# architsharma97/earl_benchmark

Hardware: AMD Instinct MI355X
Metric: env steps/sec (aggregate) at N parallel envs (higher is better)
Workload: dtype f64

## Files before the change

### earl_benchmark_amd/_abi.py

```python
import ctypes as C
import os

EARL_OK = 0
REWARD_SPARSE, REWARD_DENSE = 0, 1
REWARD_TYPES = {'sparse': REWARD_SPARSE, 'dense': REWARD_DENSE}
TABLETOP3_EVAL_CHUNK = 8


class TabletopCfg(C.Structure):
  _fields_ = [('n', C.c_int32), ('env_offset', C.c_int32), ('reward_type', C.c_int32), ('wide_init', C.c_int32),
              ('reset_at_goal', C.c_int32), ('horizon', C.c_int32), ('goal_change_frequency', C.c_int32),
              ('auto_reset', C.c_int32), ('n_goals', C.c_int32), ('n_sample_goals', C.c_int32),
              ('seed', C.c_uint64), ('counter', C.c_uint64)]


class TabletopState(C.Structure):
  _fields_ = [('qpos', C.c_void_p), ('attached', C.c_void_p), ('goal_idx', C.c_void_p), ('goal_table', C.c_void_p),
              ('steps_since_reset', C.c_void_p), ('num_interventions', C.c_void_p),
              ('steps_since_goal_change', C.c_void_p), ('lifelong_return', C.c_void_p), ('counter_base', C.c_void_p)]


class TabletopOut(C.Structure):
  _fields_ = [('obs', C.c_void_p), ('reward', C.c_void_p), ('done', C.c_void_p), ('success', C.c_void_p), ('reward_f64', C.c_void_p)]


ACT_NONE, ACT_RELU, ACT_TANH = 0, 1, 2
ACTIVATIONS = {'none': ACT_NONE, 'relu': ACT_RELU, 'tanh': ACT_TANH}


class MlpPolicy(C.Structure):
  _fields_ = [('n_layers', C.c_int32), ('dims', C.c_int32 * 4), ('hidden_act', C.c_int32), ('out_act', C.c_int32), ('precision', C.c_int32),
              ('params', C.c_void_p)]


HEAD_MEAN, HEAD_SAMPLE = 0, 1
LOGSTD_CLAMP, LOGSTD_TANH = 0, 1
LOGSTD_MAPS = {'clamp': LOGSTD_CLAMP, 'tanh': LOGSTD_TANH}


class GaussianHead(C.Structure):
  _fields_ = [('mode', C.c_int32), ('log_std_map', C.c_int32), ('log_std_min', C.c_float), ('log_std_max', C.c_float), ('eps_out', C.c_void_p)]


class PolicyPopulation(C.Structure):
  _fields_ = [('n_policies', C.c_int32), ('envs_per_policy', C.c_int32), ('param_stride', C.c_int64)]


class EpisodeSummary(C.Structure):
  _fields_ = [('ret', C.c_void_p), ('success_last', C.c_void_p), ('first_success', C.c_void_p)]


class PlanParams(C.Structure):
  _fields_ = [('K', C.c_int32), ('H', C.c_int32), ('iterations', C.c_int32), ('iteration0', C.c_int32), ('sigma', C.c_float * 3), ('noise_counter', C.c_uint32),
              ('inv_temperature', C.c_double)]


class MpcOut(C.Structure):
  _fields_ = [('act', C.c_void_p), ('plan', C.c_void_p), ('ret0', C.c_void_p), ('best_ret', C.c_void_p)]


MPC_MAX_K, MPC_MAX_H = 1024, 256


class PlanValue(C.Structure):
  _fields_ = [('discount', C.c_double), ('value', C.POINTER(MlpPolicy))]


PLAN_VALUE_MAX_H1 = 16


class PlanPrior(C.Structure):
  _fields_ = [('policy', C.POINTER(MlpPolicy)), ('branches', C.c_int32), ('sigma', C.c_float * 3), ('act', C.c_void_p)]


PLAN_PRIOR_MAX_H1 = 16


class CemParams(C.Structure):
  _fields_ = [('K', C.c_int32), ('H', C.c_int32), ('iterations', C.c_int32), ('iteration0', C.c_int32), ('elites', C.c_int32), ('sigma', C.c_float * 3),
              ('noise_counter', C.c_uint32), ('alpha', C.c_float), ('std_min', C.c_float), ('std_max', C.c_float)]


CEM_MAX_K = 1024


class AgentPair(C.Structure):
  _fields_ = [('switch_every', C.c_int32 * 2), ('switch_on_success', C.c_int32), ('pad_', C.c_int32), ('param_stride', C.c_int64), ('backward_goal', C.c_void_p),
              ('phase', C.c_void_p), ('steps_in_phase', C.c_void_p), ('agent_out', C.c_void_p), ('forward_success', C.c_void_p), ('backward_success', C.c_void_p)]


class BackwardGoals(C.Structure):
  _fields_ = [('table', C.c_void_p), ('n_rows', C.c_int32), ('pad_', C.c_int32), ('row', C.c_void_p), ('row_out', C.c_void_p)]


PRECISION_BF16 = 16
PAIR_MAX_H2 = 128


class MotorParams(C.Structure):
  _fields_ = [('kp', C.c_double), ('kd', C.c_double), ('voltage', C.c_double), ('viscous_damping', C.c_double),
              ('torque_control', C.c_int32)]


class KitchenParams(C.Structure):
  _fields_ = [('pos_bound', C.c_double * 2 * 23), ('vel_bound', C.c_double * 2 * 23), ('pos_noise_amp', C.c_double * 23),
              ('act_mid', C.c_double * 9), ('act_amp', C.c_double * 9), ('mocap_range', C.c_double * 3),
              ('mocap_clip_lower', C.c_double * 3), ('mocap_clip_upper', C.c_double * 3), ('step_duration', C.c_double),
              ('robot_noise_ratio', C.c_double)]


class SawyerCfg(C.Structure):
  _fields_ = [('n', C.c_int32), ('env_offset', C.c_int32), ('reward_type', C.c_int32), ('horizon', C.c_int32),
              ('frame_skip', C.c_int32), ('att_hand', C.c_int32), ('att_right', C.c_int32), ('att_left', C.c_int32),
              ('att_obj', C.c_int32), ('obj_dof', C.c_int32), ('obj_kind', C.c_int32), ('n_goal_rows', C.c_int32), ('goal_change_frequency', C.c_int32), ('n_wide', C.c_int32),
              ('att_grasp', C.c_int32), ('att_lpad', C.c_int32), ('att_rpad', C.c_int32), ('pad2_', C.c_int32),
              ('action_scale', C.c_double),
              ('mocap_low', C.c_double * 3), ('mocap_high', C.c_double * 3), ('mocap_quat', C.c_double * 4),
              ('success_radius', C.c_double), ('hand_init_pos', C.c_double * 3), ('obj_init_pos', C.c_double * 3),
              ('obj_init_angle', C.c_double), ('angle_noise', C.c_double * 2),
              ('obj_low', C.c_double * 3), ('obj_high', C.c_double * 3), ('obj_reject_xy', C.c_double * 2), ('obj_reject_radius', C.c_double),
              ('goal_table', C.c_void_p), ('wide_table', C.c_void_p), ('wide_shift', C.c_double * 3), ('wide_noise', C.c_double),
              ('init_tcp', C.c_double * 3), ('box_corners', C.c_double * 3 * 4),
              ('seed', C.c_uint64), ('counter', C.c_uint64), ('step_counter', C.c_uint64)]


class SawyerState(C.Structure):
  _fields_ = [('qpos', C.c_void_p), ('qvel', C.c_void_p), ('mocap_pos', C.c_void_p), ('goal', C.c_void_p),
              ('steps_since_reset', C.c_void_p), ('steps_since_goal_change', C.c_void_p), ('obj_init', C.c_void_p),
              ('last_obs', C.c_void_p), ('fail_count', C.c_void_p), ('sched', C.c_void_p)]


class SawyerOut(C.Structure):
  _fields_ = [('obs', C.c_void_p), ('reward', C.c_void_p), ('done', C.c_void_p), ('success', C.c_void_p), ('status', C.c_void_p), ('info', C.c_void_p)]


class SawyerBranchWs(C.Structure):
  _fields_ = [('base', C.c_void_p), ('bytes', C.c_int64)]


class SawyerPlanParams(C.Structure):
  _fields_ = [('K', C.c_int32), ('H', C.c_int32), ('iterations', C.c_int32), ('iteration0', C.c_int32), ('sigma', C.c_float * 4), ('noise_counter', C.c_uint32),
              ('inv_temperature', C.c_double)]


class SawyerCemParams(C.Structure):
  _fields_ = [('K', C.c_int32), ('H', C.c_int32), ('iterations', C.c_int32), ('iteration0', C.c_int32), ('elites', C.c_int32), ('sigma', C.c_float * 4),
              ('noise_counter', C.c_uint32), ('alpha', C.c_float), ('std_min', C.c_float), ('std_max', C.c_float)]


class SawyerPlanPrior(C.Structure):
  _fields_ = [('policy', C.POINTER(MlpPolicy)), ('branches', C.c_int32), ('sigma', C.c_float * 4), ('obs0', C.c_void_p), ('act', C.c_void_p)]


SAWYER_PLAN_MAX_K = 8192
SAWYER_CEM_MAX_E = 1024
SAWYER_INFO = 8
SAWYER_INFO_KEYS = ('success', 'near_object', 'grasp_success', 'grasp_reward', 'in_place_reward', 'obj_to_target', 'unscaled_reward')
STEP_DIVERGED = 1


class KitchenCfg(C.Structure):
  _fields_ = [('n', C.c_int32), ('env_offset', C.c_int32), ('horizon', C.c_int32), ('frame_skip', C.c_int32), ('sensor_noise', C.c_int32),
              ('n_att', C.c_int32), ('site_att', C.c_int32 * 8), ('seed', C.c_uint64), ('counter', C.c_uint64), ('mocap_quat_dev', C.c_void_p)]


class KitchenState(C.Structure):
  _fields_ = [(k, C.c_void_p) for k in ('qpos', 'qvel', 'mocap_pos', 'goal', 'last_qp_robot', 'att_xpos', 'steps_since_reset', 'fail_count', 'last_obs',
                                        'action64', 'ctrl9', 'noise', 'qpos_bak', 'qvel_bak', 'sites', 'bad', 'mocap_bak', 'att_bak')]


class KitchenOut(C.Structure):
  _fields_ = [(k, C.c_void_p) for k in ('obs', 'reward', 'done', 'success', 'status')]


class MinitaurCfg(C.Structure):
  _fields_ = [('n', C.c_int32), ('env_offset', C.c_int32), ('horizon', C.c_int32), ('num_substeps', C.c_int32), ('settle_steps', C.c_int32),
              ('randomize', C.c_int32), ('n_goals', C.c_int32), ('goal_change_frequency', C.c_int32), ('overheat_steps', C.c_int32),
              ('motor_dof', C.c_int32 * 8), ('pad_', C.c_int32), ('motor_dir', C.c_double * 8), ('motor_kp', C.c_double), ('motor_kd', C.c_double),
              ('motor_velocity_limit', C.c_double), ('overheat_torque', C.c_double), ('distance_weight', C.c_double), ('energy_weight', C.c_double),
              ('success_radius', C.c_double), ('goal_table', C.c_void_p), ('reset_qpos', C.c_void_p),
              ('base_mass_err', C.c_double * 2), ('leg_mass_err', C.c_double * 2), ('leg_mass', C.c_double), ('motor_mass', C.c_double),
              ('foot_friction', C.c_double * 2), ('seed', C.c_uint64), ('counter', C.c_uint64), ('step_counter', C.c_uint64)]


class MinitaurState(C.Structure):
  _fields_ = [(k, C.c_void_p) for k in ('qpos', 'qvel', 'goal', 'motor_param', 'observed_torque', 'overheat', 'motor_enabled', 'steps_since_reset',
                                        'steps_since_goal_change', 'fail_count', 'last_obs')]


class MinitaurOut(C.Structure):
  _fields_ = [(k, C.c_void_p) for k in ('obs', 'reward', 'done', 'success', 'status')]


_P = C.POINTER
SIGNATURES = {
    'earl_tabletop_step': [_P(TabletopCfg), _P(TabletopState), C.c_void_p, C.c_void_p, _P(TabletopOut), C.c_void_p],
    'earl_tabletop_rollout': [_P(TabletopCfg), _P(TabletopState), C.c_int32, C.c_void_p, _P(TabletopOut), C.c_void_p],
    'earl_tabletop_reset_rollout': [_P(TabletopCfg), _P(TabletopState), C.c_int32, C.c_void_p, _P(TabletopOut), C.c_void_p],
    'earl_tabletop_eval_episodes': [_P(TabletopCfg), _P(TabletopState), C.c_int32, C.c_int32, C.c_void_p, C.c_int64, _P(TabletopOut), C.c_void_p],
    'earl_tabletop_policy_rollout': [_P(TabletopCfg), _P(TabletopState), _P(MlpPolicy), C.c_int32, C.c_int32, C.c_int32, _P(TabletopOut), C.c_void_p, C.c_void_p],
    'earl_tabletop_policy_rollout_gaussian': [_P(TabletopCfg), _P(TabletopState), _P(MlpPolicy), _P(GaussianHead), C.c_int32, C.c_int32, C.c_int32, _P(TabletopOut),
                                              C.c_void_p, C.c_void_p],
    'earl_tabletop_population_rollout': [_P(TabletopCfg), _P(TabletopState), _P(MlpPolicy), _P(PolicyPopulation), _P(GaussianHead), C.c_int32, C.c_int32, C.c_int32,
                                         _P(TabletopOut), C.c_void_p, _P(EpisodeSummary), C.c_void_p],
    'earl_tabletop_pair_rollout': [_P(TabletopCfg), _P(TabletopState), _P(MlpPolicy), _P(AgentPair), _P(GaussianHead), C.c_int32, C.c_int32, C.c_int32, _P(TabletopOut),
                                   C.c_void_p, C.c_void_p],
    'earl_tabletop_reset': [_P(TabletopCfg), _P(TabletopState), C.c_void_p, C.c_void_p, C.c_void_p, C.c_void_p],
    'earl_tabletop_observe': [_P(TabletopCfg), _P(TabletopState), _P(TabletopOut), C.c_void_p],
    'earl_tabletop_reward': [C.c_int32, C.c_void_p, C.c_int32, C.c_int32, C.c_void_p, C.c_void_p, C.c_void_p],
    'earl_tabletop_valid_init': [C.c_int32, C.c_void_p, C.c_void_p, C.c_void_p],
    'earl_tabletop3_step': [_P(TabletopCfg), _P(TabletopState), C.c_void_p, _P(TabletopOut), C.c_void_p],
    'earl_tabletop3_rollout': [_P(TabletopCfg), _P(TabletopState), C.c_int32, C.c_void_p, _P(TabletopOut), C.c_void_p],
    'earl_tabletop3_reset': [_P(TabletopCfg), _P(TabletopState), C.c_void_p, C.c_void_p, C.c_void_p],
    'earl_tabletop3_reward': [C.c_int32, C.c_void_p, C.c_int32, C.c_void_p, C.c_void_p, C.c_void_p],
    'earl_tabletop3_eval_episodes': [_P(TabletopCfg), _P(TabletopState), C.c_int32, C.c_int32, C.c_void_p, C.c_int64, _P(TabletopOut), C.c_void_p],
    'earl_tabletop3_policy_rollout': [_P(TabletopCfg), _P(TabletopState), _P(MlpPolicy), _P(PolicyPopulation), _P(GaussianHead), C.c_int32, C.c_int32, C.c_int32,
                                      _P(TabletopOut), C.c_void_p, _P(EpisodeSummary), C.c_void_p],
    'earl_tabletop3_pair_rollout': [_P(TabletopCfg), _P(TabletopState), _P(MlpPolicy), _P(AgentPair), _P(GaussianHead), C.c_int32, C.c_int32, C.c_int32, _P(TabletopOut),
                                    C.c_void_p, C.c_void_p],
    'earl_tabletop_branch_rollout': [_P(TabletopCfg), _P(TabletopState), C.c_int32, C.c_int32, C.c_void_p, C.c_int64, _P(EpisodeSummary), C.c_void_p, C.c_void_p],
    'earl_tabletop3_branch_rollout': [_P(TabletopCfg), _P(TabletopState), C.c_int32, C.c_int32, C.c_void_p, C.c_int64, _P(EpisodeSummary), C.c_void_p, C.c_void_p],
    'earl_tabletop_plan_mppi': [_P(TabletopCfg), _P(TabletopState), _P(PlanParams)] + [C.c_void_p] * 7,
    'earl_tabletop3_plan_mppi': [_P(TabletopCfg), _P(TabletopState), _P(PlanParams)] + [C.c_void_p] * 7,
    'earl_tabletop_plan_candidates': [_P(TabletopCfg), _P(PlanParams), C.c_int32, C.c_void_p, C.c_void_p, C.c_void_p],
    'earl_tabletop_mpc_rollout': [_P(TabletopCfg), _P(TabletopState), _P(PlanParams), C.c_int32, _P(TabletopOut), _P(MpcOut), C.c_void_p],
    'earl_tabletop3_mpc_rollout': [_P(TabletopCfg), _P(TabletopState), _P(PlanParams), C.c_int32, _P(TabletopOut), _P(MpcOut), C.c_void_p],
    'earl_tabletop_plan_mppi_value': [_P(TabletopCfg), _P(TabletopState), _P(PlanParams), _P(PlanValue)] + [C.c_void_p] * 7,
    'earl_tabletop3_plan_mppi_value': [_P(TabletopCfg), _P(TabletopState), _P(PlanParams), _P(PlanValue)] + [C.c_void_p] * 7,
    'earl_tabletop_mpc_rollout_value': [_P(TabletopCfg), _P(TabletopState), _P(PlanParams), _P(PlanValue), C.c_int32, _P(TabletopOut), _P(MpcOut), C.c_void_p],
    'earl_tabletop3_mpc_rollout_value': [_P(TabletopCfg), _P(TabletopState), _P(PlanParams), _P(PlanValue), C.c_int32, _P(TabletopOut), _P(MpcOut), C.c_void_p],
    'earl_tabletop_plan_mppi_prior': [_P(TabletopCfg), _P(TabletopState), _P(PlanParams), _P(PlanValue), _P(PlanPrior)] + [C.c_void_p] * 7,
    'earl_tabletop3_plan_mppi_prior': [_P(TabletopCfg), _P(TabletopState), _P(PlanParams), _P(PlanValue), _P(PlanPrior)] + [C.c_void_p] * 7,
    'earl_tabletop_plan_cem': [_P(TabletopCfg), _P(TabletopState), _P(CemParams), _P(PlanValue)] + [C.c_void_p] * 9,
    'earl_tabletop3_plan_cem': [_P(TabletopCfg), _P(TabletopState), _P(CemParams), _P(PlanValue)] + [C.c_void_p] * 9,
    'earl_tabletop_cem_candidates': [_P(TabletopCfg), _P(CemParams), C.c_int32, C.c_void_p, C.c_void_p, C.c_void_p, C.c_void_p],
    'earl_tabletop_mpc_rollout_cem': [_P(TabletopCfg), _P(TabletopState), _P(CemParams), _P(PlanValue), C.c_int32, _P(TabletopOut), _P(MpcOut), C.c_void_p],
    'earl_tabletop3_mpc_rollout_cem': [_P(TabletopCfg), _P(TabletopState), _P(CemParams), _P(PlanValue), C.c_int32, _P(TabletopOut), _P(MpcOut), C.c_void_p],
    'earl_debug_set_rollout_impl': [C.c_int],
    'earl_debug_set_rollout3_form': [C.c_int],
    'earl_debug_set_rollout_wgs_per_cu': [C.c_int],
    'earl_debug_read_ws_profile': [C.c_void_p, C.c_int32],
    'earl_sawyer_sparse_f64': [C.c_int32, C.c_void_p, C.c_double, C.c_void_p, C.c_void_p, C.c_void_p],
    'earl_sawyer_sparse_f32': [C.c_int32, C.c_void_p, C.c_double, C.c_void_p, C.c_void_p, C.c_void_p],
    'earl_minitaur_leg_to_motor': [C.c_int32, C.c_void_p, C.c_void_p, C.c_void_p],
    'earl_minitaur_motor_torque': [C.c_int32, _P(MotorParams), C.c_void_p, C.c_void_p, C.c_void_p, C.c_void_p, C.c_void_p, C.c_void_p],
    'earl_minitaur_reward': [C.c_int32, C.c_void_p, C.c_double, C.c_double, C.c_double, C.c_void_p, C.c_void_p, C.c_void_p],
    'earl_kitchen_reward': [C.c_int32] + [C.c_void_p] * 6,
    'earl_kitchen_default_params': [_P(KitchenParams)],
    'earl_kitchen_action': [C.c_int32, _P(KitchenParams)] + [C.c_void_p] * 5,
    'earl_kitchen_obs': [C.c_int32, _P(KitchenParams)] + [C.c_void_p] * 5,
    'earl_philox_uniform': [C.c_int32, C.c_int32, C.c_uint64, C.c_uint64, C.c_int32, C.c_uint32, C.c_double, C.c_double, C.c_void_p, C.c_void_p],
    'earl_physics_step': [C.c_void_p, C.c_void_p, C.c_int32, C.c_int32, C.c_int32] + [C.c_void_p] * 7,
    'earl_physics_forward': [C.c_void_p, C.c_void_p, C.c_int32, C.c_int32] + [C.c_void_p] * 9,
    'earl_physics_model_size': [],
    'earl_physics_model24_size': [],
    'earl_collision_model_size': [],
    'earl_sawyer_cfg_size': [],
    'earl_physics_forget_table': [C.c_void_p],
    'earl_debug_set_physics_lanes': [C.c_int],
    'earl_debug_set_door_variant': [C.c_int],
    'earl_debug_set_peg_schedule': [C.c_int],
    'earl_debug_set_sawyer_prior_launches': [C.c_int],
    'earl_kitchen_step': [C.c_void_p, C.c_void_p, _P(KitchenParams), _P(KitchenCfg), _P(KitchenState), C.c_void_p, _P(KitchenOut), C.c_void_p],
    'earl_kitchen_rollout': [C.c_void_p, C.c_void_p, _P(KitchenParams), _P(KitchenCfg), _P(KitchenState), C.c_void_p, C.c_int32, _P(KitchenOut), C.c_void_p],
    'earl_sawyer_rollout': [C.c_void_p, C.c_void_p, C.c_int32, _P(SawyerCfg), _P(SawyerState), C.c_void_p, C.c_int32, _P(SawyerOut), C.c_void_p],
    'earl_minitaur_rollout': [C.c_void_p, C.c_void_p, _P(MinitaurCfg), _P(MinitaurState), C.c_void_p, C.c_int32, _P(MinitaurOut), C.c_void_p],
    'earl_sawyer_rollout_clocked': [C.c_void_p, C.c_void_p, C.c_int32, _P(SawyerCfg), _P(SawyerState), C.c_void_p, C.c_int32, C.c_void_p, _P(SawyerOut), C.c_void_p],
    'earl_kitchen_rollout_clocked': [C.c_void_p, C.c_void_p, _P(KitchenParams), _P(KitchenCfg), _P(KitchenState), C.c_void_p, C.c_int32, C.c_void_p, _P(KitchenOut),
                                     C.c_void_p],
    'earl_minitaur_rollout_clocked': [C.c_void_p, C.c_void_p, _P(MinitaurCfg), _P(MinitaurState), C.c_void_p, C.c_int32, C.c_void_p, _P(MinitaurOut), C.c_void_p],
    'earl_sawyer_policy_rollout': [C.c_void_p, C.c_void_p, C.c_int32, _P(SawyerCfg), _P(SawyerState), _P(MlpPolicy), _P(GaussianHead), C.c_void_p, C.c_int32, C.c_void_p,
                                   C.c_void_p, _P(SawyerOut), C.c_void_p],
    'earl_sawyer_population_rollout': [C.c_void_p, C.c_void_p, C.c_int32, _P(SawyerCfg), _P(SawyerState), _P(MlpPolicy), _P(PolicyPopulation), _P(GaussianHead), C.c_void_p,
                                       C.c_int32, C.c_void_p, C.c_void_p, _P(SawyerOut), _P(EpisodeSummary), C.c_void_p],
    'earl_sawyer_pair_rollout': [C.c_void_p, C.c_void_p, C.c_int32, _P(SawyerCfg), _P(SawyerState), _P(MlpPolicy), _P(AgentPair), _P(GaussianHead), C.c_void_p,
                                 C.c_int32, C.c_void_p, C.c_void_p, _P(SawyerOut), C.c_void_p],
    'earl_sawyer_agents_rollout': [C.c_void_p, C.c_void_p, C.c_int32, _P(SawyerCfg), _P(SawyerState), _P(MlpPolicy), _P(AgentPair), _P(PolicyPopulation), _P(BackwardGoals),
                                   _P(GaussianHead), C.c_void_p, C.c_int32, C.c_void_p, C.c_void_p, _P(SawyerOut), _P(EpisodeSummary), C.c_void_p],
    'earl_sawyer_branch_ws_bytes': [C.c_int32, C.c_int32, C.c_int32, _P(C.c_int64)],
    'earl_sawyer_branch_rollout': [C.c_void_p, C.c_void_p, C.c_int32, _P(SawyerCfg), _P(SawyerState), C.c_int32, C.c_int32, C.c_void_p, C.c_int64, C.c_void_p,
                                   _P(SawyerBranchWs), _P(EpisodeSummary), C.c_void_p, C.c_void_p, C.c_void_p],
    'earl_sawyer_plan_ws_bytes': [C.c_int32, C.c_int32, C.c_int32, C.c_int32, _P(C.c_int64)],
    'earl_sawyer_plan_mppi': [C.c_void_p, C.c_void_p, C.c_int32, _P(SawyerCfg), _P(SawyerState), _P(SawyerPlanParams), C.c_void_p, C.c_void_p, C.c_void_p, C.c_void_p,
                              C.c_void_p, C.c_void_p, C.c_void_p, C.c_void_p, _P(SawyerBranchWs), C.c_void_p],
    'earl_sawyer_plan_candidates': [_P(SawyerCfg), _P(SawyerPlanParams), C.c_int32, C.c_void_p, C.c_void_p, C.c_void_p],
    'earl_sawyer_plan_cem': [C.c_void_p, C.c_void_p, C.c_int32, _P(SawyerCfg), _P(SawyerState), _P(SawyerCemParams)] + [C.c_void_p] * 11 + [_P(SawyerBranchWs), C.c_void_p],
    'earl_sawyer_cem_candidates': [_P(SawyerCfg), _P(SawyerCemParams), C.c_int32, C.c_void_p, C.c_void_p, C.c_void_p, C.c_void_p],
    'earl_sawyer_cem_update': [_P(SawyerCfg), _P(SawyerCemParams), C.c_int32] + [C.c_void_p] * 11,
    'earl_sawyer_value_ws_bytes': [C.c_int32, C.c_int32, C.c_int32, C.c_int32, _P(C.c_int64)],
    'earl_sawyer_branch_rollout_value': [C.c_void_p, C.c_void_p, C.c_int32, _P(SawyerCfg), _P(SawyerState), C.c_int32, C.c_int32, C.c_void_p, C.c_int64, C.c_void_p,
                                         _P(PlanValue), _P(SawyerBranchWs), _P(EpisodeSummary), C.c_void_p, C.c_void_p, C.c_void_p],
    'earl_sawyer_plan_mppi_value': [C.c_void_p, C.c_void_p, C.c_int32, _P(SawyerCfg), _P(SawyerState), _P(SawyerPlanParams), _P(PlanValue)] + [C.c_void_p] * 8
                                   + [_P(SawyerBranchWs), C.c_void_p],
    'earl_sawyer_plan_cem_value': [C.c_void_p, C.c_void_p, C.c_int32, _P(SawyerCfg), _P(SawyerState), _P(SawyerCemParams), _P(PlanValue)] + [C.c_void_p] * 11
                                  + [_P(SawyerBranchWs), C.c_void_p],
    'earl_sawyer_prior_ws_bytes': [C.c_int32, C.c_int32, C.c_int32, C.c_int32, _P(C.c_int64)],
    'earl_sawyer_branch_rollout_prior': [C.c_void_p, C.c_void_p, C.c_int32, _P(SawyerCfg), _P(SawyerState), C.c_int32, C.c_int32, C.c_void_p, C.c_int64, C.c_void_p,
                                         _P(PlanValue), _P(SawyerPlanPrior), C.c_int32, C.c_uint32, _P(SawyerBranchWs), _P(EpisodeSummary), C.c_void_p, C.c_void_p, C.c_void_p],
    'earl_sawyer_plan_mppi_prior': [C.c_void_p, C.c_void_p, C.c_int32, _P(SawyerCfg), _P(SawyerState), _P(SawyerPlanParams), _P(PlanValue), _P(SawyerPlanPrior)]
                                   + [C.c_void_p] * 8 + [_P(SawyerBranchWs), C.c_void_p],
    'earl_sawyer_plan_cem_prior': [C.c_void_p, C.c_void_p, C.c_int32, _P(SawyerCfg), _P(SawyerState), _P(SawyerCemParams), _P(PlanValue), _P(SawyerPlanPrior)]
                                  + [C.c_void_p] * 11 + [_P(SawyerBranchWs), C.c_void_p],
    'earl_minitaur_policy_rollout': [C.c_void_p, C.c_void_p, _P(MinitaurCfg), _P(MinitaurState), _P(MlpPolicy), _P(GaussianHead), C.c_void_p, C.c_int32, C.c_void_p,
                                     C.c_void_p, _P(MinitaurOut), C.c_void_p],
    'earl_minitaur_population_rollout': [C.c_void_p, C.c_void_p, _P(MinitaurCfg), _P(MinitaurState), _P(MlpPolicy), _P(PolicyPopulation), _P(GaussianHead), C.c_void_p,
                                         C.c_int32, C.c_void_p, C.c_void_p, _P(MinitaurOut), _P(EpisodeSummary), C.c_void_p],
    'earl_minitaur_agents_rollout': [C.c_void_p, C.c_void_p, _P(MinitaurCfg), _P(MinitaurState), _P(MlpPolicy), _P(AgentPair), _P(PolicyPopulation), _P(BackwardGoals),
                                     _P(GaussianHead), C.c_void_p, C.c_int32, C.c_void_p, C.c_void_p, _P(MinitaurOut), _P(EpisodeSummary), C.c_void_p],
    'earl_kitchen_population_rollout': [C.c_void_p, C.c_void_p, _P(KitchenParams), _P(KitchenCfg), _P(KitchenState), _P(MlpPolicy), _P(PolicyPopulation), _P(GaussianHead),
                                        C.c_void_p, C.c_int32, C.c_void_p, C.c_void_p, _P(KitchenOut), _P(EpisodeSummary), C.c_void_p],
    'earl_kitchen_agents_rollout': [C.c_void_p, C.c_void_p, _P(KitchenParams), _P(KitchenCfg), _P(KitchenState), _P(MlpPolicy), _P(AgentPair), _P(PolicyPopulation),
                                    _P(BackwardGoals), C.c_void_p, C.c_int32, _P(GaussianHead), C.c_void_p, C.c_int32, C.c_void_p, C.c_void_p, _P(KitchenOut),
                                    _P(EpisodeSummary), C.c_void_p],
    'earl_kitchen_policy_rollout': [C.c_void_p, C.c_void_p, _P(KitchenParams), _P(KitchenCfg), _P(KitchenState), _P(MlpPolicy), _P(GaussianHead), C.c_void_p, C.c_int32,
                                    C.c_void_p, C.c_void_p, _P(KitchenOut), C.c_void_p],
    'earl_minitaur_reset': [C.c_void_p, C.c_void_p, _P(MinitaurCfg), _P(MinitaurState), C.c_void_p, C.c_void_p, C.c_void_p],
    'earl_minitaur_cfg_size': [],
    'earl_debug_set_minitaur_stepper': [C.c_int],
    'earl_debug_set_minitaur_duo': [C.c_int],
    'earl_debug_set_solo': [C.c_int],
    'earl_debug_set_solo_mt': [C.c_int],
    'earl_sawyer_reset': [C.c_void_p, C.c_int32, _P(SawyerCfg), _P(SawyerState)] + [C.c_void_p] * 5,
    'earl_sawyer_observe': [C.c_void_p, C.c_int32, _P(SawyerCfg), _P(SawyerState), C.c_void_p, C.c_void_p],
    'earl_sawyer_door_reward': [_P(SawyerCfg), C.c_int32, C.c_void_p, C.c_void_p, C.c_void_p, C.c_void_p],
    'earl_sawyer_door_info': [_P(SawyerCfg), C.c_int32, C.c_void_p, C.c_void_p, C.c_void_p, C.c_void_p],
    'earl_version': [],
    'earl_last_error': [],
    'earl_device_count': [],
}
_RESTYPES = {'earl_version': C.c_char_p, 'earl_last_error': C.c_char_p}

LIB_PATH = os.path.join(os.path.dirname(os.path.abspath(__file__)), 'csrc', 'libearl_hip.so')
_lib = None


class EarlHipError(RuntimeError):
  pass


def load():
  global _lib
  if _lib is None:
    if not os.path.exists(LIB_PATH):
      raise EarlHipError(f'{LIB_PATH} not found: build it with `python -c "import __graft_entry__ as g; g.build()"` '
                         '(or `make -C earl_benchmark_amd/csrc`). There is no CPU fallback.')
    import torch
    lib = C.CDLL(LIB_PATH)
    for name, argtypes in SIGNATURES.items():
      fn = getattr(lib, name)
      fn.argtypes = argtypes
      fn.restype = _RESTYPES.get(name, C.c_int)
    _lib = lib
  return _lib


HOST_LIB_PATH = os.path.join(os.path.dirname(os.path.abspath(__file__)), 'csrc', 'libearl_host.so')
HOST_SIGNATURES = {name + '_cpu': argtypes[:-1] for name, argtypes in SIGNATURES.items()
                   if name.startswith(('earl_tabletop_', 'earl_tabletop3_'))}
HOST_EXTRA_SIGNATURES = {
    'earl_mlp_policy_forward_cpu': ([_P(MlpPolicy), _P(GaussianHead), C.c_int32, C.c_void_p, C.c_void_p, C.c_void_p], C.c_int32),
    'earl_sawyer_plan_candidates_cpu': ([_P(SawyerCfg), _P(SawyerPlanParams), C.c_int32, C.c_void_p, C.c_void_p], C.c_int32),
    'earl_sawyer_plan_update_cpu': ([_P(SawyerCfg), _P(SawyerPlanParams), C.c_int32] + [C.c_void_p] * 7, C.c_int32),
    'earl_sawyer_cem_candidates_cpu': ([_P(SawyerCfg), _P(SawyerCemParams), C.c_int32, C.c_void_p, C.c_void_p, C.c_void_p], C.c_int32),
    'earl_sawyer_cem_update_cpu': ([_P(SawyerCfg), _P(SawyerCemParams), C.c_int32] + [C.c_void_p] * 10, C.c_int32),
    'earl_sawyer_value_terminal_cpu': ([_P(PlanValue), C.c_int32, C.c_int32, C.c_void_p, C.c_void_p], C.c_int32),
    'earl_sawyer_prior_actions_cpu': ([_P(SawyerCfg), _P(SawyerPlanPrior), C.c_int32, C.c_int32, C.c_int32, C.c_uint32, C.c_int32, C.c_void_p, C.c_void_p], C.c_int32),
    'earl_tanh_f32': ([C.c_float], C.c_float),
    'earl_exp_f32': ([C.c_float], C.c_float),
    'earl_normal_quantile_f32': ([C.c_uint32], C.c_float),
}
_host = None


class HostLib:

  def __init__(self, cdll):
    self._cdll = cdll
    for name, argtypes in HOST_SIGNATURES.items():
      fn = getattr(cdll, name)
      fn.argtypes, fn.restype = argtypes, C.c_int
      setattr(self, name, fn)
      setattr(self, name[:-4], (lambda f: (lambda *a: f(*a[:-1])))(fn))
    for name, (argtypes, restype) in HOST_EXTRA_SIGNATURES.items():
      fn = getattr(cdll, name)
      fn.argtypes, fn.restype = argtypes, restype
      setattr(self, name, fn)
    cdll.earl_host_last_error.restype = C.c_char_p
    cdll.earl_host_version.restype = C.c_char_p
    cdll.earl_host_set_threads.argtypes = [C.c_int]
    self.earl_last_error = cdll.earl_host_last_error
    self.earl_version = cdll.earl_host_version
    self.set_threads = cdll.earl_host_set_threads


def load_host():
  global _host
  if _host is None:
    if not os.path.exists(HOST_LIB_PATH):
      raise EarlHipError(f'{HOST_LIB_PATH} not found: build it with `make -C earl_benchmark_amd/csrc libearl_host.so`')
    try:
      flags = next((ln for ln in open('/proc/cpuinfo') if ln.startswith('flags')), '')
    except OSError:
      flags = 'avx2 fma'
    missing = [f for f in ('avx2', 'fma') if f not in flags.split()]
    if missing:
      raise EarlHipError(f'{HOST_LIB_PATH} needs a CPU with {" and ".join(missing)} (built with -mavx2 -mfma); this one has neither the HIP path (device="cpu" was asked for) nor those')
    _host = HostLib(C.CDLL(HOST_LIB_PATH))
  return _host


def check(rc, what, lib=None):
  if rc != EARL_OK:
    msg = (lib or load()).earl_last_error()
    raise EarlHipError(f'{what} failed with code {rc}: {msg.decode() if msg else "?"}')
```

### earl_benchmark_amd/csrc/minitaur_stepper.h

```cpp
#pragma once

template <int CTRL>
__device__ __forceinline__ double dpp_quad(const double v) {
  const int lo = __builtin_amdgcn_update_dpp(0, __double2loint(v), CTRL, 0xf, 0xf, false);
  const int hi = __builtin_amdgcn_update_dpp(0, __double2hiint(v), CTRL, 0xf, 0xf, false);
  return __hiloint2double(hi, lo);
}
template <int CTRL> __device__ __forceinline__ V3 dpp_quad(const V3& v) { return {dpp_quad<CTRL>(v.x), dpp_quad<CTRL>(v.y), dpp_quad<CTRL>(v.z)}; }
template <int CTRL> __device__ __forceinline__ Q4 dpp_quad(const Q4& q) { return {dpp_quad<CTRL>(q.w), dpp_quad<CTRL>(q.x), dpp_quad<CTRL>(q.y), dpp_quad<CTRL>(q.z)}; }
constexpr int QP_PARENT = 0xA0;
constexpr int QP_CHILD = 0xF5;
constexpr int QP_SWAP1 = 0xB1;
constexpr int QP_SWAP2 = 0x4E;
template <int P> constexpr int qp_bcast() { return P * 0x55; }

__device__ __forceinline__ double kc(double x) {
  asm volatile("" : "+s"(x));
  return x;
}
__device__ __forceinline__ void sincos_kc(double x, double& sn, double& cs) {
  const double k = rint(x * kc(6.36619772367581382433e-01));
  double r = fma(-k, kc(1.57079632673412561417e+00), x);
  r = fma(-k, kc(6.07710050650619224932e-11), r);
  const double z = r * r;
  double ps = fma(z, kc(1.58969099521155010221e-10), kc(-2.50507602534068634195e-08));
  ps = fma(z, ps, kc(2.75573137070700676789e-06));
  ps = fma(z, ps, kc(-1.98412698298579493134e-04));
  ps = fma(z, ps, kc(8.33333333332248946124e-03));
  ps = fma(z, ps, kc(-1.66666666666666324348e-01));
  const double sr = fma(r * z, ps, r);
  double pc = fma(z, kc(-1.13596475577881948265e-11), kc(2.08757232129817482790e-09));
  pc = fma(z, pc, kc(-2.75573143513906633035e-07));
  pc = fma(z, pc, kc(2.48015872894767294178e-05));
  pc = fma(z, pc, kc(-1.38888888888741095749e-03));
  pc = fma(z, pc, kc(4.16666666666666019037e-02));
  const double cr = fma(z * z, pc, fma(-0.5, z, 1.0));
  const int q = (int)k & 3;
  sn = (q == 0) ? sr : ((q == 1) ? cr : ((q == 2) ? -sr : -cr));
  cs = (q == 0) ? cr : ((q == 1) ? -sr : ((q == 2) ? -cr : sr));
}

#ifdef EARL_MT_DEBUG
__device__ int g_mt_dbg[4096 * 8 * 32];
__device__ double g_mt_dbg_al[4096 * 8 * 32];
__device__ double g_mt_dbg_x[5][4096 * 8 * 32];
__device__ double g_mt_dbg_ph[8][4096 * 8 * 32];
#define DBG_PH(k, v) do { if (isl) g_mt_dbg_ph[k][((size_t)s.dbg_env * 8 + (s.dbg_ts & 7)) * 32 + l] = (v); } while (0)
#else
#define DBG_PH(k, v) do {} while (0)
#endif
struct MTDims {
  static constexpr int NV = 22, NR = 6, NLEG = 4, LS = 4, NH = 16, LPE = 32, MC = EARL_MAXCON, MB = 8;
};

struct PairTabMT {
  static constexpr int MP = 64;
  double pos[MP][3], r[MP], margin[MP];
  int link[MP], cls[MP];
};
__device__ __forceinline__ void stage_pairs_mt(PairTabMT& t, const earl_collision_model* __restrict__ col) {
  const int i = threadIdx.x;
  if (col && i < PairTabMT::MP && i < col->n_pair) {
    t.pos[i][0] = col->pair_rec[i].pos[0]; t.pos[i][1] = col->pair_rec[i].pos[1]; t.pos[i][2] = col->pair_rec[i].pos[2];
    t.r[i] = col->pair_rec[i].r; t.margin[i] = col->pair_rec[i].margin;
    t.link[i] = col->pair_rec[i].sph_link; t.cls[i] = col->pair_rec[i].cls;
  }
}
template <int N>
__device__ __forceinline__ void chol_small(double (&L)[N * (N + 1) / 2]) {
#pragma unroll
  for (int j = 0; j < N; ++j) {
    double d = L[j * (j + 1) / 2 + j];
#pragma unroll
    for (int p = 0; p < j; ++p) d = fma(-L[j * (j + 1) / 2 + p], L[j * (j + 1) / 2 + p], d);
    const double inv = rsq2(d);
    L[j * (j + 1) / 2 + j] = inv;
#pragma unroll
    for (int i = j + 1; i < N; ++i) {
      double t = L[i * (i + 1) / 2 + j];
#pragma unroll
      for (int p = 0; p < j; ++p) t = fma(-L[i * (i + 1) / 2 + p], L[j * (j + 1) / 2 + p], t);
      L[i * (i + 1) / 2 + j] = t * inv;
    }
  }
}

struct SharedMTData {
  static constexpr int NV = MTDims::NV, MC = MTDims::MC;
  double qp[NV], qv[NV];
  double bq[4];
  double aprev[NV];
  struct { double ext[NV]; double motor_volt, motor_visc; double mscale[3], foot_mu; } xt;
  double eres[12], eD[12], ear[12];
  struct { double obs_t[8], cmd[8]; int oh[8], en[8]; double goal[2]; int steps, sgc, pad_[2]; } ev;
  struct { double cD, cmu, car[4]; unsigned int cact; int cd1, cd2, pid; } c3[MC];
  unsigned int tb[NV][4];
#ifdef EARL_MT_DEBUG
  int dbg_env, dbg_ts, dbg_pad[2];
#endif
  union {
    double ct[MC][8];
    double cw[MC][8];
  };
  double CJr[MC][3][6];
  double CJh[MC][3][2];
  int crow[MC][2];
  union {
    struct { double obs[46]; } kit;
    struct {
      double Xq[NV][4], Xp[NV][3];
      double Sh[MTDims::NH][6];
      double redI[9][10];
      double redF[9][6];
    } dyn;
    struct {
      double Bw[NV][6];
      double rw[NV];
      double sh_keep[MTDims::NH][6];
      double Aw[MTDims::NH][4];
      int nct;
    } hand;
    struct {
      double HA[MTDims::NLEG][10];
      double HB[MTDims::NH][6];
      double HR[6][6];
      double rc[NV];
      double Wl[6][16];
      double part[6][4];
      double Y[16];
      double LL[MTDims::NLEG][10];
      double SS[22];
      double xr0[6];
    } pas;
  };
};
static_assert(sizeof(((SharedMTData*)nullptr)->ev) % 16 == 0 && sizeof(((SharedMTData*)nullptr)->c3) % 16 == 0 && sizeof(((SharedMTData*)nullptr)->tb) % 16 == 0 && offsetof(SharedMTData, dyn) % 16 == 0, "16-byte alignment of the blocks the kernels read as b128");
static_assert(offsetof(SharedMTData, hand.sh_keep) == offsetof(SharedMTData, dyn.Sh) && offsetof(SharedMTData, hand.Aw) == offsetof(SharedMTData, dyn.redI) &&
              sizeof(((SharedMTData*)nullptr)->hand) <= sizeof(((SharedMTData*)nullptr)->dyn), "the hand-over block keeps clear of the motion subspaces and fits the dynamics block");
struct SharedMT : SharedMTData {
  static constexpr int R = (int)(sizeof(SharedMTData) % 256);
  static constexpr int PAD = R <= 64 ? 64 - R : (R <= 192 ? 192 - R : 320 - R);
  char bank_pad[PAD == 0 ? 16 : PAD];
};
static_assert(sizeof(SharedMT) % 16 == 0, "an env block is a whole number of 16-byte words: the blocks of one wave all keep the alignment ds_read_b128 needs");

__device__ __forceinline__ void integrate_mt(SharedMT& s, const earl_link_model24& m, const int sub, const bool isl, const int l, const double dt, const double al,
                                             const double qd, const double ql_, const Q4 Qb) {
  fence();
  if (isl) {
    const double nv_ = fma(dt, al, qd);
    s.qv[l] = nv_;
    s.qp[l] = fma(dt, nv_, ql_);
  }
  fence();
  {
    const int bd = m.ball_dof;
    const V3 wbd{s.qv[bd], s.qv[bd + 1], s.qv[bd + 2]};
    auto norm2 = [](const Q4& q) { return fma(q.z, q.z, fma(q.y, q.y, fma(q.x, q.x, q.w * q.w))); };
    auto mul4 = [](const Q4& a, const Q4& b) {
      return Q4{fma(-a.z, b.z, fma(-a.y, b.y, fma(-a.x, b.x, a.w * b.w))), fma(-a.z, b.y, fma(a.y, b.z, fma(a.x, b.w, a.w * b.x))),
                fma(a.z, b.x, fma(a.y, b.w, fma(-a.x, b.z, a.w * b.y))), fma(a.z, b.w, fma(-a.y, b.x, fma(a.x, b.y, a.w * b.z)))};
    };
    Q4 q0 = Qb;
    const double n0 = rsq2(norm2(q0));
    q0 = Q4{q0.w * n0, q0.x * n0, q0.y * n0, q0.z * n0};
    const double w2 = fma(wbd.z, wbd.z, fma(wbd.y, wbd.y, wbd.x * wbd.x));
    const double iw = w2 > 0 ? rsq2(w2 > 0 ? w2 : 1.0) : 0.0;
    double sn, cs;
    sincos_kc(0.5 * dt * (w2 * iw), sn, cs);
    const Q4 q1 = mul4(q0, Q4{cs, sn * wbd.x * iw, sn * wbd.y * iw, sn * wbd.z * iw});
    const double n1 = rsq2(norm2(q1));
    if (sub == 0) { s.bq[0] = q1.w * n1; s.bq[1] = q1.x * n1; s.bq[2] = q1.y * n1; s.bq[3] = q1.z * n1; }
    fence();
  }
}

template <bool INTEGRATE, int ROLE = 0>
__device__ __forceinline__ void substep_mt(SharedMT& s, const earl_link_model24& m, const BlkTable<MTDims::MB, true>& bt, const PairTabMT& pt,
                                           const int sub, const int grp, const bool warm, double* qacc_out) {
  constexpr int NV = MTDims::NV, MC = MTDims::MC, LPE = MTDims::LPE;
  const int maxcon = bt.max_con < MC ? bt.max_con : MC;
  const double dt = m.dt;
  const bool isroot = sub < 6, ishinge = sub >= 8 && sub < 24, isl = isroot || ishinge;
  const int l = isroot ? sub : (ishinge ? sub - 2 : NV - 1);
  const int hq = (sub - 8) & 3;
  const int leg = ishinge ? (sub - 8) >> 2 : 0;
  const bool lower = ishinge && (hq & 1), upper = ishinge && !(hq & 1);
  PSTART();
  const V3 Pb = ld3(s.qp);
  const Q4 Qb = ldq(s.bq);
  double Rb[3][3];
  qmat(Qb, Rb);
  Q4 Q; V3 P;
  const V3 ax = ld3(m.jaxis[l]);
  const int jt = m.jtype[l];
  const double ql_ = s.qp[l], qd = s.qv[l];
  double Bw[6], Aw[4], rw;
  int nct = 0, ncmax = 0;
  if constexpr (ROLE != 2) {
  {
    const Q4 tq = ldq(m.tquat[l]);
    const V3 tp = ld3(m.tpos[l]);
    double sn, cs;
    sincos_kc(jt == 0 ? 0.5 * ql_ : 0.0, sn, cs);
    const Q4 qloc = qmul(tq, Q4{cs, sn * ax.x, sn * ax.y, sn * ax.z});
    const Q4 Qu = qmul(Qb, qloc);
    const V3 Pu = add(Pb, mulv(Rb, tp));
    const Q4 Qp = dpp_quad<QP_PARENT>(Qu);
    const V3 Pp = dpp_quad<QP_PARENT>(Pu);
    double Rp[3][3];
    qmat(Qp, Rp);
    const Q4 Qw = qmul(Qp, qloc);
    const V3 Pw = add(Pp, mulv(Rp, tp));
    const Q4 Qr = selq(sub < 3, Q4{1, 0, 0, 0}, Qb);
    const V3 Pr{Pb.x, sub >= 1 ? Pb.y : 0.0, sub >= 2 ? Pb.z : 0.0};
    Q = selq(isroot, Qr, selq(lower, Qw, Qu));
    P = selv(isroot, Pr, selv(lower, Pw, Pu));
  }
#ifdef EARL_MT_DEBUG_FRAMES
  DBG_PH(0, Q.w); DBG_PH(1, Q.x); DBG_PH(2, Q.y); DBG_PH(3, Q.z); DBG_PH(4, P.x); DBG_PH(5, P.y); DBG_PH(6, P.z); DBG_PH(7, ql_);
#else
  DBG_PH(0, Q.w + 2 * Q.x + 3 * Q.y + 5 * Q.z + 7 * P.x + 11 * P.y + 13 * P.z);
  DBG_PH(5, ql_); DBG_PH(6, Qb.w + 2 * Qb.x + 3 * Qb.y + 5 * Qb.z + 7 * Pb.x + 11 * Pb.y + 13 * Pb.z); DBG_PH(7, qd);
#endif
  if (isl) {
    double* oq = s.dyn.Xq[l];
    double* op = s.dyn.Xp[l];
    oq[0] = Q.w; oq[1] = Q.x; oq[2] = Q.y; oq[3] = Q.z; op[0] = P.x; op[1] = P.y; op[2] = P.z;
  }
  fence();
  unsigned int nearw = 0, nearg = 0;
  {
    const int b = sub < bt.n_blk ? sub : 0;
    const int bl = bt.link[b];
    V3 cs = ld3(bt.center[b]);
    {
      double Rl[3][3];
      qmat(ldq(s.dyn.Xq[bl < 0 ? 0 : bl]), Rl);
      cs = selv(bl < 0, cs, add(ld3(s.dyn.Xp[bl < 0 ? 0 : bl]), mulv(Rl, cs)));
    }
    double Rbx[3][3];
    qmat(ldq(bt.box_quat[b]), Rbx);
    const V3 x = mulvT(Rbx, vsub(cs, ld3(bt.box_pos[b]))), h = ld3(bt.box_half[b]);
    const V3 d{x.x - fmin(fmax(x.x, -h.x), h.x), x.y - fmin(fmax(x.y, -h.y), h.y), x.z - fmin(fmax(x.z, -h.z), h.z)};
    const bool nearb = sub < bt.n_blk && dot(d, d) < bt.reach[b] * bt.reach[b];
    const unsigned long long bal = __ballot(nearb);
    nearg = (unsigned int)((bal >> (grp * 32)) & 0xFFFFFFFFull);
    nearw = (unsigned int)((bal | (bal >> 32)) & 0xFFFFFFFFull);
  }
  PSTAMP(0);
  V3 Sw, Sv;
  double I10[10];
  double R[3][3];
  qmat(Q, R);
  {
    const V3 aw = mulv(R, ax);
    const V3 anchor = add(P, mulv(R, ld3(m.jpos[l])));
    const bool rot = jt != 1;
    Sw = selv(rot, aw, V3{0, 0, 0});
    Sv = selv(rot, cross(anchor, aw), aw);
    const int root = m.ball_dof + 2;
    const double ms = l < root ? 1.0 : (l == root ? s.xt.mscale[0] : (m.parent[l] == root ? s.xt.mscale[1] : s.xt.mscale[2]));
    const double mass = m.mass[l] * ms;
    const V3 c = add(P, mulv(R, ld3(m.com[l])));
    const double* in = m.inertia[l];
    const double I[3][3] = {{in[0] * ms, in[3] * ms, in[4] * ms}, {in[3] * ms, in[1] * ms, in[5] * ms}, {in[4] * ms, in[5] * ms, in[2] * ms}};
    double T[3][3], W[3][3];
#pragma unroll
    for (int r = 0; r < 3; ++r)
#pragma unroll
      for (int cc = 0; cc < 3; ++cc) T[r][cc] = R[r][0] * I[0][cc] + R[r][1] * I[1][cc] + R[r][2] * I[2][cc];
#pragma unroll
    for (int r = 0; r < 3; ++r)
#pragma unroll
      for (int cc = r; cc < 3; ++cc) W[r][cc] = T[r][0] * R[cc][0] + T[r][1] * R[cc][1] + T[r][2] * R[cc][2];
    const double c2 = dot(c, c);
    I10[0] = mass;
    I10[1] = mass * c.x; I10[2] = mass * c.y; I10[3] = mass * c.z;
    I10[4] = W[0][0] + mass * (c2 - c.x * c.x);
    I10[5] = W[1][1] + mass * (c2 - c.y * c.y);
    I10[6] = W[2][2] + mass * (c2 - c.z * c.z);
    I10[7] = W[0][1] - mass * c.x * c.y;
    I10[8] = W[0][2] - mass * c.x * c.z;
    I10[9] = W[1][2] - mass * c.y * c.z;
    if (ishinge) {
      double* o = s.dyn.Sh[l - 6];
      o[0] = Sw.x; o[1] = Sw.y; o[2] = Sw.z; o[3] = Sv.x; o[4] = Sv.y; o[5] = Sv.z;
    }
  }
  
#ifndef EARL_MT_DEBUG_FRAMES
  DBG_PH(1, Sw.x + 2 * Sw.y + 3 * Sw.z + 5 * Sv.x + 7 * Sv.y + 11 * Sv.z + 13 * I10[0] + 17 * I10[1] + 19 * I10[2] + 23 * I10[3] + 29 * I10[4] + 31 * I10[5] + 37 * I10[6] + 41 * I10[7] + 43 * I10[8] + 47 * I10[9]);
#endif
  PSTAMP(1);
  double Ic[10];
#pragma unroll
  for (int e = 0; e < 10; ++e) {
    const double ch = dpp_quad<QP_CHILD>(I10[e]);
    Ic[e] = upper ? I10[e] + ch : I10[e];
  }
  if (upper || sub == 5) {
    double* o = s.dyn.redI[upper ? (l - 6) >> 1 : 8];
#pragma unroll
    for (int e = 0; e < 10; ++e) o[e] = Ic[e];
  }
  fence();
  {
    double tot[10];
#pragma unroll
    for (int e = 0; e < 10; ++e) tot[e] = s.dyn.redI[8][e];
#ifndef EARL_MT_NO_CHUNK
#define EARL_MT_NO_CHUNK 0
#endif
    if constexpr (ROLE == 0 || EARL_MT_NO_CHUNK) {
#pragma unroll
      for (int u = 0; u < 8; ++u)
#pragma unroll
        for (int e = 0; e < 10; ++e) tot[e] += s.dyn.redI[u][e];
    } else {
#pragma unroll
      for (int u = 0; u < 8; u += 2) {
        double part[20];
#pragma unroll
        for (int e = 0; e < 10; ++e) { part[e] = s.dyn.redI[u][e]; part[10 + e] = s.dyn.redI[u + 1][e]; }
        pin_batch(part);
#pragma unroll
        for (int e = 0; e < 10; ++e) tot[e] += part[e];
#pragma unroll
        for (int e = 0; e < 10; ++e) tot[e] += part[10 + e];
        pin_batch(tot);
      }
    }
#pragma unroll
    for (int e = 0; e < 10; ++e) Ic[e] = isroot ? tot[e] : Ic[e];
  }
  
#ifndef EARL_MT_DEBUG_FRAMES
  DBG_PH(2, Ic[0] + 2 * Ic[1] + 3 * Ic[2] + 5 * Ic[3] + 7 * Ic[4] + 11 * Ic[5] + 13 * Ic[6] + 17 * Ic[7] + 19 * Ic[8] + 23 * Ic[9]);
#endif
  PSTAMP(3);
  double g6[6], Add, Ach;
  {
    V3 n, f;
    iapply(Ic, Sw, Sv, n, f);
    const V3 mo = mulvT(Rb, add(n, cross(f, Pb)));
    g6[0] = f.x; g6[1] = f.y; g6[2] = f.z; g6[3] = mo.x; g6[4] = mo.y; g6[5] = mo.z;
    Add = dot(Sw, n) + dot(Sv, f) + m.armature[l];
    const V3 nc = dpp_quad<QP_CHILD>(n), fc = dpp_quad<QP_CHILD>(f);
    Ach = dot(Sw, nc) + dot(Sv, fc);
  }
  
#ifndef EARL_MT_DEBUG_FRAMES
  DBG_PH(3, g6[0] + 2 * g6[1] + 3 * g6[2] + 5 * g6[3] + 7 * g6[4] + 11 * g6[5] + 13 * Add + 17 * Ach);
#endif
  PSTAMP(4);
  const V3 vlin = ld3(s.qv), om = ld3(s.qv + 3);
  const V3 wb = mulv(Rb, om);
  const V3 vb = add(vlin, cross(Pb, wb));
  double tau_l;
  {
    const V3 wu = add(wb, scl(Sw, qd)), vu = add(vb, scl(Sv, qd));
    const V3 wpar = dpp_quad<QP_PARENT>(wu), vpar = dpp_quad<QP_PARENT>(vu);
    const V3 w = selv(isroot, wb, selv(lower, add(wpar, scl(Sw, qd)), wu));
    const V3 v = selv(isroot, vb, selv(lower, add(vpar, scl(Sv, qd)), vu));
    const V3 cwh = scl(cross(w, Sw), qd), cvh = scl(add(cross(v, Sw), cross(w, Sv)), qd);
    const V3 cw = selv(ishinge, cwh, V3{0, 0, 0});
    const V3 cv = selv(ishinge, cvh, scl(cross(vlin, Sw), qd));
    const V3 ab{-m.gravity[0], -m.gravity[1], -m.gravity[2]};
    const V3 avb = add(ab, cross(vlin, wb));
    const V3 awu = cw, avu = add(avb, cv);
    const V3 awp = dpp_quad<QP_PARENT>(awu), avp = dpp_quad<QP_PARENT>(avu);
    const V3 aw = selv(isroot, V3{0, 0, 0}, selv(lower, add(awp, cw), awu));
    const V3 av = selv(isroot, avb, selv(lower, add(avp, cv), avu));
    V3 n1, f1, n2, f2;
    iapply(I10, aw, av, n1, f1);
    iapply(I10, w, v, n2, f2);
    const V3 n = add(n1, add(cross(w, n2), cross(v, f2)));
    const V3 f = add(f1, cross(w, f2));
    const V3 nch = dpp_quad<QP_CHILD>(n), fch = dpp_quad<QP_CHILD>(f);
    V3 ns = selv(upper, add(n, nch), n), fs = selv(upper, add(f, fch), f);
    if (upper || sub == 5) {
      double* o = s.dyn.redF[upper ? (l - 6) >> 1 : 8];
      o[0] = ns.x; o[1] = ns.y; o[2] = ns.z; o[3] = fs.x; o[4] = fs.y; o[5] = fs.z;
    }
    fence();
    V3 nt = ld3(s.dyn.redF[8]), ft = ld3(s.dyn.redF[8] + 3);
    if constexpr (ROLE == 0 || EARL_MT_NO_CHUNK) {
#pragma unroll
      for (int u = 0; u < 8; ++u) { nt = add(nt, ld3(s.dyn.redF[u])); ft = add(ft, ld3(s.dyn.redF[u] + 3)); }
    } else {
#pragma unroll
      for (int u = 0; u < 8; u += 4) {
        double part[24];
#pragma unroll
        for (int k = 0; k < 24; ++k) part[k] = s.dyn.redF[u + k / 6][k % 6];
        pin_batch(part);
#pragma unroll
        for (int w = 0; w < 4; ++w) { nt = add(nt, V3{part[6 * w], part[6 * w + 1], part[6 * w + 2]}); ft = add(ft, V3{part[6 * w + 3], part[6 * w + 4], part[6 * w + 5]}); }
        nt = V3{pinned(nt.x), pinned(nt.y), pinned(nt.z)}; ft = V3{pinned(ft.x), pinned(ft.y), pinned(ft.z)};
      }
    }
    ns = selv(isroot, nt, ns); fs = selv(isroot, ft, fs);
    tau_l = -m.damping[l] * qd - (dot(Sw, ns) + dot(Sv, fs)) + s.xt.ext[l];
  }
  
#ifndef EARL_MT_DEBUG_FRAMES
  DBG_PH(4, tau_l);
#endif
  PSTAMP(5);
  if (nearw) {
    unsigned int rest = nearw;
    while (rest) {
      int myb = -1, myoff = 0, used = 0;
      unsigned int taken = 0;
      for (unsigned int r2 = rest; r2; r2 &= r2 - 1u) {
        const int b = __builtin_ctz(r2);
        const int sz = bt.end[b] - bt.begin[b];
        if (used + sz > LPE) { if (used == 0) { taken = 1u << b; used = sz; if (sub < sz) { myb = b; myoff = 0; } } break; }
        if (sub >= used && sub < used + sz) { myb = b; myoff = used; }
        used += sz;
        taken |= 1u << b;
      }
      rest &= ~taken;
      const bool has = myb >= 0;
      const int b = has ? myb : 0;
      const bool mine = has && ((nearg >> b) & 1u);
      const int bsz = bt.end[b] - bt.begin[b];
      const V3 pb = ld3(bt.box_pos[b]);
      double Rbx[3][3];
      qmat(ldq(bt.box_quat[b]), Rbx);
      const V3 h = ld3(bt.box_half[b]);
      const int room = bt.cap[b] & 255;
      const int pi = has ? bt.begin[b] + (sub - myoff < bsz ? sub - myoff : bsz - 1) : 0;
      const bool valid = mine && sub - myoff < bsz;
      const int lk = pt.link[pi], cls = pt.cls[pi];
      const double r = pt.r[pi], margin = pt.margin[pi];
      V3 c = ld3(pt.pos[pi]);
      {
        double Rl[3][3];
        qmat(ldq(s.dyn.Xq[lk < 0 ? 0 : lk]), Rl);
        c = selv(lk < 0, c, add(ld3(s.dyn.Xp[lk < 0 ? 0 : lk]), mulv(Rl, c)));
      }
      const V3 x = mulvT(Rbx, vsub(c, pb));
      V3 q{fmin(fmax(x.x, -h.x), h.x), fmin(fmax(x.y, -h.y), h.y), fmin(fmax(x.z, -h.z), h.z)};
      const bool outside = fabs(x.x) > h.x || fabs(x.y) > h.y || fabs(x.z) > h.z;
      const V3 dd = vsub(x, q);
      const double d2 = dot(dd, dd);
      const double inv = rsq2(outside ? d2 : 1.0);
      const double gx = h.x - fabs(x.x), gy = h.y - fabs(x.y), gz = h.z - fabs(x.z);
      const int axn = (gx <= gy && gx <= gz) ? 0 : (gy <= gz ? 1 : 2);
      const double xa = pick3(x, axn), ha = pick3(h, axn), sg = xa >= 0 ? 1.0 : -1.0;
      const V3 ni{axn == 0 ? sg : 0.0, axn == 1 ? sg : 0.0, axn == 2 ? sg : 0.0};
      const V3 qi{axn == 0 ? sg * ha : x.x, axn == 1 ? sg * ha : x.y, axn == 2 ? sg * ha : x.z};
      const double dist = outside ? d2 * inv - r : -(ha - fabs(xa)) - r;
      const V3 nl = selv(outside, scl(dd, inv), ni);
      q = selv(outside, q, qi);
      const bool hit = valid && dist < margin;
      const unsigned long long bal = __ballot(hit);
      const unsigned int gb = (unsigned int)((bal >> (grp * 32)) & 0xFFFFFFFFull);
      const unsigned int seg = has ? (unsigned int)(((1ull << bsz) - 1ull) << myoff) : 0u;
      const int before_blk = __popc(gb & seg & ((1u << sub) - 1u));
      const bool accept = hit && before_blk < room;
      const unsigned long long bal2 = __ballot(accept);
      const unsigned int ga = (unsigned int)((bal2 >> (grp * 32)) & 0xFFFFFFFFull);
      const int slot = nct + __popc(ga & ((1u << sub) - 1u));
      if (accept && slot < maxcon) {
        const V3 n = mulv(Rbx, nl);
        const V3 p = add(add(pb, mulv(Rbx, q)), scl(n, 0.5 * dist));
        double* o = s.ct[slot];
        o[0] = dist; o[1] = n.x; o[2] = n.y; o[3] = n.z; o[4] = p.x; o[5] = p.y; o[6] = p.z;
        o[7] = (double)(cls + 64 * (lk + 1) + 4096 * pi);
      }
      const int took = __popc(ga);
      nct = nct + took < maxcon ? nct + took : maxcon;
    }
    fence();
  }
  PSTAMP(2);
  PCOUNT(20, 1); PCOUNT(21, nearw ? 1 : 0); PCOUNT(22, __popc(nearw));
  if (nearw && __any(nct > 0)) {
#pragma unroll
    for (int k = 0; k < MC; ++k) ncmax = __any(nct > k) ? k + 1 : ncmax;
  }
  {
    const int k1 = m.con_att1[leg], k2 = m.con_att2[leg];
    const V3 pa = add(P, mulv(R, ld3(m.att_pos[hq == 3 ? k1 : k2])));
    const V3 p1 = dpp_quad<qp_bcast<3>()>(pa), p2 = dpp_quad<qp_bcast<1>()>(pa);
    const V3 d = vsub(p1, p2);
    const double w1 = (ishinge && hq >= 2) ? 1.0 : 0.0, w2 = (ishinge && hq < 2) ? 1.0 : 0.0;
    const V3 JE = vsub(scl(add(Sv, cross(Sw, p1)), w1), scl(add(Sv, cross(Sw, p2)), w2));
    V3 jv = scl(JE, qd);
    jv = add(jv, dpp_quad<QP_SWAP1>(jv));
    jv = add(jv, dpp_quad<QP_SWAP2>(jv));
    jv = add(jv, cross(wb, d));
    const int c = hq < 3 ? hq : 2;
    const double res = pick3(d, c);
    double kk, bb;
    kb_of(m.con_solref[leg], m.con_solimp[leg], dt, kk, bb);
    const double dd = imp_p2(m.con_solimp[leg], res);
    const double eDm = rcp_nr(fmax((1 - dd) * m.con_invweight[leg] * rcp_nr(dd), 1e-15));
    const double earm = -bb * pick3(jv, c) - kk * dd * res;
    if (ishinge && hq < 3) { s.eres[3 * leg + hq] = res; s.eD[3 * leg + hq] = eDm; s.ear[3 * leg + hq] = earm; }
    const V3 eDv{dpp_quad<qp_bcast<0>()>(eDm), dpp_quad<qp_bcast<1>()>(eDm), dpp_quad<qp_bcast<2>()>(eDm)};
    const V3 earv{dpp_quad<qp_bcast<0>()>(earm), dpp_quad<qp_bcast<1>()>(earm), dpp_quad<qp_bcast<2>()>(earm)};
    const V3 dj{eDv.x * JE.x, eDv.y * JE.y, eDv.z * JE.z};
    const V3 bx = mulvT(Rb, cross(d, dj));
    double Bh[6] = {g6[0], g6[1], g6[2], g6[3] + bx.x, g6[4] + bx.y, g6[5] + bx.z};
    double Ah[4];
    {
      const V3 j0 = dpp_quad<qp_bcast<0>()>(JE), j1 = dpp_quad<qp_bcast<1>()>(JE), j2 = dpp_quad<qp_bcast<2>()>(JE), j3 = dpp_quad<qp_bcast<3>()>(JE);
      Ah[0] = dot(j0, dj); Ah[1] = dot(j1, dj); Ah[2] = dot(j2, dj); Ah[3] = dot(j3, dj);
#pragma unroll
      for (int p = 0; p < 4; ++p) Ah[p] += p == hq ? Add : ((upper && p == hq + 1) ? Ach : 0.0);
    }
    const double gh = tau_l + dot(dj, earv);
    fence();
    V3 T{0, 0, 0}, G{0, 0, 0};
#pragma unroll
    for (int e = 0; e < MTDims::NLEG; ++e) {
      const V3 de = ld3(s.eres + 3 * e), De = ld3(s.eD + 3 * e), are = ld3(s.ear + 3 * e);
      const V3 sd = cross(Sw, de);
      const V3 u{De.x * sd.x, De.y * sd.y, De.z * sd.z};
      T = add(T, cross(de, u));
      G = add(G, cross(de, V3{De.x * are.x, De.y * are.y, De.z * are.z}));
    }
    const V3 rx = mulvT(Rb, T);
    double Br[6] = {g6[0], g6[1], g6[2], g6[3] + rx.x, g6[4] + rx.y, g6[5] + rx.z};
#pragma unroll
    for (int i = 0; i < 6; ++i) Br[i] += sub == i ? m.armature[l] : 0.0;
    const double gr = tau_l + dot(Sw, G);
#pragma unroll
    for (int i = 0; i < 6; ++i) Bw[i] = isroot ? Br[i] : Bh[i];
#pragma unroll
    for (int p = 0; p < 4; ++p) Aw[p] = Ah[p];
    rw = isroot ? gr : gh;
  }
  PSTAMP(7);
  }
  if constexpr (ROLE == 1) {
    if (isl) {
#pragma unroll
      for (int i = 0; i < 6; ++i) s.hand.Bw[l][i] = Bw[i];
      s.hand.rw[l] = rw;
    }
    if (ishinge) {
#pragma unroll
      for (int p = 0; p < 4; ++p) s.hand.Aw[l - 6][p] = Aw[p];
    }
    if (sub == 0) s.hand.nct = nct;
  }
  if constexpr (ROLE == 0) {
    pin_batch(Bw); pin_batch(Aw); rw = pinned(rw);
  }
  if constexpr (ROLE == 2) {
    nct = s.hand.nct;
    if (__any(nct > 0)) {
#pragma unroll
      for (int k = 0; k < MC; ++k) ncmax = __any(nct > k) ? k + 1 : ncmax;
    }
  }
  double cD = 0, cmu = 0, car[4] = {0, 0, 0, 0};
  unsigned int cact = 0;
  int cd1 = -1, cd2 = -1;
  int cpid = -1;
  if constexpr (ROLE == 2) {
    const int c = sub < MC ? sub : MC - 1;
    cD = s.c3[c].cD; cmu = s.c3[c].cmu;
#pragma unroll
    for (int k = 0; k < 4; ++k) car[k] = s.c3[c].car[k];
    cact = s.c3[c].cact; cd1 = s.c3[c].cd1; cd2 = s.c3[c].cd2;
  }
  if (ROLE != 2 && ncmax > 0) {
    const int c = sub < MC ? sub : MC - 1;
    const bool cv = sub < nct;
    unsigned int pact = s.c3[c].cact;
    int ppid = s.c3[c].pid;
    double rec[8];
#pragma unroll
    for (int k = 0; k < 8; ++k) rec[k] = s.ct[c][k];
    pin_batch(rec);
    asm volatile("" : "+v"(pact), "+v"(ppid));
#pragma unroll
    for (int k = 0; k < 8; ++k) rec[k] = cv ? rec[k] : 0.0;
    const V3 n = selv(cv, V3{rec[1], rec[2], rec[3]}, V3{0, 0, 1}), p = selv(cv, V3{rec[4], rec[5], rec[6]}, V3{0, 0, 0});
    const int pk = cv ? (int)rec[7] : 0;
    const int cls = pk & 63, ls = ((pk >> 6) & 63) - 1;
    cpid = cv ? (pk >> 12) : -1;
    const double ax_ = fabs(n.x), ay_ = fabs(n.y), az_ = fabs(n.z);
    const int ia = (ax_ <= ay_ && ax_ <= az_) ? 0 : (ay_ <= az_ ? 1 : 2);
    const V3 e{ia == 0 ? 1.0 : 0.0, ia == 1 ? 1.0 : 0.0, ia == 2 ? 1.0 : 0.0};
    V3 t1 = cross(n, e);
    t1 = scl(t1, rsq2(dot(t1, t1)));
    const V3 t2 = cross(n, t1);
    cd2 = ls >= 6 ? ls : -1;
    double ctab[6] = {bt.cls_margin[cls], bt.cls_mu[cls], bt.kb_cls[cls][0], bt.kb_cls[cls][1], bt.cls_invw[cls], s.xt.foot_mu};
    double simp[5];
#pragma unroll
    for (int k = 0; k < 5; ++k) simp[k] = bt.cls_solimp[cls][k];
    int par2 = m.parent[cd2 >= 0 ? cd2 : 0], parls = m.parent[ls > 0 ? ls : 0];
    asm volatile("" : "+v"(par2), "+v"(parls));
    pin_batch(ctab); pin_batch(simp);
    cd1 = (cd2 >= 0 && par2 >= 6) ? par2 : -1;
    const V3 rp = vsub(p, Pb);
    const V3 dirs[3] = {n, t1, t2};
    double Jr[3][6], Jh[3][2];
    double sh1[6], sh2[6], qa[4] = {s.qv[cd1 >= 0 ? cd1 : 0], s.qv[cd2 >= 0 ? cd2 : 0], s.aprev[cd1 >= 0 ? cd1 : 0], s.aprev[cd2 >= 0 ? cd2 : 0]};
#pragma unroll
    for (int k = 0; k < 6; ++k) { sh1[k] = s.dyn.Sh[cd1 >= 0 ? cd1 - 6 : 0][k]; sh2[k] = s.dyn.Sh[cd2 >= 0 ? cd2 - 6 : 0][k]; }
    double qr[6], ar[6];
#pragma unroll
    for (int r = 0; r < 6; ++r) { qr[r] = s.qv[r]; ar[r] = s.aprev[r]; }
    pin_batch(sh1); pin_batch(sh2); pin_batch(qa); pin_batch(qr); pin_batch(ar);
    const double* s1 = sh1;
    const double* s2 = sh2;
    const V3 jp1 = add(ld3(s1 + 3), cross(ld3(s1), p)), jp2 = add(ld3(s2 + 3), cross(ld3(s2), p));
#pragma unroll
    for (int k = 0; k < 3; ++k) {
      const V3 t = dirs[k];
      const V3 mo = mulvT(Rb, cross(rp, t));
      Jr[k][0] = cv ? t.x : 0.0; Jr[k][1] = cv ? t.y : 0.0; Jr[k][2] = cv ? t.z : 0.0;
      Jr[k][3] = cv ? mo.x : 0.0; Jr[k][4] = cv ? mo.y : 0.0; Jr[k][5] = cv ? mo.z : 0.0;
      Jh[k][0] = cd1 >= 0 ? dot(t, jp1) : 0.0;
      Jh[k][1] = cd2 >= 0 ? dot(t, jp2) : 0.0;
    }
    if (sub < MC) {
#pragma unroll
      for (int k = 0; k < 3; ++k) {
#pragma unroll
        for (int r = 0; r < 6; ++r) s.CJr[c][k][r] = Jr[k][r];
        s.CJh[c][k][0] = Jh[k][0]; s.CJh[c][k][1] = Jh[k][1];
      }
      s.crow[c][0] = cd1; s.crow[c][1] = cd2;
    }
    double jv[3], jp[3];
    {
      const double q1 = cd1 >= 0 ? qa[0] : 0.0, q2 = cd2 >= 0 ? qa[1] : 0.0;
      const double a1 = cd1 >= 0 ? qa[2] : 0.0, a2 = cd2 >= 0 ? qa[3] : 0.0;
#pragma unroll
      for (int k = 0; k < 3; ++k) {
        double a_ = 0, b_ = 0;
#pragma unroll
        for (int r = 0; r < 6; ++r) { a_ = fma(Jr[k][r], qr[r], a_); b_ = fma(Jr[k][r], ar[r], b_); }
        a_ = fma(Jh[k][0], q1, a_); a_ = fma(Jh[k][1], q2, a_);
        b_ = fma(Jh[k][0], a1, b_); b_ = fma(Jh[k][1], a2, b_);
        jv[k] = a_; jp[k] = b_;
      }
    }
    const double margin = ctab[0];
    cmu = ctab[1];
    {
      const int root = m.ball_dof + 2;
      cmu = (ctab[5] > 0 && ls > root && parls != root) ? ctab[5] : cmu;
    }
    const double kk = ctab[2], bb = ctab[3];
    const double dd = imp_p2(simp, rec[0] - margin);
    const double R0 = fmax((1 - dd) * ctab[4] * rcp_nr(dd), 1e-15);
    cD = cv ? rcp_nr(2 * cmu * cmu * R0) : 0.0;
    const double basea = -kk * dd * (rec[0] - margin);
    car[0] = fma(-bb, fma(cmu, jv[1], jv[0]), basea); car[1] = fma(-bb, fma(-cmu, jv[1], jv[0]), basea);
    car[2] = fma(-bb, fma(cmu, jv[2], jv[0]), basea); car[3] = fma(-bb, fma(-cmu, jv[2], jv[0]), basea);
    unsigned int wbits = 0;
    wbits |= (fma(cmu, jp[1], jp[0]) - car[0] < 0) ? 1u : 0u;
    wbits |= (fma(-cmu, jp[1], jp[0]) - car[1] < 0) ? 2u : 0u;
    wbits |= (fma(cmu, jp[2], jp[0]) - car[2] < 0) ? 4u : 0u;
    wbits |= (fma(-cmu, jp[2], jp[0]) - car[3] < 0) ? 8u : 0u;
#ifndef EARL_MT_NO_CARRY
    cact = cv ? (warm ? ((ppid == cpid) ? pact : wbits) : 0xFu) : 0u;
#else
    cact = cv ? (warm ? wbits : 0xFu) : 0u;
#endif
  }
#ifdef EARL_MT_DEBUG
  if constexpr (ROLE != 2) {
    int* row = g_mt_dbg + ((size_t)s.dbg_env * 8 + (s.dbg_ts & 7)) * 32;
    if (sub < MC) row[4 + sub] = (int)cact;
    if (sub == 0) { row[0] = nct; row[1] = warm ? 1 : 0; }
  }
#endif
  if constexpr (ROLE == 0) {
    cD = pinned(cD); cmu = pinned(cmu); pin_batch(car);
    asm volatile("" : "+v"(cact), "+v"(cd1), "+v"(cd2));
  }
  if constexpr (ROLE == 1) {
    if (sub < MC) {
      s.c3[sub].cD = cD; s.c3[sub].cmu = cmu;
#pragma unroll
      for (int k = 0; k < 4; ++k) s.c3[sub].car[k] = car[k];
      s.c3[sub].cact = cact; s.c3[sub].cd1 = cd1; s.c3[sub].cd2 = cd2; s.c3[sub].pid = cpid;
    }
  }
  unsigned int tbits = 0, sbits = 0, cbits = 0;
  if constexpr (ROLE == 2) {
    tbits = s.tb[l][0]; sbits = s.tb[l][1]; cbits = s.tb[l][2];
  }
  if (ROLE != 2 && ncmax > 0) {
    fence();
#pragma unroll
    for (int c = 0; c < MC; ++c) {
      const int d1 = s.crow[c][0], d2 = s.crow[c][1];
      tbits |= (isroot || l == d1 || l == d2) ? (1u << c) : 0u;
      sbits |= l == d2 ? (1u << c) : 0u;
      cbits |= l == d1 ? (1u << c) : 0u;
    }
  }
  if constexpr (ROLE == 1) {
    if (isl) { s.tb[l][0] = tbits; s.tb[l][1] = sbits; s.tb[l][2] = cbits; }
    return;
  }
  PSTAMP(6);
  PSTAMP(9);
  if constexpr (ROLE == 2) {
    const int hl = ishinge ? l - 6 : 0;
#pragma unroll
    for (int i = 0; i < 6; ++i) Bw[i] = s.hand.Bw[l][i];
#pragma unroll
    for (int p = 0; p < 4; ++p) Aw[p] = s.hand.Aw[hl][p];
    rw = s.hand.rw[l];
    pin_batch(Bw); pin_batch(Aw); rw = pinned(rw);
    fence();
  }
#ifdef EARL_MT_DEBUG
  if (isl) {
    const size_t o_ = ((size_t)s.dbg_env * 8 + (s.dbg_ts & 7)) * 32 + l;
    g_mt_dbg_x[0][o_] = rw;
    g_mt_dbg_x[1][o_] = Bw[0] + 2 * Bw[1] + 3 * Bw[2] + 5 * Bw[3] + 7 * Bw[4] + 11 * Bw[5];
    g_mt_dbg_x[2][o_] = Aw[0] + 2 * Aw[1] + 3 * Aw[2] + 5 * Aw[3];
    g_mt_dbg_x[4][o_] = s.xt.ext[l];
  }
#endif
  double al = 0.0;
  PCOUNT(23, ncmax > 0 ? 1 : 0); PCOUNT(24, ncmax);
  for (int it = 0; it < 8; ++it) {
    PCOUNT(25, 1);
#ifdef EARL_MT_DEBUG
    if (sub == 0) g_mt_dbg[((size_t)s.dbg_env * 8 + (s.dbg_ts & 7)) * 32 + 2] = it + 1;
#endif
    KSTART();
    if (ncmax > 0) {
      if (sub < MC) {
        const double a1 = (cact & 1u) ? cD : 0.0, a2 = (cact & 2u) ? cD : 0.0, a3 = (cact & 4u) ? cD : 0.0, a4 = (cact & 8u) ? cD : 0.0;
        double* w = s.cw[sub];
        w[0] = a1 + a2 + a3 + a4; w[1] = cmu * (a1 - a2); w[2] = cmu * (a3 - a4); w[3] = cmu * cmu * (a1 + a2); w[4] = cmu * cmu * (a3 + a4);
        w[5] = a1 * car[0] + a2 * car[1] + a3 * car[2] + a4 * car[3];
        w[6] = cmu * (a1 * car[0] - a2 * car[1]);
        w[7] = cmu * (a3 * car[2] - a4 * car[3]);
      }
      fence();
    }
    KSTAMP(16);
    {
      double acc6[6] = {0, 0, 0, 0, 0, 0}, accd = 0, accc = 0, rr = rw;
      static_assert(MC % 4 == 0, "contact slots in groups of four");
      for (int c4 = 0; c4 < ncmax; c4 += 4) {
#pragma unroll
        for (int u = 0; u < 4; ++u) {
          const int c = c4 + u;
          const double* w = s.cw[c];
          const int slot = (sbits >> c) & 1u;
          const double tmask = ((tbits >> c) & 1u) ? 1.0 : 0.0, cmask = ((cbits >> c) & 1u) ? 1.0 : 0.0;
          double j[3], jc[3], wv[8], jr[18];
  #pragma unroll
          for (int k = 0; k < 3; ++k) {
            j[k] = *(isroot ? &s.CJr[c][k][l] : &s.CJh[c][k][slot]);
            jc[k] = s.CJh[c][k][1];
          }
  #pragma unroll
          for (int k = 0; k < 8; ++k) wv[k] = w[k];
  #pragma unroll
          for (int k = 0; k < 3; ++k)
  #pragma unroll
            for (int i = 0; i < 6; ++i) jr[6 * k + i] = s.CJr[c][k][i];
          pin6(j[0], j[1], j[2], jc[0], jc[1], jc[2]); pin_batch(wv); pin_batch(jr);
  #pragma unroll
          for (int k = 0; k < 3; ++k) j[k] *= tmask;
          const double v0 = wv[0] * j[0] + wv[1] * j[1] + wv[2] * j[2], v1 = wv[1] * j[0] + wv[3] * j[1], v2 = wv[2] * j[0] + wv[4] * j[2];
          rr += wv[5] * j[0] + wv[6] * j[1] + wv[7] * j[2];
  #pragma unroll
          for (int i = 0; i < 6; ++i) acc6[i] += jr[i] * v0 + jr[6 + i] * v1 + jr[12 + i] * v2;
          accd += j[0] * v0 + j[1] * v1 + j[2] * v2;
          accc += (jc[0] * v0 + jc[1] * v1 + jc[2] * v2) * cmask;
        }
      }
      if (isroot) {
#pragma unroll
        for (int i = 0; i < 6; ++i) s.pas.HR[l][i] = Bw[i] + acc6[i];
      }
      if (ishinge) {
#pragma unroll
        for (int i = 0; i < 6; ++i) s.pas.HB[l - 6][i] = Bw[i] + acc6[i];
#pragma unroll
        for (int p = 0; p < 4; ++p)
          if (p >= hq) s.pas.HA[leg][p * (p + 1) / 2 + hq] = Aw[p] + (p == hq ? accd : ((upper && p == hq + 1) ? accc : 0.0));
      }
      if (isl) s.pas.rc[l] = rr;
    }
    fence();
    KSTAMP(17);
    double xr[6];
    {
      const int t = sub < 24 ? sub : 23;
      const int i = t % 6, k = t / 6;
      double L[10], Bc[4], bk[4];
#pragma unroll
      for (int e = 0; e < 10; ++e) L[e] = s.pas.HA[k][e];
#pragma unroll
      for (int j = 0; j < 4; ++j) { Bc[j] = s.pas.HB[4 * k + j][i]; bk[j] = s.pas.rc[6 + 4 * k + j]; }
      pin_batch(L); pin_batch(Bc); pin_batch(bk);
      chol_small<4>(L);
      double W[4], y[4], pt = 0.0;
#pragma unroll
      for (int j = 0; j < 4; ++j) {
        double sw = Bc[j], sy = bk[j];
#pragma unroll
        for (int p = 0; p < j; ++p) { sw = fma(-W[p], L[j * (j + 1) / 2 + p], sw); sy = fma(-y[p], L[j * (j + 1) / 2 + p], sy); }
        W[j] = sw * L[j * (j + 1) / 2 + j];
        y[j] = sy * L[j * (j + 1) / 2 + j];
        pt = fma(W[j], y[j], pt);
      }
      if (sub < 24) {
#pragma unroll
        for (int j = 0; j < 4; ++j) s.pas.Wl[i][4 * k + j] = W[j];
        s.pas.part[i][k] = pt;
        if (i == 0) {
#pragma unroll
          for (int j = 0; j < 4; ++j) s.pas.Y[4 * k + j] = y[j];
#pragma unroll
          for (int e = 0; e < 10; ++e) s.pas.LL[k][e] = L[e];
        }
      }
    }
    fence();
    {
      const int e = sub < 21 ? sub : 20;
      const int i = e >= 15 ? 5 : (e >= 10 ? 4 : (e >= 6 ? 3 : (e >= 3 ? 2 : (e >= 1 ? 1 : 0))));
      const int c = e - i * (i + 1) / 2;
      double s0 = s.pas.HR[i][c], s1 = 0.0, s2 = 0.0, s3 = 0.0;
      double wi[16], wc[16];
#pragma unroll
      for (int p = 0; p < 16; ++p) { wi[p] = s.pas.Wl[i][p]; wc[p] = s.pas.Wl[c][p]; }
      s0 = pinned(s0); pin_batch(wi); pin_batch(wc);
#pragma unroll
      for (int p = 0; p < 16; p += 4) {
        s0 = fma(-wi[p], wc[p], s0); s1 = fma(-wi[p + 1], wc[p + 1], s1);
        s2 = fma(-wi[p + 2], wc[p + 2], s2); s3 = fma(-wi[p + 3], wc[p + 3], s3);
      }
      if (sub < 21) s.pas.SS[e] = (s0 + s1) + (s2 + s3);
      const int ri = sub >= 21 && sub < 27 ? sub - 21 : 0;
      const double x0 = s.pas.rc[ri] - ((s.pas.part[ri][0] + s.pas.part[ri][1]) + (s.pas.part[ri][2] + s.pas.part[ri][3]));
      if (sub >= 21 && sub < 27) s.pas.xr0[ri] = x0;
    }
    fence();
    {
      double Lr[21];
#pragma unroll
      for (int e = 0; e < 21; ++e) Lr[e] = s.pas.SS[e];
#pragma unroll
      for (int i = 0; i < 6; ++i) xr[i] = s.pas.xr0[i];
      double Lk[10], z[4], wl[24];
#pragma unroll
      for (int e = 0; e < 10; ++e) Lk[e] = s.pas.LL[leg][e];
#pragma unroll
      for (int j = 0; j < 4; ++j) {
        z[j] = s.pas.Y[4 * leg + j];
#pragma unroll
        for (int i = 0; i < 6; ++i) wl[6 * j + i] = s.pas.Wl[i][4 * leg + j];
      }
      pin_batch(Lr); pin_batch(xr); pin_batch(Lk); pin_batch(z);
      chol_small<6>(Lr);
      solve_regs<6, 6>(Lr, xr);
#pragma unroll
      for (int j = 0; j < 4; ++j) {
        double zz = z[j];
#pragma unroll
        for (int i = 0; i < 6; ++i) zz = fma(-wl[6 * j + i], xr[i], zz);
        z[j] = zz;
      }
#pragma unroll
      for (int j = 3; j >= 0; --j) {
        double zz = z[j];
#pragma unroll
        for (int p = j + 1; p < 4; ++p) zz = fma(-Lk[p * (p + 1) / 2 + j], z[p], zz);
        z[j] = zz * Lk[j * (j + 1) / 2 + j];
      }
      const double xh = hq == 0 ? z[0] : (hq == 1 ? z[1] : (hq == 2 ? z[2] : z[3]));
      double xo = 0.0;
#pragma unroll
      for (int i = 0; i < 6; ++i) xo = sub == i ? xr[i] : xo;
      al = isroot ? xo : xh;
      if (isl) s.aprev[l] = al;
    }
    KSTAMP(18);
    bool changed = false;
    if (ncmax > 0) {
      fence();
      const int c = sub < MC ? sub : MC - 1;
      double cj[18], ch[6], ah[2] = {s.aprev[cd1 >= 0 ? cd1 : 0], s.aprev[cd2 >= 0 ? cd2 : 0]};
#pragma unroll
      for (int k = 0; k < 3; ++k) {
#pragma unroll
        for (int r = 0; r < 6; ++r) cj[6 * k + r] = s.CJr[c][k][r];
        ch[2 * k] = s.CJh[c][k][0]; ch[2 * k + 1] = s.CJh[c][k][1];
      }
      pin_batch(ah); pin_batch(ch); pin_batch(cj);
      const double a1 = cd1 >= 0 ? ah[0] : 0.0, a2 = cd2 >= 0 ? ah[1] : 0.0;
      double an[3];
#pragma unroll
      for (int k = 0; k < 3; ++k) {
        double a_ = 0;
#pragma unroll
        for (int r = 0; r < 6; ++r) a_ = fma(cj[6 * k + r], xr[r], a_);
        a_ = fma(ch[2 * k], a1, a_); a_ = fma(ch[2 * k + 1], a2, a_);
        an[k] = a_;
      }
      unsigned int nb = 0;
      nb |= (fma(cmu, an[1], an[0]) - car[0] < 0) ? 1u : 0u;
      nb |= (fma(-cmu, an[1], an[0]) - car[1] < 0) ? 2u : 0u;
      nb |= (fma(cmu, an[2], an[0]) - car[2] < 0) ? 4u : 0u;
      nb |= (fma(-cmu, an[2], an[0]) - car[3] < 0) ? 8u : 0u;
      nb = sub < nct ? nb : 0u;
      changed = nb != cact;
      cact = nb;
    }
    KSTAMP(19);
    if (!__any(changed)) break;
    PCOUNT(10, it == 2 ? 1 : 0);
    PCOUNT(12, it == 6 ? 1 : 0);
  }
#ifdef EARL_MT_DEBUG
  {
    int* row = g_mt_dbg + ((size_t)s.dbg_env * 8 + (s.dbg_ts & 7)) * 32;
    if (sub < MC) row[16 + sub] = (int)cact;
    if (isl) reinterpret_cast<double*>(g_mt_dbg_al)[((size_t)s.dbg_env * 8 + (s.dbg_ts & 7)) * 32 + l] = al;
    fence();
    if (sub == 0) s.dbg_ts = s.dbg_ts + 1;
    fence();
  }
#endif
  if constexpr (ROLE == 2) {
    if (ncmax > 0 && sub < MC) s.c3[sub].cact = cact;
  } else {
    if (sub < MC) { s.c3[sub].cact = cact; s.c3[sub].pid = cpid; }
  }
  PSTAMP(8);
  if constexpr (ROLE == 2) return;
  if constexpr (!INTEGRATE) {
    if (qacc_out && isl) qacc_out[l] = al;
  } else {
    integrate_mt(s, m, sub, isl, l, dt, al, qd, ql_, Qb);
#ifdef EARL_MT_DEBUG
    if (isl) g_mt_dbg_x[3][((size_t)s.dbg_env * 8 + ((s.dbg_ts - 1) & 7)) * 32 + l] = s.qv[l];
#endif
    PSTAMP(11);
  }
}
```

### earl_benchmark_amd/csrc/physics_env_minitaur.h

```cpp

struct MinitaurArgs {
  const void* m;
  const earl_collision_model* col;
  earl_minitaur_cfg cfg;
  earl_minitaur_state st;
  earl_minitaur_out out;
  const float* action; int T;
  const uint8_t* mask; double* reset_obs;
  int solo;
  const uint64_t* clock;
};
__device__ __forceinline__ double mt_draw(const earl_minitaur_cfg& cfg, const uint32_t stream, const int env, const uint64_t counter) {
  const earl::U4 b = earl::philox4x32_10(earl::U4{stream, (uint32_t)(cfg.env_offset + env), (uint32_t)counter, (uint32_t)(counter >> 32)},
                                         (uint32_t)cfg.seed, (uint32_t)(cfg.seed >> 32));
  return earl::u01(b.x, b.y);
}
#ifndef EARL_MT_WPB
#define EARL_MT_WPB 4
#endif
#ifndef EARL_MT_BLOCKS
#define EARL_MT_BLOCKS 1
#endif
#ifndef EARL_MT_DUO_DEFAULT
#define EARL_MT_DUO_DEFAULT -1
#endif
template <bool ARROW> constexpr int mt_wpb() { return ARROW ? EARL_MT_WPB : Lim<22>::WPB; }

#include "policy_closed_loop.h"
struct MinitaurPolicyArgs : ClosedLoopArgs<MinitaurArgs> {};
static_assert(std::is_standard_layout<MinitaurArgs>::value && std::is_trivially_copyable<MinitaurPolicyArgs>::value, "the policy phase reads MinitaurPolicyArgs as laid out in the kernel-argument segment");
__device__ __noinline__ float minitaur_policy_action(const uint64_t ka_bits, const uint64_t ev, const uint32_t gid, const uint64_t seed, const double* __restrict__ seen, const int env,
                                                     const size_t row, const int sub, const bool live) {
#pragma clang fp contract(off)
  const EARL_KARG MinitaurPolicyArgs* ka = cl_kernarg<MinitaurPolicyArgs>(ka_bits);
  const int n_layers = ka->pol.n_layers, d1 = ka->pol.dims[1], d2 = ka->pol.dims[2], d3 = ka->pol.dims[3];
  const int hidden_act = ka->pol.hidden_act, out_act = ka->pol.out_act;
  if (!seen) seen = ka->obs0 + (size_t)env * 32;
  float h[8];
  h[0] = live ? (float)seen[sub] : 0.f;
#pragma unroll
  for (int i = 1; i < 8; ++i) h[i] = 0.f;
  const pol_elem* w = cl_policy_weights(ka, gid, env, row, sub == 0 && live);
  pol_layer<32, true>(w, w + (size_t)d1 * 32, 32, d1, hidden_act, sub, h);
  w += (size_t)d1 * (32 + 1);
  if (n_layers == 3) {
    pol_layer<32, true>(w, w + (size_t)d2 * d1, d1, d2, hidden_act, sub, h);
    w += (size_t)d2 * (d1 + 1);
  }
  const int KL = n_layers == 3 ? d2 : d1, NL = n_layers == 3 ? d3 : d2;
  pol_layer<32, true>(w, w + (size_t)NL * KL, KL, NL, EARL_ACT_NONE, sub, h);
  float u;
  if (ka->gauss) {
    const float raw = __shfl(h[0], (sub & 7) + 8, 32);
    const int d = sub & 3;
    const earl::U4 b = earl::philox4x32_10(earl::U4{earl::kGaussDraw + (uint32_t)((sub >> 2) & 1), gid, (uint32_t)ev, (uint32_t)(ev >> 32)}, (uint32_t)seed, (uint32_t)(seed >> 32));
    const float eps = earl::normal_quantile_f32((d == 0 ? b.x : (d == 1 ? b.y : (d == 2 ? b.z : b.w))) >> 8);
    u = earl::gaussian_head_action(earl_gaussian_head{ka->head.mode, ka->head.log_std_map, ka->head.log_std_min, ka->head.log_std_max, nullptr}, out_act, h[0], raw, eps);
    float* eps_out = ka->head.eps_out;
    if (sub < 8 && live && eps_out) eps_out[row * 8 + sub] = eps;
  } else {
    u = earl::policy_act(h[0], out_act);
  }
  float* act_out = ka->act_out;
  if (sub < 8 && live && act_out) act_out[row * 8 + sub] = u;
  return u;
}
template <bool POLICY, class A>
__device__ __forceinline__ void mt_step_action(const A& a, const int t, const int n, const int env, const int sub, const bool live, double (&a64)[8]) {
#pragma clang fp contract(off)
  const size_t row = (size_t)t * n + env;
  if constexpr (POLICY) {
    const double* seen = t > 0 ? (a.out.obs ? a.out.obs + (row - n) * 32 : a.st.last_obs + (size_t)env * 32) : nullptr;
    const uint64_t ev = a.cfg.step_counter + (a.clock ? a.clock[1] : 0) + (uint64_t)t;
    const float u = minitaur_policy_action((uint64_t)cl_kernarg<MinitaurPolicyArgs>(), ev, (uint32_t)(a.cfg.env_offset + env), a.cfg.seed, seen, env, row, sub, live);
#pragma unroll
    for (int k = 0; k < 8; ++k) a64[k] = earl::mt_clipd((double)__shfl(u, k, 32), -1.01, 1.01);
  } else {
#pragma unroll
    for (int k = 0; k < 8; ++k) a64[k] = earl::mt_clipd((double)a.action[row * 8 + k], -1.01, 1.01);
  }
}
template <class A>
__device__ __forceinline__ void mt_pair_handover(const A& a, const int t, const int env, const size_t row, const int sub, const bool live, const bool failed, const uint8_t suc,
                                                 double& goal0, double& goal1) {
#pragma clang fp contract(off)
  const bool success = __shfl((int)((!failed && suc) ? 1 : 0), 0, 32) != 0;
  cl_pair_handover(cl_kernarg<MinitaurPolicyArgs>(), t, env, row, sub == 0 && live, success, (uint32_t)(a.cfg.env_offset + env), a.cfg.seed, a.cfg.step_counter,
                   a.clock ? a.clock + 1 : nullptr, a.cfg.goal_table, a.cfg.n_goals, [&](const double* table, const int gi) {
                     goal0 = table[2 * gi]; goal1 = table[2 * gi + 1];
                     if (live && sub >= 30) (a.out.obs ? a.out.obs + row * 32 : a.st.last_obs + (size_t)env * 32)[sub] = sub == 30 ? goal0 : goal1;
                     if (live && sub == 0) { a.st.goal[(size_t)env * 2] = goal0; a.st.goal[(size_t)env * 2 + 1] = goal1; }
                   });
}
template <bool RESET, bool ARROW>
__global__ __launch_bounds__(64 * mt_wpb<ARROW>(), ARROW ? EARL_MT_BLOCKS : 1) void minitaur_kernel(const MinitaurArgs a) {
#include "physics_env_minitaur_rollout.inc"
}
template <bool RESET, bool ARROW>
__global__ __launch_bounds__(64 * mt_wpb<ARROW>(), ARROW ? EARL_MT_BLOCKS : 1) void minitaur_policy_kernel(const MinitaurPolicyArgs a) {
#include "physics_env_minitaur_rollout.inc"
  static_assert(!RESET && ARROW, "the policy form derives from minitaur_kernel<false, true>");
}

constexpr int MT_DUO_PAIRS = 4;
#ifndef EARL_POLICY_BF16
__global__ __launch_bounds__(128 * MT_DUO_PAIRS, 1) void minitaur_duo_kernel(const MinitaurArgs a) {
#include "physics_env_minitaur_duo.inc"
}
#endif
__global__ __launch_bounds__(128 * MT_DUO_PAIRS, 1) void minitaur_policy_duo_kernel(const MinitaurPolicyArgs a) {
#include "physics_env_minitaur_duo.inc"
}
```

### earl_benchmark_amd/csrc/physics_env_minitaur_duo.inc

```
#pragma clang fp contract(off)
  constexpr bool POLICY = std::is_same<decltype(a), const MinitaurPolicyArgs>::value;
  constexpr int NV = 22, LPE = 32, EPW = 64 / LPE, NP = MT_DUO_PAIRS;
  __shared__ alignas(16) typename ModelOf<NV>::T m;
  __shared__ alignas(16) BlkTable<Lim<NV>::MB, Lim<NV>::KBT> bt;
  __shared__ alignas(16) SharedMT sh[NP * 2 * EPW];
  __shared__ alignas(16) PairTabMT ptab;
  __shared__ int slots_done[NP][2];
  if (threadIdx.x < 2 * NP) (&slots_done[0][0])[threadIdx.x] = 0;
  stage_blocks(bt, a.col);
  stage_kb<NV>(bt, a.m, a.col);
  stage_pairs_mt(ptab, a.col);
  stage_model(m, a.m);
  const earl_minitaur_cfg& cfg = a.cfg;
  const int lane = threadIdx.x & 63, wave = __builtin_amdgcn_readfirstlane(threadIdx.x >> 6), sub = lane % LPE, grp = lane / LPE, n = cfg.n;
  const int pair = wave & (NP - 1);
  const bool role_b = wave >= NP;
  const int NS = cfg.num_substeps, TT = a.T * NS;
  const int gcf = a.st.steps_since_goal_change ? cfg.goal_change_frequency : 0;
  auto env_of = [&](const int q, const int grp_) { return (int)((blockIdx.x * NP + pair) * 2 + q) * EPW + grp_; };
  if (!role_b) {
    for (int q = 0; q < 2; ++q) {
      const int env_raw = env_of(q, grp), env = env_raw < n ? env_raw : n - 1;
      SharedMT& s = sh[(pair * 2 + q) * EPW + grp];
      const double* mp = a.st.motor_param + (size_t)env * 6;
      load_state<NV>(s, m, a.st.qpos + (size_t)env * m.nq, a.st.qvel + (size_t)env * NV, sub);
#ifdef EARL_MT_DEBUG
      if (sub == 0) { s.dbg_env = env < 4096 ? env : 4095; s.dbg_ts = 0; }
#endif
      if (sub < NV) s.xt.ext[sub] = 0.0;
      if (sub < 8) {
        s.ev.oh[sub] = a.st.overheat[(size_t)env * 8 + sub]; s.ev.en[sub] = a.st.motor_enabled[(size_t)env * 8 + sub] != 0 ? 1 : 0;
        s.ev.obs_t[sub] = a.st.observed_torque[(size_t)env * 8 + sub]; s.ev.cmd[sub] = 0.0;
      }
      if (sub == 0) {
        s.xt.mscale[0] = mp[2]; s.xt.mscale[1] = mp[3]; s.xt.mscale[2] = mp[4]; s.xt.foot_mu = mp[5]; s.xt.motor_volt = mp[0]; s.xt.motor_visc = mp[1];
        s.ev.goal[0] = a.st.goal[(size_t)env * 2]; s.ev.goal[1] = a.st.goal[(size_t)env * 2 + 1];
        s.ev.steps = a.st.steps_since_reset ? a.st.steps_since_reset[env] : 0;
        s.ev.sgc = gcf > 0 ? a.st.steps_since_goal_change[env] : 0;
      }
    }
    fence();
  }
  auto finish_step = [&](SharedMT& s, const int env, const bool live, const int t, const int sub, const int grp) {
    const size_t row = (size_t)t * n + env;
    const bool bad_lane = (sub < NV && !(fabs(s.qp[sub]) < EARL_BAD_VALUE && fabs(s.qv[sub]) < EARL_BAD_VALUE)) || (sub < 4 && !(fabs(s.bq[sub]) < EARL_BAD_VALUE));
    const bool failed = group_any<LPE>(bad_lane, grp);
    const int steps = s.ev.steps + 1;
    double goal0 = s.ev.goal[0], goal1 = s.ev.goal[1];
    double v;
    [[maybe_unused]] double rew = 0.0;
    [[maybe_unused]] uint8_t suc = 0;
    if (failed) {
      load_state<NV>(s, m, a.st.qpos + (size_t)env * m.nq, a.st.qvel + (size_t)env * NV, sub);
      if (sub < 8) {
        s.ev.oh[sub] = a.st.overheat[(size_t)env * 8 + sub]; s.ev.en[sub] = a.st.motor_enabled[(size_t)env * 8 + sub] != 0 ? 1 : 0; s.ev.obs_t[sub] = a.st.observed_torque[(size_t)env * 8 + sub];
      }
      if constexpr (POLICY) {
        if (a.out.obs) {
          v = t > 0 ? a.out.obs[(row - n) * 32 + sub] : (a.st.last_obs ? a.st.last_obs[(size_t)env * 32 + sub] : NAN);
          if (live) a.out.obs[row * 32 + sub] = v;
        }
        if (live && sub == 0 && a.st.fail_count) a.st.fail_count[env] += 1;
      } else {
      v = t > 0 ? a.out.obs[(row - n) * 32 + sub] : (a.st.last_obs ? a.st.last_obs[(size_t)env * 32 + sub] : NAN);
      if (live) {
        a.out.obs[row * 32 + sub] = v;
        if (sub == 0) {
          a.out.reward[row] = 0.0; a.out.success[row] = 0;
          if (a.st.fail_count) a.st.fail_count[env] += 1;
        }
      }
      }
      fence();
    } else {
      if (sub < 8) s.kit.obs[16 + sub] = s.ev.obs_t[sub];
      fence();
      if (sub < 8) v = s.qp[cfg.motor_dof[sub]] * cfg.motor_dir[sub];
      else if (sub < 16) v = s.qv[cfg.motor_dof[sub - 8]] * cfg.motor_dir[sub - 8];
      else if (sub < 24) v = s.kit.obs[sub];
      else if (sub < 28) v = s.bq[sub == 27 ? 0 : sub - 23];
      else if (sub < 30) v = s.qp[sub - 28];
      else v = sub == 30 ? goal0 : goal1;
      fence();
      s.kit.obs[sub] = v;
      fence();
      {
        const double qn = renormalised_quat_entry<NV>(s, sub);
        fence();
        if (live) store_state<NV>(s, m, a.st.qpos + (size_t)env * m.nq, a.st.qvel + (size_t)env * NV, sub);
        if (sub < 4) s.bq[sub] = qn;
        fence();
      }
      if (live) {
        if (sub < 8) {
          a.st.overheat[(size_t)env * 8 + sub] = s.ev.oh[sub]; a.st.motor_enabled[(size_t)env * 8 + sub] = s.ev.en[sub] ? 1 : 0; a.st.observed_torque[(size_t)env * 8 + sub] = s.ev.obs_t[sub];
        }
        if constexpr (POLICY) {
          (a.out.obs ? a.out.obs + row * 32 : a.st.last_obs + (size_t)env * 32)[sub] = v;
          if (sub == 0) {
            const double* o = s.kit.obs;
            const double xd = o[28] - goal0, yd = o[29] - goal1;
            double dotp = 0.0;
#pragma unroll
            for (int k = 0; k < 8; ++k) dotp = fma(o[16 + k], o[8 + k], dotp);
            rew = cfg.distance_weight * (-fabs(xd) - fabs(yd)) - cfg.energy_weight * (fabs(dotp) * m.dt);
            suc = sqrt(xd * xd + yd * yd) < cfg.success_radius;
          }
        } else {
        a.out.obs[row * 32 + sub] = v;
        if (sub == 0) {
          const double* o = s.kit.obs;
          const double xd = o[28] - goal0, yd = o[29] - goal1;
          double dotp = 0.0;
#pragma unroll
          for (int k = 0; k < 8; ++k) dotp = fma(o[16 + k], o[8 + k], dotp);
          a.out.reward[row] = cfg.distance_weight * (-fabs(xd) - fabs(yd)) - cfg.energy_weight * (fabs(dotp) * m.dt);
          a.out.success[row] = sqrt(xd * xd + yd * yd) < cfg.success_radius;
        }
        }
      }
    }
    if constexpr (POLICY) {
      if (sub == 0 && live) {
        const double r_t = failed ? 0.0 : rew;
        const uint8_t s_t = failed ? (uint8_t)0 : suc;
        if (a.out.reward) a.out.reward[row] = r_t;
        if (a.out.success) a.out.success[row] = s_t;
        cl_episode_summary(cl_kernarg<MinitaurPolicyArgs>(), t, env, r_t, s_t);
        if (a.out.status) a.out.status[row] = failed ? EARL_STEP_DIVERGED : 0;
        if (a.out.done) a.out.done[row] = (cfg.horizon > 0 && steps >= cfg.horizon) ? 1 : 0;
      }
    } else {
    if (sub == 0 && live) {
      if (a.out.status) a.out.status[row] = failed ? EARL_STEP_DIVERGED : 0;
      a.out.done[row] = (cfg.horizon > 0 && steps >= cfg.horizon) ? 1 : 0;
    }
    }
    if constexpr (POLICY) mt_pair_handover(a, t, env, row, sub, live, failed, suc, goal0, goal1);
    int sgc = s.ev.sgc;
    fence();
    if (gcf > 0 && ++sgc >= gcf) {
      sgc = 0;
      int gi = (int)(mt_draw(cfg, 0xFFFEu, env, cfg.step_counter + (a.clock ? a.clock[1] : 0) + (uint64_t)t) * (double)cfg.n_goals);
      gi = gi >= cfg.n_goals ? cfg.n_goals - 1 : gi;
      goal0 = cfg.goal_table[2 * gi]; goal1 = cfg.goal_table[2 * gi + 1];
      if constexpr (POLICY) {
        if (live && sub >= 30) (a.out.obs ? a.out.obs + row * 32 : a.st.last_obs + (size_t)env * 32)[sub] = sub == 30 ? goal0 : goal1;
      } else
      if (live && sub >= 30) a.out.obs[row * 32 + sub] = sub == 30 ? goal0 : goal1;
      if (live && sub == 0) { a.st.goal[(size_t)env * 2] = goal0; a.st.goal[(size_t)env * 2 + 1] = goal1; }
    }
    if (sub == 0) { s.ev.steps = steps; s.ev.sgc = sgc; s.ev.goal[0] = goal0; s.ev.goal[1] = goal1; }
    __builtin_amdgcn_fence(__ATOMIC_SEQ_CST, "agent");
    fence();
  };
#ifdef EARL_PHYS_PROF
  const unsigned long long duo_t0 = __builtin_readcyclecounter();
  unsigned long long duo_wait = 0;
#endif
  for (int j = 0; j <= 2 * TT + 1; ++j) {
#ifdef EARL_PHYS_PROF
    const unsigned long long slot_t0 = __builtin_readcyclecounter();
#endif
    if (!role_b) {
      int lane_ = lane;
      asm volatile("" : "+v"(lane_));
      const int sub = lane_ % LPE, grp = lane_ / LPE;
      const int q = j & 1, ts = j >> 1, t = ts / NS, k = ts - t * NS;
      const int env_raw = env_of(q, grp), env = env_raw < n ? env_raw : n - 1;
      const bool live = env_raw < n;
      SharedMT& s = sh[(pair * 2 + q) * EPW + grp];
      if (ts > 0) {
        const bool isroot = sub < 6, ishinge = sub >= 8 && sub < 24, isl = isroot || ishinge;
        const int l = isroot ? sub : (ishinge ? sub - 2 : NV - 1);
        const double al = s.aprev[l], qd = s.qv[l], ql = s.qp[l];
        const Q4 Qb = ldq(s.bq);
        integrate_mt(s, m, sub, isl, l, m.dt, al, qd, ql, Qb);
      }
      if (k == 0) {
        if (t > 0) finish_step(s, env, live, t - 1, sub, grp);
        if (t < a.T) {
          double a64[8];
          mt_step_action<POLICY>(a, t, n, env, sub, live, a64);
          if (sub < 8) s.ev.cmd[sub] = earl::mt_leg_to_motor(a64, sub);
        }
      }
      if (ts < TT) {
        if (sub < 8) {
          int ml = sub;
          asm volatile("" : "+v"(ml));
          const int mdof = cfg.motor_dof[ml & 7];
          const double mdir = cfg.motor_dir[ml & 7], lim = m.dt * cfg.motor_velocity_limit;
          const double qm = s.qp[mdof] * mdir, qdm = s.qv[mdof] * mdir;
          const double c = earl::mt_clipd(s.ev.cmd[sub], qm - lim, qm + lim);
          double act, obs;
          earl::mt_motor_torque(cfg.motor_kp, cfg.motor_kd, s.xt.motor_volt, s.xt.motor_visc, false, c, qm, qdm, act, obs);
          const int oh = fabs(act) > cfg.overheat_torque ? s.ev.oh[sub] + 1 : 0;
          int en = s.ev.en[sub];
          if (oh > cfg.overheat_steps) en = 0;
          s.ev.oh[sub] = oh; s.ev.en[sub] = en; s.ev.obs_t[sub] = obs;
          s.xt.ext[mdof] = en ? act * mdir : 0.0;
        }
        fence();
        int sub_ = sub;
        asm volatile("" : "+v"(sub_));
        __builtin_assume(sub_ >= 0 && sub_ < LPE);
        substep_mt<true, 1>(s, m, bt, ptab, sub_, grp, k > 0, nullptr);
      }
    } else if (j >= 1) {
      const int jj = j - 1, q = jj & 1, ts = jj >> 1;
      if (ts < TT) {
        SharedMT& s = sh[(pair * 2 + q) * EPW + grp];
        int sub_ = sub;
        asm volatile("" : "+v"(sub_));
        __builtin_assume(sub_ >= 0 && sub_ < LPE);
        substep_mt<true, 2>(s, m, bt, ptab, sub_, grp, (ts % NS) > 0, nullptr);
      }
    }
#ifdef EARL_PHYS_PROF
    const unsigned long long slot_t1 = __builtin_readcyclecounter();
#endif
    {
      __builtin_amdgcn_fence(__ATOMIC_RELEASE, "workgroup");
      volatile int* mine = &slots_done[pair][role_b ? 1 : 0];
      volatile int* other = &slots_done[pair][role_b ? 0 : 1];
      if (lane == 0) *mine = j + 1;
      while (*other < j + 1) __builtin_amdgcn_s_sleep(4);
      __builtin_amdgcn_fence(__ATOMIC_ACQUIRE, "workgroup");
    }
#ifdef EARL_PHYS_PROF
    PCOUNT(26, slot_t1 - slot_t0); PCOUNT(27, __builtin_readcyclecounter() - slot_t1); PCOUNT(28, 1);
    duo_wait += __builtin_readcyclecounter() - slot_t1;
#endif
  }
#ifdef EARL_PHYS_PROF
  if (lane == 0 && blockIdx.x * 2 * NP + wave < 2048) {
    g_wave_cycles[blockIdx.x * 2 * NP + wave] = __builtin_readcyclecounter() - duo_t0;
    g_wave_cycles[2048 + blockIdx.x * 2 * NP + wave] = duo_wait;
  }
#endif
  if (!role_b) {
    for (int q = 0; q < 2; ++q) {
      const int env_raw = env_of(q, grp), env = env_raw < n ? env_raw : n - 1;
      SharedMT& s = sh[(pair * 2 + q) * EPW + grp];
      if (env_raw < n) {
        if (sub == 0) {
          if (a.st.steps_since_reset) a.st.steps_since_reset[env] = s.ev.steps;
          if (gcf > 0) a.st.steps_since_goal_change[env] = s.ev.sgc;
        }
        if constexpr (POLICY) {
          if (a.out.obs && a.st.last_obs && a.T > 0) a.st.last_obs[(size_t)env * 32 + sub] = a.out.obs[((size_t)(a.T - 1) * n + env) * 32 + sub];
        } else
        if (a.st.last_obs && a.T > 0) a.st.last_obs[(size_t)env * 32 + sub] = a.out.obs[((size_t)(a.T - 1) * n + env) * 32 + sub];
      }
    }
  }
```

### earl_benchmark_amd/csrc/physics_launch.h

```cpp
#pragma once

extern "C" __attribute__((visibility("hidden"))) int earl_unit_table_cone(const void* col, void* stream);
extern "C" __attribute__((visibility("hidden"))) void earl_unit_l64_physics(const void* pargs, int nv, int integrate, void* stream);
extern "C" __attribute__((visibility("hidden"))) void earl_unit_l64_sawyer_rollout(const void* sawyer_args, int nv, void* stream);
extern "C" __attribute__((visibility("hidden"))) void earl_unit_kitchen_physics(const void* pargs, int integrate, void* stream);
extern "C" __attribute__((visibility("hidden"))) void earl_unit_kitchen_policy_rollout(const void* kitchen_policy_args, void* stream);
extern "C" __attribute__((visibility("hidden"))) int earl_unit_w8_sawyer_rollout(const void* sawyer_args, void* stream);
extern "C" __attribute__((visibility("hidden"))) int earl_unit_w8_sawyer_policy_rollout(const void* sawyer_policy_args, void* stream);
extern "C" __attribute__((visibility("hidden"))) int earl_unit_bf16_sawyer_policy_rollout(const void* sawyer_policy_args, int nv, int sliced, void* stream);
extern "C" __attribute__((visibility("hidden"))) int earl_unit_w8_bf16_sawyer_policy_rollout(const void* sawyer_policy_args, void* stream);
extern "C" __attribute__((visibility("hidden"))) int earl_unit_mt_bf16_policy_rollout(const void* minitaur_policy_args, int duo, void* stream);
extern "C" __attribute__((visibility("hidden"))) void earl_unit_kitchen_bf16_policy_rollout(const void* kitchen_policy_args, void* stream);
extern "C" __attribute__((visibility("hidden"))) int earl_unit_branch_replicate(const void* sawyer_branch_args, const void* src_state, int nv, void* stream);
extern "C" __attribute__((visibility("hidden"))) int earl_unit_branch_sawyer_rollout(const void* sawyer_branch_args, int nv, int sliced, void* stream);
extern "C" __attribute__((visibility("hidden"))) int earl_unit_branch_w8_sawyer_rollout(const void* sawyer_branch_args, void* stream);
extern "C" __attribute__((visibility("hidden"))) int earl_unit_branch_value_sawyer_rollout(const void* sawyer_branch_value_args, int nv, int sliced, void* stream);
extern "C" __attribute__((visibility("hidden"))) int earl_unit_branch_value_w8_sawyer_rollout(const void* sawyer_branch_value_args, void* stream);
extern "C" __attribute__((visibility("hidden"))) int earl_unit_branch_prior_sawyer_rollout(const void* sawyer_branch_prior_args, int nv, int sliced, void* stream);
extern "C" __attribute__((visibility("hidden"))) int earl_unit_branch_prior_w8_sawyer_rollout(const void* sawyer_branch_prior_args, void* stream);
extern "C" int earl_sawyer_rollout_door_w8(const earl_link_model* model, const earl_collision_model* col, const earl_sawyer_cfg* cfg, const earl_sawyer_state* st,
                                           const float* action, int32_t T, const earl_sawyer_out* out, earl_stream_t stream);

namespace {

int launched(const char* what) {
  const hipError_t e = hipGetLastError();
  if (e != hipSuccess) {
    fprintf(stderr, "earl_physics: %s: %s\n", what, hipGetErrorString(e));
    return EARL_ERR_LAUNCH;
  }
  return EARL_OK;
}

int check_cone(const earl_collision_model* col, const bool want_elliptic, hipStream_t st, const char* what) {
  if (!col) return EARL_OK;
  const int cone = earl_unit_table_cone(col, st);
  if (cone < 0) return EARL_OK;
  if (cone != (want_elliptic ? 1 : 0)) {
    fprintf(stderr, "earl_physics: %s: the collision table is compiled for the %s friction cone, this model size runs the %s one (earl_collision_model.cone)\n", what,
            cone == 1 ? "elliptic" : "pyramidal", want_elliptic ? "elliptic" : "pyramidal");
    return EARL_ERR_ARG;
  }
  return EARL_OK;
}

int cu_count() {
  int dev = 0, cus = 256;
  if (hipGetDevice(&dev) == hipSuccess) (void)hipDeviceGetAttribute(&cus, hipDeviceAttributeMultiprocessorCount, dev);
  return cus;
}

int g_solo = -1;
int solo_mode(int n) {
  if (g_solo >= 0) return g_solo;
  const int cus = cu_count();
  return n <= cus ? 2 : (n <= 4 * cus ? 1 : 0);
}
int solo_grid(int n, int solo, int wpb) { return solo == 2 ? n : (solo == 1 ? (n + wpb - 1) / wpb : (n + 2 * wpb - 1) / (2 * wpb)); }

template <int NV, int LPE> int grid_for(int n) { constexpr int epb = (64 / LPE) * Lim<NV>::WPB; return (n + epb - 1) / epb; }
template <int NV> constexpr int block_for() { return 64 * Lim<NV>::WPB; }

#ifdef EARL_PHYS_PROF
template <int = 0> int prof_set_wave(int block, int thread) {
  const int v[2] = {block, thread};
  return hipMemcpyToSymbol(HIP_SYMBOL(g_prof_sel), v, sizeof(v)) == hipSuccess ? EARL_OK : EARL_ERR_LAUNCH;
}
template <int = 0> int prof_read_wave_cycles(unsigned long long* out) {
  return hipMemcpyFromSymbol(out, HIP_SYMBOL(g_wave_cycles), sizeof(unsigned long long) * 4096) == hipSuccess ? EARL_OK : EARL_ERR_LAUNCH;
}
template <int = 0> int prof_read_phases(unsigned long long* out, int reset) {
  if (hipMemcpyFromSymbol(out, HIP_SYMBOL(g_phys_prof), sizeof(unsigned long long) * 32) != hipSuccess) return EARL_ERR_LAUNCH;
  if (reset) {
    unsigned long long z[32] = {0};
    if (hipMemcpyToSymbol(HIP_SYMBOL(g_phys_prof), z, sizeof(z)) != hipSuccess) return EARL_ERR_LAUNCH;
  }
  return EARL_OK;
}
#endif

}
```

### earl_benchmark_amd/csrc/physics_mt.hip

```cpp
#include "minitaur_device.h"
#include "physics_stepper.h"
#include "policy_check.h"
#include "policy_math.h"

namespace {
#include "minitaur_stepper.h"
#include "physics_env_minitaur.h"
}

#include "physics_launch.h"

namespace {

int g_mt_stepper = 1;
int g_mt_duo = EARL_MT_DUO_DEFAULT;

bool mt_use_duo(int n) {
  const int cus = cu_count();
  const long rounds_one = (n + 8L * cus - 1) / (8L * cus), rounds_two = (n + 16L * cus - 1) / (16L * cus);
  return 16 * rounds_two < 10 * rounds_one;
}

enum class MtForm { Generic, Duo, Tree };
MtForm minitaur_form(int n, int solo, int num_substeps) {
  if (!g_mt_stepper) return MtForm::Generic;
  return solo == 0 && num_substeps > 0 && (g_mt_duo > 0 || (g_mt_duo < 0 && mt_use_duo(n))) ? MtForm::Duo : MtForm::Tree;
}
bool minitaur_args_ok(const earl_minitaur_cfg* cfg, const earl_minitaur_state* st) {
  if (cfg->n < 0 || !cfg->goal_table || cfg->n_goals < 1) return false;
  if (!st->qpos || !st->qvel || !st->goal || !st->motor_param || !st->observed_torque || !st->overheat || !st->motor_enabled) return false;
  return cfg->goal_change_frequency <= 0 || st->steps_since_goal_change;
}

}

extern "C" {

int earl_minitaur_rollout_clocked(const void* model24, const earl_collision_model* col, const earl_minitaur_cfg* cfg, const earl_minitaur_state* st,
                                  const float* action, int32_t T, const uint64_t* clock, const earl_minitaur_out* out, earl_stream_t stream) {
  if (!model24 || !cfg || !st || !out || !action || T < 0 || !minitaur_args_ok(cfg, st)) return EARL_ERR_ARG;
  if (!out->obs || !out->reward || !out->done || !out->success || cfg->num_substeps < 0) return EARL_ERR_ARG;
  if (cfg->n == 0 || T == 0) return EARL_OK;
  if (int rc = check_cone(col, false, (hipStream_t)stream, "minitaur_rollout")) return rc;
  MinitaurArgs a{model24, col, *cfg, *st, *out, action, T, nullptr, nullptr, solo_mode(cfg->n), clock};
  const MtForm form = minitaur_form(cfg->n, a.solo, cfg->num_substeps);
  if (form == MtForm::Duo) {
    minitaur_duo_kernel<<<(unsigned)((cfg->n + 16 * MT_DUO_PAIRS / 4 - 1) / (4 * MT_DUO_PAIRS)), 128 * MT_DUO_PAIRS, 0, (hipStream_t)stream>>>(a);
    return launched("minitaur_rollout (two waves per SIMD)");
  }
  if (form == MtForm::Tree) minitaur_kernel<false, true><<<solo_grid(cfg->n, a.solo, EARL_MT_WPB), 64 * EARL_MT_WPB, 0, (hipStream_t)stream>>>(a);
  else minitaur_kernel<false, false><<<solo_grid(cfg->n, a.solo, Lim<22>::WPB), block_for<22>(), 0, (hipStream_t)stream>>>(a);
  return launched("minitaur_rollout");
}
static int minitaur_closed_loop(const void* model24, const earl_collision_model* col, const earl_minitaur_cfg* cfg, const earl_minitaur_state* st,
                                const earl_mlp_policy* policy, const earl_policy_population* pop, const earl_agent_pair* pair, bool paired, const earl_backward_goals* goals,
                                const earl_gaussian_head* head, const double* obs0, int32_t T, const uint64_t* clock, float* actions, const earl_minitaur_out* out,
                                const earl_episode_summary* summary, earl_stream_t stream) {
  if (!model24 || !cfg || !st || !out || !policy || !obs0 || T < 0 || !minitaur_args_ok(cfg, st) || cfg->num_substeps < 0) return EARL_ERR_ARG;
  if (!out->obs && !st->last_obs) return EARL_ERR_ARG;
  if (paired && !pair) return EARL_ERR_ARG;
  if (earl::contract::check_closed_loop(*policy, 32, 8, earl::contract::kParamsAligned16 | earl::contract::kBoundedOutput | earl::contract::kBf16Params, head, pop, cfg->env_offset, cfg->n,
                                        paired ? pair : nullptr, cfg->goal_change_frequency, goals, cfg->n_goals, nullptr))
    return EARL_ERR_ARG;
  if (!g_mt_stepper) return EARL_ERR_ARG;
  if (cfg->n == 0 || T == 0) return EARL_OK;
  if (int rc = check_cone(col, false, (hipStream_t)stream, "minitaur_policy_rollout")) return rc;
  MinitaurPolicyArgs a;
  static_cast<MinitaurArgs&>(a) = MinitaurArgs{model24, col, *cfg, *st, *out, nullptr, T, nullptr, nullptr, solo_mode(cfg->n), clock};
  fill_closed_loop(a, *policy, head, obs0, actions, pop, summary, paired ? pair : nullptr, goals, nullptr, 0);
  const bool duo = minitaur_form(cfg->n, a.solo, cfg->num_substeps) == MtForm::Duo;
  if (policy->precision == EARL_PRECISION_BF16) return earl_unit_mt_bf16_policy_rollout(&a, duo ? 1 : 0, stream);
  if (duo) {
    minitaur_policy_duo_kernel<<<(unsigned)((cfg->n + 16 * MT_DUO_PAIRS / 4 - 1) / (4 * MT_DUO_PAIRS)), 128 * MT_DUO_PAIRS, 0, (hipStream_t)stream>>>(a);
    return launched("minitaur_policy_rollout (two waves per SIMD)");
  }
  minitaur_policy_kernel<false, true><<<solo_grid(cfg->n, a.solo, EARL_MT_WPB), 64 * EARL_MT_WPB, 0, (hipStream_t)stream>>>(a);
  return launched("minitaur_policy_rollout");
}
int earl_minitaur_population_rollout(const void* model24, const earl_collision_model* col, const earl_minitaur_cfg* cfg, const earl_minitaur_state* st,
                                     const earl_mlp_policy* policy, const earl_policy_population* pop, const earl_gaussian_head* head, const double* obs0, int32_t T,
                                     const uint64_t* clock, float* actions, const earl_minitaur_out* out, const earl_episode_summary* summary, earl_stream_t stream) {
  return minitaur_closed_loop(model24, col, cfg, st, policy, pop, nullptr, false, nullptr, head, obs0, T, clock, actions, out, summary, stream);
}
int earl_minitaur_agents_rollout(const void* model24, const earl_collision_model* col, const earl_minitaur_cfg* cfg, const earl_minitaur_state* st,
                                 const earl_mlp_policy* policy, const earl_agent_pair* pair, const earl_policy_population* pop, const earl_backward_goals* goals,
                                 const earl_gaussian_head* head, const double* obs0, int32_t T, const uint64_t* clock, float* actions, const earl_minitaur_out* out,
                                 const earl_episode_summary* summary, earl_stream_t stream) {
  return minitaur_closed_loop(model24, col, cfg, st, policy, pop, pair, true, goals, head, obs0, T, clock, actions, out, summary, stream);
}
int earl_minitaur_policy_rollout(const void* model24, const earl_collision_model* col, const earl_minitaur_cfg* cfg, const earl_minitaur_state* st,
                                 const earl_mlp_policy* policy, const earl_gaussian_head* head, const double* obs0, int32_t T, const uint64_t* clock, float* actions,
                                 const earl_minitaur_out* out, earl_stream_t stream) {
  if (!actions || !out || !out->obs || !out->reward || !out->done || !out->success) return EARL_ERR_ARG;
  return earl_minitaur_population_rollout(model24, col, cfg, st, policy, nullptr, head, obs0, T, clock, actions, out, nullptr, stream);
}
int earl_minitaur_rollout(const void* model24, const earl_collision_model* col, const earl_minitaur_cfg* cfg, const earl_minitaur_state* st,
                          const float* action, int32_t T, const earl_minitaur_out* out, earl_stream_t stream) {
  return earl_minitaur_rollout_clocked(model24, col, cfg, st, action, T, nullptr, out, stream);
}
int earl_minitaur_reset(const void* model24, const earl_collision_model* col, const earl_minitaur_cfg* cfg, const earl_minitaur_state* st,
                        const uint8_t* mask, double* obs, earl_stream_t stream) {
  if (!model24 || !cfg || !st || !minitaur_args_ok(cfg, st) || !cfg->reset_qpos || cfg->settle_steps < 0) return EARL_ERR_ARG;
  if (cfg->n == 0) return EARL_OK;
  if (int rc = check_cone(col, false, (hipStream_t)stream, "minitaur_reset")) return rc;
  MinitaurArgs a{model24, col, *cfg, *st, earl_minitaur_out{nullptr, nullptr, nullptr, nullptr, nullptr}, nullptr, 0, mask, obs, solo_mode(cfg->n), nullptr};
  if (g_mt_stepper) minitaur_kernel<true, true><<<solo_grid(cfg->n, a.solo, EARL_MT_WPB), 64 * EARL_MT_WPB, 0, (hipStream_t)stream>>>(a);
  else minitaur_kernel<true, false><<<solo_grid(cfg->n, a.solo, Lim<22>::WPB), block_for<22>(), 0, (hipStream_t)stream>>>(a);
  return launched("minitaur_reset");
}
int earl_minitaur_cfg_size(void) { return (int)sizeof(earl_minitaur_cfg); }
int earl_debug_set_solo_mt(int mode) {
  const int prev = g_solo;
  if (mode >= -1 && mode <= 2) g_solo = mode;
  return prev;
}
int earl_debug_set_minitaur_stepper(int tree) {
  if (tree != 0 && tree != 1) return EARL_ERR_ARG;
  g_mt_stepper = tree;
  return EARL_OK;
}
int earl_debug_set_minitaur_duo(int mode) {
  const int prev = g_mt_duo;
  if (mode >= -1 && mode <= 1) g_mt_duo = mode;
  return prev;
}
#ifdef EARL_MT_DEBUG
int earl_debug_read_mt_dbg(int* out_i, double* out_d) {
  if (hipMemcpyFromSymbol(out_i, HIP_SYMBOL(g_mt_dbg), sizeof(int) * 4096 * 8 * 32) != hipSuccess) return EARL_ERR_LAUNCH;
  if (hipMemcpyFromSymbol(out_d, HIP_SYMBOL(g_mt_dbg_al), sizeof(double) * 4096 * 8 * 32) != hipSuccess) return EARL_ERR_LAUNCH;
  if (hipMemcpyFromSymbol(out_d + 4096 * 8 * 32, HIP_SYMBOL(g_mt_dbg_x), sizeof(double) * 5 * 4096 * 8 * 32) != hipSuccess) return EARL_ERR_LAUNCH;
  return hipMemcpyFromSymbol(out_d + 6 * 4096 * 8 * 32, HIP_SYMBOL(g_mt_dbg_ph), sizeof(double) * 8 * 4096 * 8 * 32) == hipSuccess ? EARL_OK : EARL_ERR_LAUNCH;
}
#endif
#ifdef EARL_PHYS_PROF
int earl_debug_set_prof_wave_mt(int block, int thread) { return prof_set_wave(block, thread); }
int earl_debug_read_wave_cycles_mt(unsigned long long* out) { return prof_read_wave_cycles(out); }
int earl_debug_read_phys_profile_mt(unsigned long long* out, int reset) { return prof_read_phases(out, reset); }
#endif

}
```

### earl_benchmark_amd/csrc/physics_stepper.h

```cpp
#include <hip/hip_runtime.h>

#include <cstdio>
#include <type_traits>

#include "../../include/earl_physics.h"
#include "../../include/earl_glue.h"
#include "philox.h"

#ifndef EARL_PHYS_NO_CONTRACT
#pragma clang fp contract(fast)
#endif

namespace {

#ifdef EARL_PHYS_PROF
__device__ unsigned long long g_phys_prof[32];
__device__ int g_prof_sel[2];
#define PROF_ME (blockIdx.x == g_prof_sel[0] && threadIdx.x == g_prof_sel[1])
#define PSTAMP(i)                                                                          \
  do {                                                                                     \
    const unsigned long long t_ = __builtin_readcyclecounter();                            \
    if (PROF_ME) g_phys_prof[i] += t_ - p_last;                                            \
    p_last = t_;                                                                           \
  } while (0)
// ... 1591 lines not shown
          const double x = p >= 0 ? (dp * gl - o * gp) * r : gl * r;
          *((isl && l >= NA) ? &s.con.rc[l] : reinterpret_cast<double*>(s.bank_pad)) = x;
        }
        solve_lead_regs<NV, NA>(Hs, [&](int i) { return s.con.dl[i]; }, a);
        fence();
#pragma unroll
        for (int i = NA; i < NV; ++i) a[i] = s.con.rc[i];
      }
    } else if constexpr (Lim<NV>::CONNECT) {
#if EARL_MT_LOOP_SOLVER
      if (isl) s.con.rc[l] += s.con.rl[l];
      chol_coop_loop<NV>(s.con.Hc, s.con.dl, l, isl);
      solve_lds_loop<NV>(s.con.Hc, s.con.rc);
      fence();
#pragma unroll
      for (int i = 0; i < NV; ++i) a[i] = s.con.rc[i];
#else
      {
        const double xl = chol_solve_rows<NV>(s.con.Hc, s.con.dl, s.con.rc[l] + s.con.rl[l], l, isl, grp);
        fence();
        if (isl) s.con.rc[l] = xl;
        fence();
#pragma unroll
        for (int i = 0; i < NV; ++i) a[i] = s.con.rc[i];
      }
#endif
    } else if constexpr (Lim<NV>::COOP) {
      chol_coop<NV>(s.con.Hc, s.con.dl, l, isl);
      solve_lds<NV>(s.con.Hc, a);
    } else if constexpr (NA == NV) {
      load_tri<NV, NV>(L, s.con.Hc, [&](int i) { return s.con.dl[i]; });
      chol_regs<NV, NV, (NV > 10)>(L);
      solve_regs<NV, NV>(L, a);
    } else if (coupled) {
#ifdef EARL_PEG_COUPLED_LDS
      chol_coop<NV>(s.con.Hc, s.con.dl, l, isl);
      solve_lds<NV>(s.con.Hc, a);
#else
      solve_schur_regs<NV, NA>(s.con.Hc, [&](int i) { return s.con.dl[i]; }, a);
#endif
    } else {
      load_tri<NV, NA>(L, s.con.Hc, [&](int i) { return s.con.dl[i]; });
      chol_regs<NV, NA, (NV > 10)>(L);
      solve_regs<NV, NA>(L, a);
    }
    KSTAMP(18);
    double al = 0;
#pragma unroll
    for (int i = 0; i < NV; ++i) al = l == i ? a[i] : al;
    const bool want = lim_inst && ((lim_lo ? al : -al) - lim_aref < 0);
    bool changed = want != act;
    act = frozen ? act : want;
    if constexpr (Lim<NV>::EXTRAS) {
      if (fr_loss > 0) {
        const double x = al - fr_aref;
        const int ns = fabs(x) * fr_D <= fr_loss ? 0 : (x > 0 ? 1 : -1);
        changed = changed || ns != fr_state;
        fr_state = ns;
      }
    }
    if (ncmax > 0) {
      const int c = sub < MC ? sub : MC - 1;
      double an = 0, at1 = 0, at2 = 0;
      if constexpr (TS < NT) {
        if (ctA) {
          double cj[3 * TS];
#pragma unroll
          for (int j = 0; j < TS; ++j) { cj[3 * j] = s.con.CJ[c][0][j]; cj[3 * j + 1] = s.con.CJ[c][1][j]; cj[3 * j + 2] = s.con.CJ[c][2][j]; }
          pin_batch(cj);
#pragma unroll
          for (int j = 0; j < TS; ++j) { an = fma(cj[3 * j], a[j], an); at1 = fma(cj[3 * j + 1], a[j], at1); at2 = fma(cj[3 * j + 2], a[j], at2); }
        }
        if (ctP) {
          double cj[3 * (NV - TS)];
#pragma unroll
          for (int j = TS; j < NV; ++j) { cj[3 * (j - TS)] = s.con.CJ[c][0][j]; cj[3 * (j - TS) + 1] = s.con.CJ[c][1][j]; cj[3 * (j - TS) + 2] = s.con.CJ[c][2][j]; }
          pin_batch(cj);
#pragma unroll
          for (int j = TS; j < NV; ++j) { an = fma(cj[3 * (j - TS)], a[j], an); at1 = fma(cj[3 * (j - TS) + 1], a[j], at1); at2 = fma(cj[3 * (j - TS) + 2], a[j], at2); }
        }
      } else if constexpr (Lim<NV>::EXTRAS) {
        double row[NV];
#pragma unroll
        for (int j = 0; j < NV; ++j) row[j] = s.con.CJ[c][0][j];
        pin_batch(row);
#pragma unroll
        for (int j = 0; j < NV; ++j) an = fma(row[j], a[j], an);
#pragma unroll
        for (int j = 0; j < NV; ++j) row[j] = s.con.CJ[c][1][j];
        pin_batch(row);
#pragma unroll
        for (int j = 0; j < NV; ++j) at1 = fma(row[j], a[j], at1);
#pragma unroll
        for (int j = 0; j < NV; ++j) row[j] = s.con.CJ[c][2][j];
        pin_batch(row);
#pragma unroll
        for (int j = 0; j < NV; ++j) at2 = fma(row[j], a[j], at2);
      } else {
#pragma unroll
        for (int j = 0; j < NV; ++j) {
          an = fma(s.con.CJ[c][0][j], a[j], an); at1 = fma(s.con.CJ[c][1][j], a[j], at1); at2 = fma(s.con.CJ[c][2][j], a[j], at2);
        }
      }
      unsigned int nb = 0;
      if constexpr (Lim<NV>::ELLIPTIC) {
        nb = sub < nct ? (unsigned int)cone_zone(an - car[0], at1 - car[1], at2 - car[2], cmu) : 0u;
        const double big = fmax(fmax(fabs(cja[0]), fabs(cja[1])), fabs(cja[2])), dif = fmax(fmax(fabs(an - cja[0]), fabs(at1 - cja[1])), fabs(at2 - cja[2]));
        changed = changed || nb != cact || (nb == 2u && dif > 1e-8 * (1.0 + big));
        if (!frozen) { cja[0] = an; cja[1] = at1; cja[2] = at2; }
        nb = frozen ? cact : nb;
      } else {
      nb |= (an + cmu * at1 - car[0] < 0) ? 1u : 0u;
      nb |= (an - cmu * at1 - car[1] < 0) ? 2u : 0u;
      nb |= (an + cmu * at2 - car[2] < 0) ? 4u : 0u;
      nb |= (an - cmu * at2 - car[3] < 0) ? 8u : 0u;
      nb = sub < nct ? nb : 0u;
      changed = changed || nb != cact;
      }
      cact = nb;
    }
    if constexpr (Lim<NV>::ELLIPTIC) {
      const bool env_changed = group_any<LPE>(changed, grp);
      if (!frozen && !env_changed) {
        if (isl) s.aprev[l] = al;
        frozen = true;
      }
      changed = !frozen;
    }
    fence();
    KSTAMP(19);
    if (!__any(changed)) break;
  }
  if constexpr (Lim<NV>::ELLIPTIC) {
    if (!frozen && isl) {
      double al = 0;
#pragma unroll
      for (int i = 0; i < NV; ++i) al = l == i ? a[i] : al;
      s.aprev[l] = al;
    }
    fence();
#pragma unroll
    for (int i = 0; i < NV; ++i) a[i] = s.aprev[i];
  }
  if constexpr (INTEGRATE) {
    double al = 0;
#pragma unroll
    for (int i = 0; i < NV; ++i) al = l == i ? a[i] : al;
    if (isl) s.aprev[l] = al;
  }
#ifdef EARL_PHYS_PROF
  {
    const unsigned long long dk = __builtin_readcyclecounter() - k9_t0;
    PCOUNT(coupled ? 27 : 28, dk);
#ifdef EARL_PHYS_PROF_ALL
    PCOUNT_ALL(29, 1); PCOUNT_ALL(30, coupled ? 1 : 0); PCOUNT_ALL(31, coupled ? dk : 0);
#endif
  }
#endif
  PSTAMP(8);
  if constexpr (!INTEGRATE) {
    double al = 0;
#pragma unroll
    for (int i = 0; i < NV; ++i) al = l == i ? a[i] : al;
    if (qacc_out && isl) qacc_out[l] = al;
    if (efc_out) {
      fence();
      if (isl) {
#pragma unroll
        for (int r = 0; r < 6; ++r) s.con.J6[r][l] = Jc[r];
      }
      fence();
      if (sub < 6) {
        double Ja = 0;
#pragma unroll
        for (int j = 0; j < NV; ++j) Ja = fma(s.con.J6[sub][j], a[j], Ja);
        efc_out[sub] = -s.con.wD[sub] * (Ja - s.con.war[sub]);
      }
      if (isl) {
        const double f = act ? -lim_D * ((lim_lo ? al : -al) - lim_aref) : 0.0;
        efc_out[6 + 2 * l] = lim_lo ? f : 0.0;
        efc_out[7 + 2 * l] = lim_lo ? 0.0 : f;
      }
    }
  } else {
    if constexpr (Lim<NV>::DAMPED) {
    {
      double acc = 0;
      if constexpr (Lim<NV>::EXTRAS) {
        double mc[NV];
#pragma unroll
        for (int j = 0; j < NV; ++j) mc[j] = s.M.sym(j, l, ltri);
        pin_batch(mc);
#pragma unroll
        for (int j = 0; j < NV; ++j) acc = fma(mc[j], a[j], acc);
      } else {
#pragma unroll
      for (int j = 0; j < NV; ++j) acc = fma(s.M.sym(j, l, ltri), a[j], acc);
      }
      if (isl) s.con.rc[l] = acc;
    }
    fence();
#pragma unroll
    for (int i = 0; i < NV; ++i) a[i] = s.con.rc[i];
    if constexpr (Lim<NV>::EXTRAS) pin_batch(a);
    if constexpr (R_OWNER) {
      constexpr int NL = NA * (NA + 1) / 2;
      __syncthreads();
      const double* const kf = peer->hwst.Hw.v;
      double Lk[NL], y[NA];
#pragma unroll
      for (int e = 0; e < NL; ++e) Lk[e] = kf[e];
      const int lf = l >= NA ? l : NA;
      const double ki = kf[NL + lf - NA];
      pin_batch(Lk);
      double gl = 0;
#pragma unroll
      for (int i = NA; i < NV; ++i) gl = i == lf ? a[i] : gl;
      *((isl && l >= NA) ? &s.con.rc[l] : reinterpret_cast<double*>(s.bank_pad)) = gl * ki;
#pragma unroll
      for (int i = 0; i < NA; ++i) y[i] = a[i];
      solve_regs<NA, NA>(Lk, y);
#pragma unroll
      for (int i = 0; i < NA; ++i) a[i] = y[i];
      fence();
#pragma unroll
      for (int i = NA; i < NV; ++i) a[i] = s.con.rc[i];
    } else {
    if (isl) s.con.dl[l] = dt * m.damping[l];
    fence();
    if constexpr (Lim<NV>::EXTRAS) {
      {
        const int lf = l >= NA ? l : NA;
        double gl = 0;
#pragma unroll
        for (int i = NA; i < NV; ++i) gl = i == lf ? a[i] : gl;
        *((isl && l >= NA) ? &s.con.rc[l] : reinterpret_cast<double*>(s.bank_pad)) = gl * rcp_nr(s.M.lo(lf, lf) + s.con.dl[lf]);
      }
      solve_lead_regs<NV, NA>(s.M, [&](int i) { return s.con.dl[i]; }, a);
      fence();
#pragma unroll
      for (int i = NA; i < NV; ++i) a[i] = s.con.rc[i];
    } else if constexpr (Lim<NV>::COOP) {
      chol_coop<NV>(s.M, s.con.dl, l, isl);
      solve_lds<NV>(s.M, a);
    } else {
      load_tri<NV, NA>(L, s.M, [&](int i) { return s.con.dl[i]; });
      chol_regs<NV, NA, (NV > 10)>(L);
      solve_regs<NV, NA>(L, a);
    }
    }
    }
    double al = 0;
#pragma unroll
    for (int i = 0; i < NV; ++i) al = l == i ? a[i] : al;
    fence();
    if (isl) {
      const double nv_ = s.qv[l] + dt * al;
      s.qv[l] = nv_;
      s.qp[l] = s.qp[l] + dt * nv_;
    }
    fence();
    if (m.ball_dof >= 0) {
      const int bd = m.ball_dof;
      const V3 wb{s.qv[bd], s.qv[bd + 1], s.qv[bd + 2]};
      Q4 q0 = ldq(s.bq);
      const double n0 = rsq_nr(q0.w * q0.w + q0.x * q0.x + q0.y * q0.y + q0.z * q0.z);
      q0 = Q4{q0.w * n0, q0.x * n0, q0.y * n0, q0.z * n0};
      const double w2 = dot(wb, wb);
      const double iw = w2 > 0 ? rsq_nr(w2 > 0 ? w2 : 1.0) : 0.0;
      double sn, cs;
      sincos_mod(0.5 * dt * (w2 * iw), sn, cs);
      Q4 q1 = qmul(q0, Q4{cs, sn * wb.x * iw, sn * wb.y * iw, sn * wb.z * iw});
      const double n1 = rsq_nr(q1.w * q1.w + q1.x * q1.x + q1.y * q1.y + q1.z * q1.z);
      fence();
      if (sub == 0) { s.bq[0] = q1.w * n1; s.bq[1] = q1.x * n1; s.bq[2] = q1.y * n1; s.bq[3] = q1.z * n1; }
      fence();
    }
    PSTAMP(11);
  }
}

template <int NV>
__device__ __forceinline__ V3 attachment(const Shared<NV>& s, const typename ModelOf<NV>::T& m, const int k) {
  const int la = m.att_link[k];
  V3 p = ld3(m.att_pos[k]);
  if (la >= 0) {
    double R[3][3];
    qmat(ldq(s.Xq[la]), R);
    p = add(ld3(s.Xp[la]), mulv(R, p));
  }
  return p;
}

template <typename MT>
__device__ __forceinline__ void stage_model(MT& dst, const void* __restrict__ src) {
  static_assert(sizeof(MT) % 8 == 0, "copied as 8-byte words");
  const unsigned long long* g = reinterpret_cast<const unsigned long long*>(src);
  unsigned long long* d = reinterpret_cast<unsigned long long*>(&dst);
  for (int i = threadIdx.x; i < (int)(sizeof(MT) / 8); i += blockDim.x) d[i] = g[i];
  __syncthreads();
}

template <int NV, typename SH>
__device__ __forceinline__ void load_state(SH& s, const typename ModelOf<NV>::T& m, const double* __restrict__ qrow, const double* __restrict__ vrow, const int sub) {
  const int bd = m.ball_dof;
  if (sub < NV) {
    s.qp[sub] = (bd < 0 || sub < bd) ? qrow[sub] : (sub > bd + 2 ? qrow[sub + 1] : 0.0);
    s.qv[sub] = vrow[sub];
    s.aprev[sub] = 0.0;
  }
  if (sub < 4) {
    double v = sub == 0 ? 1.0 : 0.0;
    if (bd >= 0) {
      const Q4 q = ldq(qrow + bd);
      v = qrow[bd + sub] * rsq_nr(q.w * q.w + q.x * q.x + q.y * q.y + q.z * q.z);
    }
    s.bq[sub] = v;
  }
}
template <int NV, typename SH>
__device__ __forceinline__ double renormalised_quat_entry(const SH& s, const int sub) {
  const Q4 q = ldq(s.bq);
  return s.bq[sub < 4 ? sub : 0] * rsq_nr(q.w * q.w + q.x * q.x + q.y * q.y + q.z * q.z);
}
template <int NV, typename SH>
__device__ __forceinline__ void store_state(const SH& s, const typename ModelOf<NV>::T& m, double* __restrict__ qrow, double* __restrict__ vrow, const int sub) {
  const int bd = m.ball_dof;
  if (sub < NV) {
    if (bd < 0 || sub < bd) qrow[sub] = s.qp[sub];
    else if (sub > bd + 2) qrow[sub + 1] = s.qp[sub];
    vrow[sub] = s.qv[sub];
  }
  if (bd >= 0 && sub < 4) qrow[bd + sub] = s.bq[sub];
}

struct PArgs {
  const void* m;
  const earl_collision_model* col;
  int n, nsub;
  double* qpos; double* qvel;
  const double* mocap_pos; const double* mocap_quat; const double* ctrl;
  double* att_xpos; double* qacc_out; double* efc_out;
  int ctrl_stride;
  int mq_stride;
};

template <int NV, int LPE, bool INTEGRATE>
__global__ __launch_bounds__(64 * Lim<NV>::WPB) void physics_kernel(const PArgs a) {
  constexpr int EPW = 64 / LPE, WPB = Lim<NV>::WPB;
  __shared__ alignas(16) typename ModelOf<NV>::T m;
  __shared__ alignas(16) BlkTable<Lim<NV>::MB, Lim<NV>::KBT> bt;
  __shared__ alignas(16) Shared<NV> sh[EPW * WPB];
  stage_blocks(bt, a.col);
  stage_kb<NV>(bt, a.m, a.col);
  stage_model(m, a.m);
  const int lane = threadIdx.x & 63, wave = __builtin_amdgcn_readfirstlane(threadIdx.x >> 6), sub = lane % LPE, grp = lane / LPE;
  const int env_raw = (blockIdx.x * WPB + wave) * EPW + grp;
  const bool live = env_raw < a.n;
  const int env = live ? env_raw : a.n - 1;
  Shared<NV>& s = sh[wave * EPW + grp];
  load_state<NV>(s, m, a.qpos + (size_t)env * m.nq, a.qvel + (size_t)env * NV, sub);
  if constexpr (Lim<NV>::NT < NV || Lim<NV>::TS < Lim<NV>::NT) {
    for (int k = sub; k < (int)(sizeof(s.M.v) / sizeof(double)); k += LPE) s.M.v[k] = 0.0;
  }
  if constexpr (Lim<NV>::EXTRAS) {
    for (int k = sub; k < (int)(sizeof(s.hwst.Hw.v) / sizeof(double)); k += LPE) s.hwst.Hw.v[k] = 0.0;
  }
  if (sub < 3) s.mocap[sub] = a.mocap_pos[(size_t)env * 3 + sub];
  fence();
  const Q4 mq = ldq(a.mocap_quat + (size_t)env * a.mq_stride);
  double ctrl[EARL_MAXACT] = {0, 0, 0, 0};
  for (int ac = 0; ac < m.n_act; ++ac) ctrl[ac] = a.ctrl[(size_t)env * (a.ctrl_stride ? a.ctrl_stride : m.n_act) + ac];
  constexpr int NC = 6 + 2 * NV;
  for (int ts = 0; ts < a.nsub; ++ts)
    substep<NV, LPE, INTEGRATE>(s, m, bt, a.col, sub, grp, mq, ctrl, INTEGRATE && ts > 0, (a.qacc_out && live) ? a.qacc_out + (size_t)env * NV : nullptr,
                                (a.efc_out && live) ? a.efc_out + (size_t)env * NC : nullptr);
  if constexpr (INTEGRATE) {
    if (live) store_state<NV>(s, m, a.qpos + (size_t)env * m.nq, a.qvel + (size_t)env * NV, sub);
  }
  if (a.att_xpos && sub < m.n_att && live) {
    const V3 p = attachment<NV>(s, m, sub);
    double* o = a.att_xpos + ((size_t)env * m.n_att + sub) * 3;
    o[0] = p.x; o[1] = p.y; o[2] = p.z;
  }
}

template <int LPE>
__device__ __forceinline__ bool group_any(const bool pred, const int grp) {
  const unsigned long long bal = __ballot(pred);
  if constexpr (LPE == 64) return bal != 0ull;
  else return ((bal >> (grp * (LPE & 63))) & ((1ull << (LPE & 63)) - 1ull)) != 0ull;
}

}
```

### include/earl_physics.h

```cpp
#ifndef EARL_PHYSICS_H
#define EARL_PHYSICS_H
#include <stdint.h>

#include "earl_tabletop.h"

#ifdef __cplusplus
extern "C" {
#endif

#define EARL_MAXV 16
#define EARL_MAXATT 8
#define EARL_MAXACT 4

typedef struct earl_link_model {
  int32_t nv, n_att, n_act, weld_att;
  int32_t n_jump;
  int32_t ball_dof;
  int32_t nq, pad_;
  int32_t jump[4][EARL_MAXV];
  int32_t parent[EARL_MAXV];
  int32_t jtype[EARL_MAXV];
  int32_t limited[EARL_MAXV];
  uint32_t anc_mask[EARL_MAXV];
  uint32_t desc_mask[EARL_MAXV];
// ... 88 lines not shown
  int32_t att_hand, att_right, att_left, att_obj;
  int32_t obj_dof;
  int32_t obj_kind;
  int32_t n_goal_rows;
  int32_t goal_change_frequency;
  int32_t n_wide;
  int32_t att_grasp, att_lpad, att_rpad;
  int32_t pad2_;
  double action_scale;
  double mocap_low[3], mocap_high[3], mocap_quat[4];
  double success_radius;
  double hand_init_pos[3], obj_init_pos[3];
  double obj_init_angle, angle_noise[2];
  double obj_low[3], obj_high[3], obj_reject_xy[2], obj_reject_radius;
  const double* goal_table;
  const double* wide_table;
  double wide_shift[3], wide_noise;
  double init_tcp[3];
  double box_corners[4][3];
  uint64_t seed, counter;
  uint64_t step_counter;
} earl_sawyer_cfg;

typedef struct earl_sawyer_state {
  double* qpos;
  double* qvel;
  double* mocap_pos;
  double* goal;
  int32_t* steps_since_reset;
  int32_t* steps_since_goal_change;
  double* obj_init;
  double* last_obs;
  int32_t* fail_count;
  int32_t* sched;
} earl_sawyer_state;

typedef struct earl_sawyer_out {
  double* obs;
  float* reward;
  uint8_t* done;
  uint8_t* success;
  uint8_t* status;
  double* info;
} earl_sawyer_out;
#define EARL_SAWYER_INFO 8
#define EARL_INFO_SUCCESS 0
#define EARL_INFO_NEAR_OBJECT 1
#define EARL_INFO_GRASP_SUCCESS 2
#define EARL_INFO_GRASP_REWARD 3
#define EARL_INFO_IN_PLACE_REWARD 4
#define EARL_INFO_OBJ_TO_TARGET 5
#define EARL_INFO_UNSCALED_REWARD 6
#define EARL_BAD_VALUE 1e10
#define EARL_STEP_DIVERGED 1

int earl_sawyer_rollout(const earl_link_model* model, const earl_collision_model* col, int32_t nv, const earl_sawyer_cfg* cfg, const earl_sawyer_state* st,
                        const float* action, int32_t T, const earl_sawyer_out* out, earl_stream_t stream);
int earl_sawyer_rollout_clocked(const earl_link_model* model, const earl_collision_model* col, int32_t nv, const earl_sawyer_cfg* cfg, const earl_sawyer_state* st,
                                const float* action, int32_t T, const uint64_t* clock, const earl_sawyer_out* out, earl_stream_t stream);

int earl_sawyer_policy_rollout(const earl_link_model* model, const earl_collision_model* col, int32_t nv, const earl_sawyer_cfg* cfg, const earl_sawyer_state* st,
                               const earl_mlp_policy* policy, const earl_gaussian_head* head, const double* obs0, int32_t T, const uint64_t* clock, float* actions,
                               const earl_sawyer_out* out, earl_stream_t stream);
int earl_sawyer_population_rollout(const earl_link_model* model, const earl_collision_model* col, int32_t nv, const earl_sawyer_cfg* cfg, const earl_sawyer_state* st,
                                   const earl_mlp_policy* policy, const earl_policy_population* pop, const earl_gaussian_head* head, const double* obs0, int32_t T,
                                   const uint64_t* clock, float* actions, const earl_sawyer_out* out, const earl_episode_summary* summary, earl_stream_t stream);
int earl_sawyer_pair_rollout(const earl_link_model* model, const earl_collision_model* col, int32_t nv, const earl_sawyer_cfg* cfg, const earl_sawyer_state* st,
                             const earl_mlp_policy* policy, const earl_agent_pair* pair, const earl_gaussian_head* head, const double* obs0, int32_t T,
                             const uint64_t* clock, float* actions, const earl_sawyer_out* out, earl_stream_t stream);
typedef struct earl_backward_goals {
  const double* table;
  int32_t  n_rows;
  int32_t  pad_;
  int32_t* row;
  int32_t* row_out;
} earl_backward_goals;
int earl_sawyer_agents_rollout(const earl_link_model* model, const earl_collision_model* col, int32_t nv, const earl_sawyer_cfg* cfg, const earl_sawyer_state* st,
                               const earl_mlp_policy* policy, const earl_agent_pair* pair, const earl_policy_population* pop, const earl_backward_goals* goals,
                               const earl_gaussian_head* head, const double* obs0, int32_t T, const uint64_t* clock, float* actions, const earl_sawyer_out* out,
                               const earl_episode_summary* summary, earl_stream_t stream);

typedef struct earl_sawyer_branch_ws {
  void*   base;
  int64_t bytes;
} earl_sawyer_branch_ws;
int earl_sawyer_branch_ws_bytes(int32_t nv, int32_t K, int32_t n, int64_t* bytes);
int earl_sawyer_branch_rollout(const earl_link_model* model, const earl_collision_model* col, int32_t nv, const earl_sawyer_cfg* cfg, const earl_sawyer_state* st,
                               int32_t K, int32_t H, const float* act, int64_t act_branch_stride, const uint64_t* clock, const earl_sawyer_branch_ws* ws,
                               const earl_episode_summary* summary, double* last_obs, int32_t* fail, earl_stream_t stream);

typedef struct earl_sawyer_plan_params {
  int32_t K;
  int32_t H;
  int32_t iterations;
  int32_t iteration0;
  float sigma[4];
  uint32_t noise_counter;
  double inv_temperature;
} earl_sawyer_plan_params;
#define EARL_SAWYER_PLAN_MAX_K 8192
int earl_sawyer_plan_ws_bytes(int32_t nv, int32_t K, int32_t H, int32_t n, int64_t* bytes);
int earl_sawyer_plan_mppi(const earl_link_model* model, const earl_collision_model* col, int32_t nv, const earl_sawyer_cfg* cfg, const earl_sawyer_state* st,
                          const earl_sawyer_plan_params* params, const float* mean, float* plan, double* ret, double* ret0, double* best_ret, int32_t* best_k,
                          int32_t* fail, const uint64_t* clock, const earl_sawyer_branch_ws* ws, earl_stream_t stream);
int earl_sawyer_plan_candidates(const earl_sawyer_cfg* cfg, const earl_sawyer_plan_params* params, int32_t j, const float* mean, float* act_out, earl_stream_t stream);
int32_t earl_sawyer_plan_candidates_cpu(const earl_sawyer_cfg* cfg, const earl_sawyer_plan_params* params, int32_t j, const float* mean, float* act_out);
int32_t earl_sawyer_plan_update_cpu(const earl_sawyer_cfg* cfg, const earl_sawyer_plan_params* params, int32_t j, const float* mean, const float* act, const double* ret,
                                    float* plan, double* ret0_row, double* best_ret, int32_t* best_k);

#define EARL_SAWYER_CEM_MAX_E 1024
typedef struct earl_sawyer_cem_params {
  int32_t K, H, iterations, iteration0;
  int32_t elites;
  float sigma[4];
  uint32_t noise_counter;
  float alpha;
  float std_min, std_max;
} earl_sawyer_cem_params;
int earl_sawyer_plan_cem(const earl_link_model* model, const earl_collision_model* col, int32_t nv, const earl_sawyer_cfg* cfg, const earl_sawyer_state* st,
                         const earl_sawyer_cem_params* params, const float* mean, const float* std0, float* plan, float* std, double* ret, double* ret0,
                         double* best_ret, int32_t* best_k, uint8_t* elite, int32_t* fail, const uint64_t* clock, const earl_sawyer_branch_ws* ws, earl_stream_t stream);
int earl_sawyer_cem_candidates(const earl_sawyer_cfg* cfg, const earl_sawyer_cem_params* params, int32_t j, const float* mean, const float* std, float* act_out,
                               earl_stream_t stream);
int earl_sawyer_cem_update(const earl_sawyer_cfg* cfg, const earl_sawyer_cem_params* params, int32_t j, const float* mean, const float* std_in, const float* act,
                           const double* ret, float* plan, float* std, double* ret0_row, double* best_ret, int32_t* best_k, uint8_t* elite, earl_stream_t stream);
int32_t earl_sawyer_cem_candidates_cpu(const earl_sawyer_cfg* cfg, const earl_sawyer_cem_params* params, int32_t j, const float* mean, const float* std, float* act_out);
int32_t earl_sawyer_cem_update_cpu(const earl_sawyer_cfg* cfg, const earl_sawyer_cem_params* params, int32_t j, const float* mean, const float* std_in, const float* act,
                                   const double* ret, float* plan, float* std, double* ret0_row, double* best_ret, int32_t* best_k, uint8_t* elite);

int earl_sawyer_value_ws_bytes(int32_t nv, int32_t K, int32_t H, int32_t n, int64_t* bytes);
int earl_sawyer_branch_rollout_value(const earl_link_model* model, const earl_collision_model* col, int32_t nv, const earl_sawyer_cfg* cfg, const earl_sawyer_state* st,
                                     int32_t K, int32_t H, const float* act, int64_t act_branch_stride, const uint64_t* clock, const earl_plan_value* pv,
                                     const earl_sawyer_branch_ws* ws, const earl_episode_summary* summary, double* last_obs, int32_t* fail, earl_stream_t stream);
int earl_sawyer_plan_mppi_value(const earl_link_model* model, const earl_collision_model* col, int32_t nv, const earl_sawyer_cfg* cfg, const earl_sawyer_state* st,
                                const earl_sawyer_plan_params* params, const earl_plan_value* pv, const float* mean, float* plan, double* ret, double* ret0,
                                double* best_ret, int32_t* best_k, int32_t* fail, const uint64_t* clock, const earl_sawyer_branch_ws* ws, earl_stream_t stream);
int earl_sawyer_plan_cem_value(const earl_link_model* model, const earl_collision_model* col, int32_t nv, const earl_sawyer_cfg* cfg, const earl_sawyer_state* st,
                               const earl_sawyer_cem_params* params, const earl_plan_value* pv, const float* mean, const float* std0, float* plan, float* std, double* ret,
                               double* ret0, double* best_ret, int32_t* best_k, uint8_t* elite, int32_t* fail, const uint64_t* clock, const earl_sawyer_branch_ws* ws,
                               earl_stream_t stream);
int32_t earl_sawyer_value_terminal_cpu(const earl_plan_value* pv, int32_t H, int32_t rows, const double* last_obs, double* ret);

typedef struct earl_sawyer_plan_prior {
  const earl_mlp_policy* policy;
  int32_t branches;
  float sigma[4];
  const double* obs0;
  float* act;
} earl_sawyer_plan_prior;
int earl_sawyer_prior_ws_bytes(int32_t nv, int32_t K, int32_t H, int32_t n, int64_t* bytes);
int earl_sawyer_branch_rollout_prior(const earl_link_model* model, const earl_collision_model* col, int32_t nv, const earl_sawyer_cfg* cfg, const earl_sawyer_state* st,
                                     int32_t K, int32_t H, float* act, int64_t act_branch_stride, const uint64_t* clock, const earl_plan_value* pv,
                                     const earl_sawyer_plan_prior* prior, int32_t j, uint32_t noise_counter, const earl_sawyer_branch_ws* ws,
                                     const earl_episode_summary* summary, double* last_obs, int32_t* fail, earl_stream_t stream);
int earl_sawyer_plan_mppi_prior(const earl_link_model* model, const earl_collision_model* col, int32_t nv, const earl_sawyer_cfg* cfg, const earl_sawyer_state* st,
                                const earl_sawyer_plan_params* params, const earl_plan_value* pv, const earl_sawyer_plan_prior* prior, const float* mean, float* plan,
                                double* ret, double* ret0, double* best_ret, int32_t* best_k, int32_t* fail, const uint64_t* clock, const earl_sawyer_branch_ws* ws,
                                earl_stream_t stream);
int earl_sawyer_plan_cem_prior(const earl_link_model* model, const earl_collision_model* col, int32_t nv, const earl_sawyer_cfg* cfg, const earl_sawyer_state* st,
                               const earl_sawyer_cem_params* params, const earl_plan_value* pv, const earl_sawyer_plan_prior* prior, const float* mean, const float* std0,
                               float* plan, float* std, double* ret, double* ret0, double* best_ret, int32_t* best_k, uint8_t* elite, int32_t* fail, const uint64_t* clock,
                               const earl_sawyer_branch_ws* ws, earl_stream_t stream);
int32_t earl_sawyer_prior_actions_cpu(const earl_sawyer_cfg* cfg, const earl_sawyer_plan_prior* prior, int32_t H, int32_t k, int32_t j, uint32_t noise_counter, int32_t cem,
                                      const double* obs, float* act);

int32_t earl_mlp_policy_forward_cpu(const earl_mlp_policy* policy, const earl_gaussian_head* head, int32_t n, const float* obs, const float* eps, float* actions);
float earl_tanh_f32(float x);
float earl_exp_f32(float x);
float earl_normal_quantile_f32(uint32_t k24);

int earl_sawyer_reset(const earl_link_model* model, int32_t nv, const earl_sawyer_cfg* cfg, const earl_sawyer_state* st,
                      const double* reset_qpos, const double* reset_qvel, const uint8_t* mask, double* obs,
                      earl_stream_t stream);

int earl_sawyer_observe(const earl_link_model* model, int32_t nv, const earl_sawyer_cfg* cfg, const earl_sawyer_state* st,
                        double* obs, earl_stream_t stream);

int earl_sawyer_door_reward(const earl_sawyer_cfg* cfg, int32_t n, const double* obs, float* reward, uint8_t* success,
                            earl_stream_t stream);
int earl_sawyer_door_info(const earl_sawyer_cfg* cfg, int32_t n, const double* obs, const uint8_t* status, double* info, earl_stream_t stream);

int earl_physics_forget_table(const void* col);
int earl_debug_set_physics_lanes(int lanes_per_env);

struct earl_kitchen_params;
typedef struct earl_kitchen_cfg {
  int32_t n, env_offset;
  int32_t horizon;
  int32_t frame_skip;
  int32_t sensor_noise;
  int32_t n_att;
  int32_t site_att[8];
  uint64_t seed, counter;
  const double* mocap_quat_dev;
} earl_kitchen_cfg;
typedef struct earl_kitchen_state {
  double* qpos; double* qvel;
  double* mocap_pos;
  double* goal;
  double* last_qp_robot;
  double* att_xpos;
  int32_t* steps_since_reset;
  int32_t* fail_count;
  double* last_obs;
  double* action64;
  double* ctrl9;
  double* noise;
  double* qpos_bak; double* qvel_bak;
  double* sites;
  uint8_t* bad;
  double* mocap_bak;
  double* att_bak;
} earl_kitchen_state;
typedef struct earl_kitchen_out {
  double* obs;
  double* reward;
  uint8_t* done; uint8_t* success;
  uint8_t* status;
} earl_kitchen_out;
int earl_kitchen_step(const void* model24, const earl_collision_model* col, const struct earl_kitchen_params* params, const earl_kitchen_cfg* cfg,
                      const earl_kitchen_state* st, const float* action , const earl_kitchen_out* out, earl_stream_t stream);

int earl_kitchen_rollout(const void* model24, const earl_collision_model* col, const struct earl_kitchen_params* params, const earl_kitchen_cfg* cfg,
                         const earl_kitchen_state* st, const float* action , int32_t T, const earl_kitchen_out* out, earl_stream_t stream);
int earl_kitchen_rollout_clocked(const void* model24, const earl_collision_model* col, const struct earl_kitchen_params* params, const earl_kitchen_cfg* cfg,
                                 const earl_kitchen_state* st, const float* action , int32_t T, const uint64_t* clock, const earl_kitchen_out* out,
                                 earl_stream_t stream);
int earl_kitchen_policy_rollout(const void* model24, const earl_collision_model* col, const struct earl_kitchen_params* params, const earl_kitchen_cfg* cfg,
                                const earl_kitchen_state* st, const earl_mlp_policy* policy, const earl_gaussian_head* head, const double* obs0, int32_t T,
                                const uint64_t* clock, float* actions, const earl_kitchen_out* out, earl_stream_t stream);
int earl_kitchen_population_rollout(const void* model24, const earl_collision_model* col, const struct earl_kitchen_params* params, const earl_kitchen_cfg* cfg,
                                    const earl_kitchen_state* st, const earl_mlp_policy* policy, const earl_policy_population* pop, const earl_gaussian_head* head,
                                    const double* obs0, int32_t T, const uint64_t* clock, float* actions, const earl_kitchen_out* out,
                                    const earl_episode_summary* summary, earl_stream_t stream);
int earl_kitchen_agents_rollout(const void* model24, const earl_collision_model* col, const struct earl_kitchen_params* params, const earl_kitchen_cfg* cfg,
                                const earl_kitchen_state* st, const earl_mlp_policy* policy, const earl_agent_pair* pair, const earl_policy_population* pop,
                                const earl_backward_goals* goals, const double* forward_goals, int32_t n_forward_goals, const earl_gaussian_head* head, const double* obs0,
                                int32_t T, const uint64_t* clock, float* actions, const earl_kitchen_out* out, const earl_episode_summary* summary, earl_stream_t stream);

typedef struct earl_minitaur_cfg {
  int32_t n, env_offset;
  int32_t horizon;
  int32_t num_substeps;
  int32_t settle_steps;
  int32_t randomize;
  int32_t n_goals;
  int32_t goal_change_frequency;
  int32_t overheat_steps;
  int32_t motor_dof[8];
  int32_t pad_;
  double motor_dir[8];
  double motor_kp, motor_kd;
  double motor_velocity_limit;
  double overheat_torque;
  double distance_weight, energy_weight;
  double success_radius;
  const double* goal_table;
  const double* reset_qpos;
  double base_mass_err[2];
  double leg_mass_err[2];
  double leg_mass, motor_mass;
  double foot_friction[2];
  uint64_t seed, counter;
  uint64_t step_counter;
} earl_minitaur_cfg;
typedef struct earl_minitaur_state {
  double* qpos;
  double* qvel;
  double* goal;
  double* motor_param;
  double* observed_torque;
  int32_t* overheat;
  uint8_t* motor_enabled;
  int32_t* steps_since_reset;
  int32_t* steps_since_goal_change;
  int32_t* fail_count;
  double* last_obs;
} earl_minitaur_state;
typedef struct earl_minitaur_out {
  double* obs;
  double* reward;
  uint8_t* done; uint8_t* success;
  uint8_t* status;
} earl_minitaur_out;
int earl_minitaur_rollout(const void* model24, const earl_collision_model* col, const earl_minitaur_cfg* cfg, const earl_minitaur_state* st,
                          const float* action, int32_t T, const earl_minitaur_out* out, earl_stream_t stream);
int earl_minitaur_rollout_clocked(const void* model24, const earl_collision_model* col, const earl_minitaur_cfg* cfg, const earl_minitaur_state* st,
                                  const float* action, int32_t T, const uint64_t* clock, const earl_minitaur_out* out, earl_stream_t stream);
int earl_minitaur_policy_rollout(const void* model24, const earl_collision_model* col, const earl_minitaur_cfg* cfg, const earl_minitaur_state* st,
                                 const earl_mlp_policy* policy, const earl_gaussian_head* head, const double* obs0, int32_t T, const uint64_t* clock, float* actions,
                                 const earl_minitaur_out* out, earl_stream_t stream);
int earl_minitaur_population_rollout(const void* model24, const earl_collision_model* col, const earl_minitaur_cfg* cfg, const earl_minitaur_state* st,
                                     const earl_mlp_policy* policy, const earl_policy_population* pop, const earl_gaussian_head* head, const double* obs0, int32_t T,
                                     const uint64_t* clock, float* actions, const earl_minitaur_out* out, const earl_episode_summary* summary, earl_stream_t stream);
int earl_minitaur_agents_rollout(const void* model24, const earl_collision_model* col, const earl_minitaur_cfg* cfg, const earl_minitaur_state* st,
                                 const earl_mlp_policy* policy, const earl_agent_pair* pair, const earl_policy_population* pop, const earl_backward_goals* goals,
                                 const earl_gaussian_head* head, const double* obs0, int32_t T, const uint64_t* clock, float* actions, const earl_minitaur_out* out,
                                 const earl_episode_summary* summary, earl_stream_t stream);
int earl_minitaur_reset(const void* model24, const earl_collision_model* col, const earl_minitaur_cfg* cfg, const earl_minitaur_state* st,
                        const uint8_t* mask, double* obs, earl_stream_t stream);
int earl_minitaur_cfg_size(void);
int earl_debug_set_minitaur_stepper(int tree);
int earl_debug_set_minitaur_duo(int mode);
int earl_debug_set_solo(int mode);
int earl_debug_set_solo_mt(int mode);

int earl_debug_set_door_variant(int variant);
int earl_debug_set_peg_schedule(int sliced);
int earl_debug_set_sawyer_prior_launches(int launches);

int earl_physics_model_size(void);
int earl_physics_model24_size(void);
int earl_collision_model_size(void);
int earl_sawyer_cfg_size(void);

#ifdef __cplusplus
}
#endif
#endif
```

Measured before the change: 77.60 billion.

## Add conflict-free LDS layout variant for minitaur stepper kernels

Builds a second compilation unit of the minitaur kernels that pads contact records to 80 bytes and reorders the Schur weight rows to remove LDS bank conflicts, with compile-time checks of conflict degree. In one role it also moves the pair collision test ahead of the dynamics phase and parks the per-DOF values in LDS so they survive it, and it adds small scalar/vector register hints. It becomes the default dispatch for the non-generic forms, at the cost of extra LDS per environment and a second kernel build.

```diff
diff --git a/earl_benchmark_amd/_abi.py b/earl_benchmark_amd/_abi.py
--- a/earl_benchmark_amd/_abi.py
+++ b/earl_benchmark_amd/_abi.py
@@ -318,6 +318,7 @@
     'earl_minitaur_cfg_size': [],
     'earl_debug_set_minitaur_stepper': [C.c_int],
     'earl_debug_set_minitaur_duo': [C.c_int],
+    'earl_debug_set_minitaur_layout': [C.c_int],
     'earl_debug_set_solo': [C.c_int],
     'earl_debug_set_solo_mt': [C.c_int],
     'earl_sawyer_reset': [C.c_void_p, C.c_int32, _P(SawyerCfg), _P(SawyerState)] + [C.c_void_p] * 5,
diff --git a/earl_benchmark_amd/csrc/minitaur_stepper.h b/earl_benchmark_amd/csrc/minitaur_stepper.h
--- a/earl_benchmark_amd/csrc/minitaur_stepper.h
+++ b/earl_benchmark_amd/csrc/minitaur_stepper.h
@@ -85,8 +85,56 @@
   }
 }
 
+enum class LdsOp { ReadB32, ReadB64, ReadB128, WriteB32, WriteB64, WriteB128 };
+struct LdsLaneAddr { int a[32]; };
+constexpr int lds_conflict_degree(const LdsOp op, const LdsLaneAddr& at) {
+  const bool rd = op == LdsOp::ReadB32 || op == LdsOp::ReadB64 || op == LdsOp::ReadB128;
+  const int dwords = (op == LdsOp::ReadB32 || op == LdsOp::WriteB32) ? 1 : ((op == LdsOp::ReadB64 || op == LdsOp::WriteB64) ? 2 : 4);
+  const int banks = (rd && dwords > 1) ? 64 : 32;
+  const unsigned int g128[2] = {0x0FF0F00Fu, 0xF00F0FF0u};
+  const int ngroups = op == LdsOp::ReadB128 ? 2 : (op == LdsOp::WriteB64 ? 2 : (op == LdsOp::WriteB128 ? 4 : 1));
+  int worst = 0;
+  for (int g = 0; g < ngroups; ++g) {
+    const unsigned int members = op == LdsOp::ReadB128 ? g128[g] : (op == LdsOp::WriteB64 ? 0xFFFFu << (16 * g) : (op == LdsOp::WriteB128 ? 0xFFu << (8 * g) : 0xFFFFFFFFu));
+    int count[64] = {};
+    int seen[32] = {};
+    int nseen = 0;
+    for (int k = 0; k < 32; ++k) {
+      if (!(members >> k & 1u) || at.a[k] < 0) continue;
+      const int a = at.a[k] / 4;
+      bool dup = false;
+      for (int q = 0; q < nseen; ++q) dup = dup || seen[q] == a;
+      if (dup) continue;
+      seen[nseen++] = a;
+      for (int d = 0; d < dwords; ++d) {
+        const int b = (a + d) % banks;
+        count[b] += 1;
+        worst = count[b] > worst ? count[b] : worst;
+      }
+    }
+  }
+  return worst;
+}
+constexpr int lds_conflict_degree(const LdsOp op, const int offset, const int stride, const unsigned int lanes, const bool dof_map = false) {
+  LdsLaneAddr at{};
+  for (int k = 0; k < 32; ++k) at.a[k] = (lanes >> k & 1u) ? offset + stride * (dof_map ? (k < 6 ? k : k - 2) : k) : -1;
+  return lds_conflict_degree(op, at);
+}
+constexpr unsigned int MT_LANES_ALL = 0xFFFFFFFFu, MT_LANES_CONTACT = (1u << MTDims::MC) - 1u, MT_LANES_DOF = 0x00FFFF3Fu, MT_LANES_SOLVE = 0x00FFFFFFu;
+static_assert(lds_conflict_degree(LdsOp::ReadB32, 0, 4, MT_LANES_ALL) == 1 && lds_conflict_degree(LdsOp::ReadB64, 0, 8, MT_LANES_ALL) == 1 &&
+              lds_conflict_degree(LdsOp::ReadB128, 0, 16, MT_LANES_ALL) == 1, "consecutive reads are conflict-free");
+static_assert(lds_conflict_degree(LdsOp::ReadB32, 0, 128, MT_LANES_ALL) == 32 && lds_conflict_degree(LdsOp::ReadB64, 0, 256, MT_LANES_ALL) == 32, "a stride of all banks");
+static_assert(lds_conflict_degree(LdsOp::ReadB128, 0, 32, MT_LANES_ALL) == 2 && lds_conflict_degree(LdsOp::ReadB128, 0, 32, 0x00000FFFu) == 1, "16-byte reads, 32 bytes apart");
+static_assert(lds_conflict_degree(LdsOp::WriteB128, 0, 64, MT_LANES_ALL) == 4 && lds_conflict_degree(LdsOp::WriteB64, 0, 8, MT_LANES_ALL) == 1 &&
+              lds_conflict_degree(LdsOp::WriteB32, 0, 8, MT_LANES_ALL) == 2, "stores: groups of 8 / 16 / 32 lanes on 32 banks");
+
 struct SharedMTData {
   static constexpr int NV = MTDims::NV, MC = MTDims::MC;
+#ifdef EARL_MT_LDS_V2
+  static constexpr int CTS = 10;
+#else
+  static constexpr int CTS = 8;
+#endif
   double qp[NV], qv[NV];
   double bq[4];
   double aprev[NV];
@@ -99,8 +147,8 @@
   int dbg_env, dbg_ts, dbg_pad[2];
 #endif
   union {
-    double ct[MC][8];
-    double cw[MC][8];
+    double ct[MC][CTS];
+    double cw[MC][CTS];
   };
   double CJr[MC][3][6];
   double CJh[MC][3][2];
@@ -125,7 +173,13 @@
       double HB[MTDims::NH][6];
       double HR[6][6];
       double rc[NV];
+#ifdef EARL_MT_LDS_V2
+      double Wl[2][24][2];
+#define MT_WL(s, i, p) (s).pas.Wl[((p) >> 1) & 1][((p) >> 2) * 6 + (i)][(p) & 1]
+#else
       double Wl[6][16];
+#define MT_WL(s, i, p) (s).pas.Wl[i][p]
+#endif
       double part[6][4];
       double Y[16];
       double LL[MTDims::NLEG][10];
@@ -137,6 +191,38 @@
 static_assert(sizeof(((SharedMTData*)nullptr)->ev) % 16 == 0 && sizeof(((SharedMTData*)nullptr)->c3) % 16 == 0 && sizeof(((SharedMTData*)nullptr)->tb) % 16 == 0 && offsetof(SharedMTData, dyn) % 16 == 0, "16-byte alignment of the blocks the kernels read as b128");
 static_assert(offsetof(SharedMTData, hand.sh_keep) == offsetof(SharedMTData, dyn.Sh) && offsetof(SharedMTData, hand.Aw) == offsetof(SharedMTData, dyn.redI) &&
               sizeof(((SharedMTData*)nullptr)->hand) <= sizeof(((SharedMTData*)nullptr)->dyn), "the hand-over block keeps clear of the motion subspaces and fits the dynamics block");
+#ifdef EARL_MT_LDS_V2
+#define MT_DEG(op, stride, lanes) (lds_conflict_degree(op, 0, stride, lanes) > lds_conflict_degree(op, 16, stride, lanes) ? lds_conflict_degree(op, 0, stride, lanes) : lds_conflict_degree(op, 16, stride, lanes))
+static_assert(sizeof(((SharedMTData*)nullptr)->ct[0]) == 80, "80-byte contact records and weight rows");
+static_assert(MT_DEG(LdsOp::ReadB128, 80, MT_LANES_CONTACT) == 1 && MT_DEG(LdsOp::WriteB128, 80, MT_LANES_CONTACT) == 1, "ct, cw: lane = contact, b128 (rows of 64 bytes before: reads 2-way, stores 4-way)");
+constexpr int mt_wl_byte(const bool v2, const int i, const int p) { return v2 ? (((p >> 1) & 1) * 48 + ((p >> 2) * 6 + i) * 2 + (p & 1)) * 8 : (i * 16 + p) * 8; }
+constexpr LdsLaneAddr mt_wl_store(const bool v2, const int half) {
+  LdsLaneAddr at{};
+  for (int t = 0; t < 32; ++t) at.a[t] = t < 24 ? mt_wl_byte(v2, t % 6, 4 * (t / 6) + 2 * half) : -1;
+  return at;
+}
+constexpr LdsLaneAddr mt_wl_schur(const bool v2, const bool row_c, const int chunk) {
+  LdsLaneAddr at{};
+  for (int t = 0; t < 32; ++t) {
+    const int e = t < 21 ? t : 20;
+    const int i = e >= 15 ? 5 : (e >= 10 ? 4 : (e >= 6 ? 3 : (e >= 3 ? 2 : (e >= 1 ? 1 : 0))));
+    at.a[t] = mt_wl_byte(v2, row_c ? e - i * (i + 1) / 2 : i, 2 * chunk);
+  }
+  return at;
+}
+constexpr int mt_wl_worst(const bool v2) {
+  int w = 0;
+  for (int h = 0; h < 2; ++h) { const int d = lds_conflict_degree(LdsOp::WriteB128, mt_wl_store(v2, h)); w = d > w ? d : w; }
+  for (int q = 0; q < 16; ++q) { const int d = lds_conflict_degree(LdsOp::ReadB128, mt_wl_schur(v2, q >= 8, q & 7)); w = d > w ? d : w; }
+  return w;
+}
+static_assert(mt_wl_worst(true) == 1, "Wl: the solve's stores and the Schur stage's loads are conflict-free");
+static_assert(lds_conflict_degree(LdsOp::WriteB128, mt_wl_store(false, 0)) == 6 && lds_conflict_degree(LdsOp::ReadB128, mt_wl_schur(false, false, 0)) == 3 &&
+              lds_conflict_degree(LdsOp::ReadB128, mt_wl_schur(false, true, 0)) == 3, "... and what they were with rows of 128 bytes: 6-way stores, 3-way loads");
+static_assert(MT_DEG(LdsOp::ReadB128, 144, MT_LANES_CONTACT) == 1 && MT_DEG(LdsOp::ReadB128, 48, MT_LANES_CONTACT) == 1 && MT_DEG(LdsOp::WriteB128, 144, MT_LANES_CONTACT) == 1 &&
+              MT_DEG(LdsOp::WriteB128, 48, MT_LANES_CONTACT) == 1, "CJr (144-byte rows), CJh (48-byte rows): lane = contact, conflict-free as they are");
+static_assert(lds_conflict_degree(LdsOp::WriteB128, 0, 48, MT_LANES_DOF, true) == 1 && lds_conflict_degree(LdsOp::WriteB128, 16, 48, MT_LANES_DOF, true) == 1, "Bw, HB, HR, Sh (48-byte rows, lane = dof): conflict-free stores as they are");
+#endif
 struct SharedMT : SharedMTData {
   static constexpr int R = (int)(sizeof(SharedMTData) % 256);
   static constexpr int PAD = R <= 64 ? 64 - R : (R <= 192 ? 192 - R : 320 - R);
@@ -249,6 +335,14 @@
     nearw = (unsigned int)((bal | (bal >> 32)) & 0xFFFFFFFFull);
   }
   PSTAMP(0);
+#ifdef EARL_MT_LDS_V2
+  constexpr bool PARK = ROLE == 1;
+  if constexpr (PARK) {
+#include "minitaur_stepper_pairs.inc"
+  }
+#else
+  constexpr bool PARK = false;
+#endif
   V3 Sw, Sv;
   double I10[10];
   double R[3][3];
@@ -354,6 +448,13 @@
   DBG_PH(3, g6[0] + 2 * g6[1] + 3 * g6[2] + 5 * g6[3] + 7 * g6[4] + 11 * g6[5] + 13 * Add + 17 * Ach);
 #endif
   PSTAMP(4);
+  if constexpr (PARK) {
+    if (isl) {
+#pragma unroll
+      for (int i = 0; i < 6; ++i) s.hand.Bw[l][i] = g6[i];
+    }
+    if (ishinge) { s.hand.Aw[l - 6][0] = Add; s.hand.Aw[l - 6][1] = Ach; }
+  }
   const V3 vlin = ld3(s.qv), om = ld3(s.qv + 3);
   const V3 wb = mulv(Rb, om);
   const V3 vb = add(vlin, cross(Pb, wb));
@@ -408,74 +509,13 @@
   DBG_PH(4, tau_l);
 #endif
   PSTAMP(5);
-  if (nearw) {
-    unsigned int rest = nearw;
-    while (rest) {
-      int myb = -1, myoff = 0, used = 0;
-      unsigned int taken = 0;
-      for (unsigned int r2 = rest; r2; r2 &= r2 - 1u) {
-        const int b = __builtin_ctz(r2);
-        const int sz = bt.end[b] - bt.begin[b];
-        if (used + sz > LPE) { if (used == 0) { taken = 1u << b; used = sz; if (sub < sz) { myb = b; myoff = 0; } } break; }
-        if (sub >= used && sub < used + sz) { myb = b; myoff = used; }
-        used += sz;
-        taken |= 1u << b;
-      }
-      rest &= ~taken;
-      const bool has = myb >= 0;
-      const int b = has ? myb : 0;
-      const bool mine = has && ((nearg >> b) & 1u);
-      const int bsz = bt.end[b] - bt.begin[b];
-      const V3 pb = ld3(bt.box_pos[b]);
-      double Rbx[3][3];
-      qmat(ldq(bt.box_quat[b]), Rbx);
-      const V3 h = ld3(bt.box_half[b]);
-      const int room = bt.cap[b] & 255;
-      const int pi = has ? bt.begin[b] + (sub - myoff < bsz ? sub - myoff : bsz - 1) : 0;
-      const bool valid = mine && sub - myoff < bsz;
-      const int lk = pt.link[pi], cls = pt.cls[pi];
-      const double r = pt.r[pi], margin = pt.margin[pi];
-      V3 c = ld3(pt.pos[pi]);
-      {
-        double Rl[3][3];
-        qmat(ldq(s.dyn.Xq[lk < 0 ? 0 : lk]), Rl);
-        c = selv(lk < 0, c, add(ld3(s.dyn.Xp[lk < 0 ? 0 : lk]), mulv(Rl, c)));
-      }
-      const V3 x = mulvT(Rbx, vsub(c, pb));
-      V3 q{fmin(fmax(x.x, -h.x), h.x), fmin(fmax(x.y, -h.y), h.y), fmin(fmax(x.z, -h.z), h.z)};
-      const bool outside = fabs(x.x) > h.x || fabs(x.y) > h.y || fabs(x.z) > h.z;
-      const V3 dd = vsub(x, q);
-      const double d2 = dot(dd, dd);
-      const double inv = rsq2(outside ? d2 : 1.0);
-      const double gx = h.x - fabs(x.x), gy = h.y - fabs(x.y), gz = h.z - fabs(x.z);
-      const int axn = (gx <= gy && gx <= gz) ? 0 : (gy <= gz ? 1 : 2);
-      const double xa = pick3(x, axn), ha = pick3(h, axn), sg = xa >= 0 ? 1.0 : -1.0;
-      const V3 ni{axn == 0 ? sg : 0.0, axn == 1 ? sg : 0.0, axn == 2 ? sg : 0.0};
-      const V3 qi{axn == 0 ? sg * ha : x.x, axn == 1 ? sg * ha : x.y, axn == 2 ? sg * ha : x.z};
-      const double dist = outside ? d2 * inv - r : -(ha - fabs(xa)) - r;
-      const V3 nl = selv(outside, scl(dd, inv), ni);
-      q = selv(outside, q, qi);
-      const bool hit = valid && dist < margin;
-      const unsigned long long bal = __ballot(hit);
-      const unsigned int gb = (unsigned int)((bal >> (grp * 32)) & 0xFFFFFFFFull);
-      const unsigned int seg = has ? (unsigned int)(((1ull << bsz) - 1ull) << myoff) : 0u;
-      const int before_blk = __popc(gb & seg & ((1u << sub) - 1u));
-      const bool accept = hit && before_blk < room;
-      const unsigned long long bal2 = __ballot(accept);
-      const unsigned int ga = (unsigned int)((bal2 >> (grp * 32)) & 0xFFFFFFFFull);
-      const int slot = nct + __popc(ga & ((1u << sub) - 1u));
-      if (accept && slot < maxcon) {
-        const V3 n = mulv(Rbx, nl);
-        const V3 p = add(add(pb, mulv(Rbx, q)), scl(n, 0.5 * dist));
-        double* o = s.ct[slot];
-        o[0] = dist; o[1] = n.x; o[2] = n.y; o[3] = n.z; o[4] = p.x; o[5] = p.y; o[6] = p.z;
-        o[7] = (double)(cls + 64 * (lk + 1) + 4096 * pi);
-      }
-      const int took = __popc(ga);
-      nct = nct + took < maxcon ? nct + took : maxcon;
-    }
-    fence();
-  }
+#ifdef EARL_MT_LDS_V2
+  if constexpr (ROLE != 1) {
+#include "minitaur_stepper_pairs.inc"
+  }
+#else
+#include "minitaur_stepper_pairs.inc"
+#endif
   PSTAMP(2);
   PCOUNT(20, 1); PCOUNT(21, nearw ? 1 : 0); PCOUNT(22, __popc(nearw));
   if (nearw && __any(nct > 0)) {
@@ -483,6 +523,11 @@
     for (int k = 0; k < MC; ++k) ncmax = __any(nct > k) ? k + 1 : ncmax;
   }
   {
+    if constexpr (PARK) {
+#pragma unroll
+      for (int i = 0; i < 6; ++i) g6[i] = s.hand.Bw[l][i];
+      Add = s.hand.Aw[ishinge ? l - 6 : 0][0]; Ach = s.hand.Aw[ishinge ? l - 6 : 0][1];
+    }
     const int k1 = m.con_att1[leg], k2 = m.con_att2[leg];
     const V3 pa = add(P, mulv(R, ld3(m.att_pos[hq == 3 ? k1 : k2])));
     const V3 p1 = dpp_quad<qp_bcast<3>()>(pa), p2 = dpp_quad<qp_bcast<1>()>(pa);
@@ -819,7 +864,7 @@
       }
       if (sub < 24) {
 #pragma unroll
-        for (int j = 0; j < 4; ++j) s.pas.Wl[i][4 * k + j] = W[j];
+        for (int j = 0; j < 4; ++j) MT_WL(s, i, 4 * k + j) = W[j];
         s.pas.part[i][k] = pt;
         if (i == 0) {
 #pragma unroll
@@ -837,7 +882,7 @@
       double s0 = s.pas.HR[i][c], s1 = 0.0, s2 = 0.0, s3 = 0.0;
       double wi[16], wc[16];
 #pragma unroll
-      for (int p = 0; p < 16; ++p) { wi[p] = s.pas.Wl[i][p]; wc[p] = s.pas.Wl[c][p]; }
+      for (int p = 0; p < 16; ++p) { wi[p] = MT_WL(s, i, p); wc[p] = MT_WL(s, c, p); }
       s0 = pinned(s0); pin_batch(wi); pin_batch(wc);
 #pragma unroll
       for (int p = 0; p < 16; p += 4) {
@@ -863,7 +908,7 @@
       for (int j = 0; j < 4; ++j) {
         z[j] = s.pas.Y[4 * leg + j];
 #pragma unroll
-        for (int i = 0; i < 6; ++i) wl[6 * j + i] = s.pas.Wl[i][4 * leg + j];
+        for (int i = 0; i < 6; ++i) wl[6 * j + i] = MT_WL(s, i, 4 * leg + j);
       }
       pin_batch(Lr); pin_batch(xr); pin_batch(Lk); pin_batch(z);
       chol_small<6>(Lr);
diff --git a/earl_benchmark_amd/csrc/minitaur_stepper_pairs.inc b/earl_benchmark_amd/csrc/minitaur_stepper_pairs.inc
--- /dev/null
+++ b/earl_benchmark_amd/csrc/minitaur_stepper_pairs.inc
@@ -0,0 +1,68 @@
+  if (nearw) {
+    unsigned int rest = nearw;
+    while (rest) {
+      int myb = -1, myoff = 0, used = 0;
+      unsigned int taken = 0;
+      for (unsigned int r2 = rest; r2; r2 &= r2 - 1u) {
+        const int b = __builtin_ctz(r2);
+        const int sz = bt.end[b] - bt.begin[b];
+        if (used + sz > LPE) { if (used == 0) { taken = 1u << b; used = sz; if (sub < sz) { myb = b; myoff = 0; } } break; }
+        if (sub >= used && sub < used + sz) { myb = b; myoff = used; }
+        used += sz;
+        taken |= 1u << b;
+      }
+      rest &= ~taken;
+      const bool has = myb >= 0;
+      const int b = has ? myb : 0;
+      const bool mine = has && ((nearg >> b) & 1u);
+      const int bsz = bt.end[b] - bt.begin[b];
+      const V3 pb = ld3(bt.box_pos[b]);
+      double Rbx[3][3];
+      qmat(ldq(bt.box_quat[b]), Rbx);
+      const V3 h = ld3(bt.box_half[b]);
+      const int room = bt.cap[b] & 255;
+      const int pi = has ? bt.begin[b] + (sub - myoff < bsz ? sub - myoff : bsz - 1) : 0;
+      const bool valid = mine && sub - myoff < bsz;
+      const int lk = pt.link[pi], cls = pt.cls[pi];
+      const double r = pt.r[pi], margin = pt.margin[pi];
+      V3 c = ld3(pt.pos[pi]);
+      {
+        double Rl[3][3];
+        qmat(ldq(s.dyn.Xq[lk < 0 ? 0 : lk]), Rl);
+        c = selv(lk < 0, c, add(ld3(s.dyn.Xp[lk < 0 ? 0 : lk]), mulv(Rl, c)));
+      }
+      const V3 x = mulvT(Rbx, vsub(c, pb));
+      V3 q{fmin(fmax(x.x, -h.x), h.x), fmin(fmax(x.y, -h.y), h.y), fmin(fmax(x.z, -h.z), h.z)};
+      const bool outside = fabs(x.x) > h.x || fabs(x.y) > h.y || fabs(x.z) > h.z;
+      const V3 dd = vsub(x, q);
+      const double d2 = dot(dd, dd);
+      const double inv = rsq2(outside ? d2 : 1.0);
+      const double gx = h.x - fabs(x.x), gy = h.y - fabs(x.y), gz = h.z - fabs(x.z);
+      const int axn = (gx <= gy && gx <= gz) ? 0 : (gy <= gz ? 1 : 2);
+      const double xa = pick3(x, axn), ha = pick3(h, axn), sg = xa >= 0 ? 1.0 : -1.0;
+      const V3 ni{axn == 0 ? sg : 0.0, axn == 1 ? sg : 0.0, axn == 2 ? sg : 0.0};
+      const V3 qi{axn == 0 ? sg * ha : x.x, axn == 1 ? sg * ha : x.y, axn == 2 ? sg * ha : x.z};
+      const double dist = outside ? d2 * inv - r : -(ha - fabs(xa)) - r;
+      const V3 nl = selv(outside, scl(dd, inv), ni);
+      q = selv(outside, q, qi);
+      const bool hit = valid && dist < margin;
+      const unsigned long long bal = __ballot(hit);
+      const unsigned int gb = (unsigned int)((bal >> (grp * 32)) & 0xFFFFFFFFull);
+      const unsigned int seg = has ? (unsigned int)(((1ull << bsz) - 1ull) << myoff) : 0u;
+      const int before_blk = __popc(gb & seg & ((1u << sub) - 1u));
+      const bool accept = hit && before_blk < room;
+      const unsigned long long bal2 = __ballot(accept);
+      const unsigned int ga = (unsigned int)((bal2 >> (grp * 32)) & 0xFFFFFFFFull);
+      const int slot = nct + __popc(ga & ((1u << sub) - 1u));
+      if (accept && slot < maxcon) {
+        const V3 n = mulv(Rbx, nl);
+        const V3 p = add(add(pb, mulv(Rbx, q)), scl(n, 0.5 * dist));
+        double* o = s.ct[slot];
+        o[0] = dist; o[1] = n.x; o[2] = n.y; o[3] = n.z; o[4] = p.x; o[5] = p.y; o[6] = p.z;
+        o[7] = (double)(cls + 64 * (lk + 1) + 4096 * pi);
+      }
+      const int took = __popc(ga);
+      nct = nct + took < maxcon ? nct + took : maxcon;
+    }
+    fence();
+  }
diff --git a/earl_benchmark_amd/csrc/physics_env_minitaur.h b/earl_benchmark_amd/csrc/physics_env_minitaur.h
--- a/earl_benchmark_amd/csrc/physics_env_minitaur.h
+++ b/earl_benchmark_amd/csrc/physics_env_minitaur.h
@@ -108,6 +108,8 @@
 #include "physics_env_minitaur_duo.inc"
 }
 #endif
+#ifndef EARL_MT_LDS_V2
 __global__ __launch_bounds__(128 * MT_DUO_PAIRS, 1) void minitaur_policy_duo_kernel(const MinitaurPolicyArgs a) {
 #include "physics_env_minitaur_duo.inc"
 }
+#endif
diff --git a/earl_benchmark_amd/csrc/physics_env_minitaur_duo.inc b/earl_benchmark_amd/csrc/physics_env_minitaur_duo.inc
--- a/earl_benchmark_amd/csrc/physics_env_minitaur_duo.inc
+++ b/earl_benchmark_amd/csrc/physics_env_minitaur_duo.inc
@@ -51,7 +51,13 @@
     [[maybe_unused]] double rew = 0.0;
     [[maybe_unused]] uint8_t suc = 0;
     if (failed) {
+#ifdef EARL_MT_LDS_V2
+      const double zero = kc(0.0);
+      load_state<NV>(s, m, a.st.qpos + (size_t)env * m.nq, a.st.qvel + (size_t)env * NV, sub, zero);
+#else
+      const double zero = 0.0;
       load_state<NV>(s, m, a.st.qpos + (size_t)env * m.nq, a.st.qvel + (size_t)env * NV, sub);
+#endif
       if (sub < 8) {
         s.ev.oh[sub] = a.st.overheat[(size_t)env * 8 + sub]; s.ev.en[sub] = a.st.motor_enabled[(size_t)env * 8 + sub] != 0 ? 1 : 0; s.ev.obs_t[sub] = a.st.observed_torque[(size_t)env * 8 + sub];
       }
@@ -66,7 +72,7 @@
       if (live) {
         a.out.obs[row * 32 + sub] = v;
         if (sub == 0) {
-          a.out.reward[row] = 0.0; a.out.success[row] = 0;
+          a.out.reward[row] = zero; a.out.success[row] = 0;
           if (a.st.fail_count) a.st.fail_count[env] += 1;
         }
       }
@@ -141,7 +147,13 @@
     fence();
     if (gcf > 0 && ++sgc >= gcf) {
       sgc = 0;
+#ifdef EARL_MT_LDS_V2
+      int n_goals_ = cfg.n_goals;
+      asm volatile("" : "+s"(n_goals_));
+      int gi = (int)(mt_draw(cfg, 0xFFFEu, env, cfg.step_counter + (a.clock ? a.clock[1] : 0) + (uint64_t)t) * (double)n_goals_);
+#else
       int gi = (int)(mt_draw(cfg, 0xFFFEu, env, cfg.step_counter + (a.clock ? a.clock[1] : 0) + (uint64_t)t) * (double)cfg.n_goals);
+#endif
       gi = gi >= cfg.n_goals ? cfg.n_goals - 1 : gi;
       goal0 = cfg.goal_table[2 * gi]; goal1 = cfg.goal_table[2 * gi + 1];
       if constexpr (POLICY) {
@@ -210,6 +222,11 @@
     } else if (j >= 1) {
       const int jj = j - 1, q = jj & 1, ts = jj >> 1;
       if (ts < TT) {
+#ifdef EARL_MT_LDS_V2
+        int lane_ = lane;
+        asm volatile("" : "+v"(lane_));
+        const int grp = lane_ / LPE;
+#endif
         SharedMT& s = sh[(pair * 2 + q) * EPW + grp];
         int sub_ = sub;
         asm volatile("" : "+v"(sub_));
diff --git a/earl_benchmark_amd/csrc/physics_launch.h b/earl_benchmark_amd/csrc/physics_launch.h
--- a/earl_benchmark_amd/csrc/physics_launch.h
+++ b/earl_benchmark_amd/csrc/physics_launch.h
@@ -11,6 +11,7 @@
 extern "C" __attribute__((visibility("hidden"))) int earl_unit_w8_bf16_sawyer_policy_rollout(const void* sawyer_policy_args, void* stream);
 extern "C" __attribute__((visibility("hidden"))) int earl_unit_mt_bf16_policy_rollout(const void* minitaur_policy_args, int duo, void* stream);
 extern "C" __attribute__((visibility("hidden"))) void earl_unit_kitchen_bf16_policy_rollout(const void* kitchen_policy_args, void* stream);
+extern "C" __attribute__((visibility("hidden"))) int earl_unit_mt_v2_rollout(const void* minitaur_args, int form, void* stream);
 extern "C" __attribute__((visibility("hidden"))) int earl_unit_branch_replicate(const void* sawyer_branch_args, const void* src_state, int nv, void* stream);
 extern "C" __attribute__((visibility("hidden"))) int earl_unit_branch_sawyer_rollout(const void* sawyer_branch_args, int nv, int sliced, void* stream);
 extern "C" __attribute__((visibility("hidden"))) int earl_unit_branch_w8_sawyer_rollout(const void* sawyer_branch_args, void* stream);
diff --git a/earl_benchmark_amd/csrc/physics_mt.hip b/earl_benchmark_amd/csrc/physics_mt.hip
--- a/earl_benchmark_amd/csrc/physics_mt.hip
+++ b/earl_benchmark_amd/csrc/physics_mt.hip
@@ -14,6 +14,12 @@
 
 int g_mt_stepper = 1;
 int g_mt_duo = EARL_MT_DUO_DEFAULT;
+
+#if defined(EARL_PHYS_PROF) || defined(EARL_MT_DEBUG)
+int g_mt_layout = 0;
+#else
+int g_mt_layout = 1;
+#endif
 
 bool mt_use_duo(int n) {
   const int cus = cu_count();
@@ -44,6 +50,7 @@
   if (int rc = check_cone(col, false, (hipStream_t)stream, "minitaur_rollout")) return rc;
   MinitaurArgs a{model24, col, *cfg, *st, *out, action, T, nullptr, nullptr, solo_mode(cfg->n), clock};
   const MtForm form = minitaur_form(cfg->n, a.solo, cfg->num_substeps);
+  if (g_mt_layout == 1 && form != MtForm::Generic) return earl_unit_mt_v2_rollout(&a, form == MtForm::Duo ? 1 : 0, stream);
   if (form == MtForm::Duo) {
     minitaur_duo_kernel<<<(unsigned)((cfg->n + 16 * MT_DUO_PAIRS / 4 - 1) / (4 * MT_DUO_PAIRS)), 128 * MT_DUO_PAIRS, 0, (hipStream_t)stream>>>(a);
     return launched("minitaur_rollout (two waves per SIMD)");
@@ -124,6 +131,11 @@
   if (mode >= -1 && mode <= 1) g_mt_duo = mode;
   return prev;
 }
+int earl_debug_set_minitaur_layout(int layout) {
+  const int prev = g_mt_layout;
+  if (layout == 0 || layout == 1) g_mt_layout = layout;
+  return prev;
+}
 #ifdef EARL_MT_DEBUG
 int earl_debug_read_mt_dbg(int* out_i, double* out_d) {
   if (hipMemcpyFromSymbol(out_i, HIP_SYMBOL(g_mt_dbg), sizeof(int) * 4096 * 8 * 32) != hipSuccess) return EARL_ERR_LAUNCH;
diff --git a/earl_benchmark_amd/csrc/physics_mt_v2.hip b/earl_benchmark_amd/csrc/physics_mt_v2.hip
--- /dev/null
+++ b/earl_benchmark_amd/csrc/physics_mt_v2.hip
@@ -0,0 +1,26 @@
+#define EARL_MT_LDS_V2 1
+#include "minitaur_device.h"
+#include "physics_stepper.h"
+#include "policy_check.h"
+#include "policy_math.h"
+
+namespace {
+#include "minitaur_stepper.h"
+#include "physics_env_minitaur.h"
+}
+
+#include "physics_launch.h"
+
+extern "C" {
+
+int earl_unit_mt_v2_rollout(const void* minitaur_args, int form, void* stream) {
+  const MinitaurArgs& a = *static_cast<const MinitaurArgs*>(minitaur_args);
+  if (form == 1) {
+    minitaur_duo_kernel<<<(unsigned)((a.cfg.n + 16 * MT_DUO_PAIRS / 4 - 1) / (4 * MT_DUO_PAIRS)), 128 * MT_DUO_PAIRS, 0, (hipStream_t)stream>>>(a);
+    return launched("minitaur_rollout (two waves per SIMD, second LDS layout)");
+  }
+  minitaur_kernel<false, true><<<solo_grid(a.cfg.n, a.solo, EARL_MT_WPB), 64 * EARL_MT_WPB, 0, (hipStream_t)stream>>>(a);
+  return launched("minitaur_rollout (second LDS layout)");
+}
+
+}
diff --git a/earl_benchmark_amd/csrc/physics_stepper.h b/earl_benchmark_amd/csrc/physics_stepper.h
--- a/earl_benchmark_amd/csrc/physics_stepper.h
+++ b/earl_benchmark_amd/csrc/physics_stepper.h
@@ -1917,12 +1917,12 @@
 }
 
 template <int NV, typename SH>
-__device__ __forceinline__ void load_state(SH& s, const typename ModelOf<NV>::T& m, const double* __restrict__ qrow, const double* __restrict__ vrow, const int sub) {
+__device__ __forceinline__ void load_state(SH& s, const typename ModelOf<NV>::T& m, const double* __restrict__ qrow, const double* __restrict__ vrow, const int sub, const double aprev0 = 0.0) {
   const int bd = m.ball_dof;
   if (sub < NV) {
     s.qp[sub] = (bd < 0 || sub < bd) ? qrow[sub] : (sub > bd + 2 ? qrow[sub + 1] : 0.0);
     s.qv[sub] = vrow[sub];
-    s.aprev[sub] = 0.0;
+    s.aprev[sub] = aprev0;
   }
   if (sub < 4) {
     double v = sub == 0 ? 1.0 : 0.0;
diff --git a/include/earl_physics.h b/include/earl_physics.h
--- a/include/earl_physics.h
+++ b/include/earl_physics.h
@@ -414,6 +414,7 @@
 int earl_minitaur_cfg_size(void);
 int earl_debug_set_minitaur_stepper(int tree);
 int earl_debug_set_minitaur_duo(int mode);
+int earl_debug_set_minitaur_layout(int layout);
 int earl_debug_set_solo(int mode);
 int earl_debug_set_solo_mt(int mode);
 
```

Measured after the change: 77.16 billion. No clear change (-0.6%).
